# kubernetes-sigs/karpenter

Measured on NVIDIA H100. Metric: pods scheduled/sec, higher is better.
Workload: dtype int64

## Files before the change

### karpenter_b200/csrc/kp_api.cu

```cuda
#include <cuda_runtime.h>
#include <cub/cub.cuh>

#include <dlfcn.h>

#include <chrono>
#include <cstdio>
#include <cstdlib>
#include <memory>
#include <string>
#include <vector>

#include "kp_consolidate.cuh"
#include "kp_gosort_host.hpp"
#include "kp_prep.hpp"

#define CK(call)                                                                                     \
  do {                                                                                               \
    cudaError_t e_ = (call);                                                                         \
    if (e_ != cudaSuccess) {                                                                         \
      h->err = std::string(#call) + ": " + cudaGetErrorString(e_);                                   \
      return KP_ERR_CUDA;                                                                            \
    }                                                                                                \
  } while (0)

// ... 199 lines not shown
  if (i >= n) return;
  const KeyInfo ki{val_int, isint, univ};
  const kp_slot_case c = cs[i];
  const Slot a{c.flags_a, c.mask_a, c.gte_a, c.lte_a}, b{c.flags_b, c.mask_b, c.gte_b, c.lte_b};
  kp_slot_out o;
  memset(&o, 0, sizeof(o));
  if (slot_present(a) && slot_present(b)) {
    const Slot r = slot_intersection(ki, a, b);
    o.mask = r.m;
    o.gte = r.gte;
    o.lte = r.lte;
    o.flags = r.f;
    o.op = slot_op(r);
    o.has_intersection = slot_has_intersection(ki, a, b);
  }
  o.has_value = c.value >= 0 ? slot_has(ki, a, c.value) : 0;
  o.compatible = slot_compatible(ki, a, b, c.well_known != 0, c.allow_undefined != 0);
  out[i] = o;
}

static int kp_consolidate_impl(kp_handle* h, const kp_problem* p, const kp_consol_input* in, int64_t deadline_ms,
                               kp_consol_result* out);
extern "C" {

int kp_debug_slot_algebra(kp_handle* h, const int64_t* value_int, uint64_t value_is_int, uint64_t universe,
                          const kp_slot_case* cases, int32_t n, kp_slot_out* out) {
  if (n < 0 || !value_int || (n > 0 && (!cases || !out))) return h->err = "kp_debug_slot_algebra: bad arguments", KP_ERR_INVALID;
  cudaSetDevice(h->device);
  int64_t* dv = nullptr;
  kp_slot_case* dc = nullptr;
  kp_slot_out* dout = nullptr;
  CK(cudaMalloc(&dv, 64 * 8));
  CK(cudaMalloc(&dc, sizeof(kp_slot_case) * std::max(n, 1)));
  CK(cudaMalloc(&dout, sizeof(kp_slot_out) * std::max(n, 1)));
  CK(cudaMemcpy(dv, value_int, 64 * 8, cudaMemcpyHostToDevice));
  CK(cudaMemcpy(dc, cases, sizeof(kp_slot_case) * n, cudaMemcpyHostToDevice));
  if (n > 0) k_slot_kats<<<(n + 127) / 128, 128, 0, h->stream>>>(dv, value_is_int, universe, dc, n, dout);
  CK(cudaStreamSynchronize(h->stream));
  CK(cudaGetLastError());
  CK(cudaMemcpy(out, dout, sizeof(kp_slot_out) * n, cudaMemcpyDeviceToHost));
  cudaFree(dv);
  cudaFree(dc);
  cudaFree(dout);
  return KP_OK;
}
}

extern "C" {

#define KP_TRUNC_BLOCKS 132
int kp_version(void) { return KP_ABI_VERSION; }

int kp_go_sort_f64(const double* keys, int32_t n, int32_t* perm_out) {
  if (n < 0 || (n > 0 && (!keys || !perm_out))) return KP_ERR_INVALID;
  host_go_sort(keys, n, perm_out);
  return KP_OK;
}
int kp_go_sort_i64(const int64_t* keys, int32_t n, int32_t* perm_out) {
  if (n < 0 || (n > 0 && (!keys || !perm_out))) return KP_ERR_INVALID;
  host_go_sort(keys, n, perm_out);
  return KP_OK;
}

int kp_create(int device, kp_handle** out) {
  *out = nullptr;
  int count = 0;
  if (cudaGetDeviceCount(&count) != cudaSuccess || count == 0) return KP_ERR_CUDA;
  kp_handle* h = new kp_handle();
  if (device < 0) cudaGetDevice(&device);
  h->device = device;
  if (cudaSetDevice(device) != cudaSuccess || cudaStreamCreate(&h->stream) != cudaSuccess) {
    delete h;
    return KP_ERR_CUDA;
  }
  cudaEventCreate(&h->ev0);
  cudaEventCreate(&h->ev1);
  cudaEventCreate(&h->ev3);
  cudaDeviceGetAttribute(&h->n_sm, cudaDevAttrMultiProcessorCount, device);
  cudaDeviceSetLimit(cudaLimitStackSize, 16384);
  *out = h;
  return KP_OK;
}

void kp_destroy(kp_handle* h) {
  if (!h) return;
  cudaSetDevice(h->device);
  h->arena.destroy();
  cudaFree(h->d_devs);
  cudaFree(h->d_plan);
  if (h->comm && g_nccl.CommDestroy) g_nccl.CommDestroy(h->comm);
  if (h->ev3) cudaEventDestroy(h->ev3);
  if (h->ev0) cudaEventDestroy(h->ev0);
  if (h->ev1) cudaEventDestroy(h->ev1);
  if (h->stream) cudaStreamDestroy(h->stream);
  delete h;
}

const char* kp_last_error(kp_handle* h) { return h ? h->err.c_str() : "no handle"; }

int kp_get_stats(kp_handle* h, kp_stats* out) {
  *out = h->stats;
  return KP_OK;
}

static int upload_tables(kp_handle* h, Instance& in, const kp_problem* p, int cmax_hint) {
  HostTables& t = in.host;
  KpDev& d = in.dev;
  memset(&d, 0, sizeof(d));
  d.K = t.K;
  d.R = t.R;
  d.T = t.T;
  d.ITW = t.ITW;
  d.N = t.N;
  d.X = t.X;
  d.G = t.G;
  d.GH = t.GH;
  d.E = t.E;
  d.D = t.D;
  d.n_reqsets = t.n_reqsets;
  d.n_taintsets = t.n_taintsets;
  d.n_tolsets = t.n_tolsets;
  d.has_bounds = t.has_bounds;
  d.hostname_key = t.hostname_key;
  d.nodes_res = t.nodes_res;
  d.n_rv = t.n_rv;
  d.stable_order = p->claim_order_mode == 1;
  CK(up(h, &d.key_wellknown, t.key_wellknown));
  CK(up(h, &d.key_univ, t.key_univ));
  CK(up(h, &d.val_int, t.val_int));
  CK(up(h, &d.val_isint, t.val_isint));
  CK(up(h, &d.rs_flags, t.rs_flags));
  CK(up(h, &d.rs_mask, t.rs_mask));
  CK(up(h, &d.rs_gte, t.rs_gte));
  CK(up(h, &d.rs_lte, t.rs_lte));
  CK(up(h, &d.tol_ok, t.tol_ok));
  CK(up(h, &d.itv_off, t.itv_off));
  CK(up(h, &d.itv, t.itv));
  CK(up(h, &d.it_nokey, t.it_nokey));
  CK(up(h, &d.it_dne, t.it_dne));
  CK(up(h, &d.it_nonempty, t.it_nonempty));
  CK(up(h, &d.it_valid, t.it_valid));
  CK(up(h, &d.ge_off, t.ge_off));
  CK(up(h, &d.ge_vals, t.ge_vals));
  CK(up(h, &d.ge_bits, t.ge_bits));
  d.n_ge = (int)t.ge_vals.size();
  d.n_itv = std::max(t.itv_off[d.K], 1);
  CK(up(h, &d.off_slots, t.off_slots));
  CK(up(h, &d.off_keys, t.off_keys));
  CK(up(h, &d.offset_bits, t.offset_bits));
  CK(up(h, &d.it_capacity, t.it_capacity));
  CK(up(h, &d.tmpl_rs, t.tmpl_rs));
  CK(up(h, &d.tmpl_taintset, t.tmpl_taintset));
  CK(up(h, &d.tmpl_its_raw, t.tmpl_its_raw));
  CK(zeros(h, &d.tmpl_its, t.tmpl_its_raw.size()));
  CK(up(h, &d.tmpl_daemon, t.tmpl_daemon));
  CK(up_mut(h, in, &d.tmpl_remaining, t.tmpl_remaining));
  CK(up(h, &d.tmpl_limit_present, t.tmpl_limit_present));
  CK(up(h, &d.cls_req, t.cls_req));
  CK(up(h, &d.cls_rs, t.cls_rs));
  CK(up(h, &d.cls_tolset, t.cls_tolset));
  CK(up(h, &d.cls_relax, t.cls_relax));
  d.mv_strict = t.min_values_strict ? 1 : 0;
  CK(up(h, &d.tmpl_mv_off, t.tmpl_mv_off));
  CK(up(h, &d.tmpl_mv_key, t.tmpl_mv_key));
  CK(up(h, &d.tmpl_mv_need, t.tmpl_mv_need));
  CK(up(h, &d.mv_val_off, t.mv_val_off));
  CK(up(h, &d.mv_masks, t.mv_masks));
  CK(up(h, &d.cls_match, t.cls_match));
  CK(up(h, &d.cls_rec, t.cls_rec));
  {
    if (t.N > 64) return h->err = "more than 64 NodePools", KP_ERR_CAPACITY;
    const ClassPlan& plan = t.plan;
    const bool domain_fp = !getenv("KP_NO_DOMAIN_FP");
    const size_t XK = (size_t)std::max(t.X, 1) * t.K;
    std::vector<int64_t> pg(XK, 0), pl(XK, 0), sg(XK, 0), sl(XK, 0);
    std::vector<ClsLane> rows((size_t)std::max(t.X, 1) * 32);
    memset(rows.data(), 0, rows.size() * sizeof(ClsLane));
    for (int x = 0; x < t.X; x++) {
      const int nm = t.cls_match_off[x + 1] - t.cls_match_off[x], nr = t.cls_rec_off[x + 1] - t.cls_rec_off[x];
      const int asig = plan.asig[x];
      int tki = 0xff;
      if (!plan.chain[x]) {
        tki = asig < 64 ? asig | TKI_ABIT : 0xff;
        if (plan.fast[x] && asig < 64) tki |= TKI_FAST;
        if (plan.fp[x] && nm <= KP_PG && nr <= KP_PG && domain_fp) tki |= TKI_FP | (plan.has_tk[x] ? TKI_TK : 0);
        if (nm + nr > 0) tki |= TKI_TOPO;
      }
      const int32_t hdr[KP_HDR] = {t.cls_tolset[x], t.cls_rv[x], t.cls_match_off[x], t.cls_match_off[x + 1], t.cls_rec_off[x],
                                   t.cls_rec_off[x + 1], plan.fsig[x], plan.nsig[x], plan.hchk_off[x], plan.hchk_off[x + 1]};
      const size_t a = (size_t)t.cls_rs[x] * t.K, b = (size_t)t.cls_strict_rs[x] * t.K;
      for (int l = 0; l < 32; l++) {
        ClsLane& c = rows[(size_t)x * 32 + l];
        if (l < t.K) {
          c.pod_m = t.rs_mask[a + l];
          c.strict_m = t.rs_mask[b + l];
          c.pod_f = t.rs_flags[a + l];
          c.strict_f = t.rs_flags[b + l];
          pg[(size_t)x * t.K + l] = t.rs_gte[a + l];
          pl[(size_t)x * t.K + l] = t.rs_lte[a + l];
          sg[(size_t)x * t.K + l] = t.rs_gte[b + l];
          sl[(size_t)x * t.K + l] = t.rs_lte[b + l];
        }
        if (l < t.R) c.req = t.cls_req[(size_t)x * t.R + l];
        if (l < KP_HDR) c.hdr = hdr[l];
        if (l == KP_HDR + 2) c.hdr = (int32_t)(plan.tok[x] & 0xffffffffull);
        if (l == KP_HDR + 3) c.hdr = (int32_t)(plan.tok[x] >> 32);
        if (l == KP_HDR + 4) c.hdr = t.cls_relax[x];
        if (l == KP_HDR + 5) c.hdr = tki;
        if (l == KP_HDR + 10) c.hdr = t.cls_vol_next[x];
        if (l >= KP_HDR + 6 && l <= KP_HDR + 9 && p->n_hostports > 0 && p->class_hostports) {
          const uint64_t ports = p->class_hostports[x];
          uint64_t conf = 0;
          for (uint64_t m = ports; m;) {
            const int i = __builtin_ctzll(m);
            m &= m - 1;
            conf |= p->hostport_conflicts[i];
          }
          const uint64_t v = l < KP_HDR + 8 ? ports : conf;
          c.hdr = (int32_t)(((l - KP_HDR) & 1) ? (v >> 32) : (v & 0xffffffffull));
        }
      }
    }
    std::vector<int4> hchk;
    for (const HostCheck& c : plan.hchk) hchk.push_back(int4{c.row, c.type | (c.self << 8), c.max_skew, c.g});
    if (hchk.empty()) hchk.push_back(int4{0, 0, 0, 0});
    std::vector<int32_t> nsig_rs = plan.nsig_rs, nsig_tolset = plan.nsig_tolset;
    if (nsig_rs.empty()) {
      nsig_rs.push_back(0);
      nsig_tolset.push_back(-1);
    }
    d.tk_key = plan.tk_key;
    d.n_fsig = plan.n_fsig;
    d.n_nsig = (int)plan.nsig_rs.size();
    d.EW = (t.E + 31) / 32;
    in.strict_undefined = plan.strict_undefined ? 1 : 0;
    std::vector<int64_t> rv_req((size_t)std::max(t.n_rv, 1) * t.R, 0);
    for (int x = 0; x < t.X; x++)
      for (int r = 0; r < t.R; r++) rv_req[(size_t)t.cls_rv[x] * t.R + r] = t.cls_req[(size_t)x * t.R + r];
    {
      const int32_t *a_, *b_;
      const int64_t* c_;
      CK(up(h, &a_, nsig_rs));
      CK(up(h, &b_, nsig_tolset));
      CK(up(h, &c_, rv_req));
      in.d_nsig_rs = const_cast<int32_t*>(a_);
      in.d_nsig_tolset = const_cast<int32_t*>(b_);
      in.d_rv_req = const_cast<int64_t*>(c_);
    }
    CK(up(h, &d.cls_hchk, hchk));
    std::vector<uint32_t> nact(std::max(d.EW, 1), 0);
    for (int n = 0; n < t.E; n++)
      if (t.node_flags[n] & KP_NODE_SCHEDULABLE) nact[n >> 5] |= 1u << (n & 31);
    CK(up_mut(h, in, &d.nactive, nact));
    d.ESW = (d.EW + 31) / 32;
    CK(zeros(h, &d.nfit_sum, (size_t)std::max(t.n_rv, 1) * std::max(d.ESW, 1)));
    CK(zeros(h, &d.nstat_sum, (size_t)std::max(d.n_nsig, 1) * std::max(d.ESW, 1)));
    CK(zeros(h, &d.nfit, (size_t)std::max(t.n_rv, 1) * std::max(d.EW, 1)));
    CK(zeros(h, &d.nstat, (size_t)std::max(d.n_nsig, 1) * std::max(d.EW, 1)));
    CK(up(h, &d.cls_lane, rows));
    CK(up(h, &d.cp_g, pg));
    CK(up(h, &d.cp_l, pl));
    CK(up(h, &d.cs_g, sg));
    CK(up(h, &d.cs_l, sl));
  }
  CK(up(h, &d.groups, t.groups));
  CK(up(h, &d.filter_rs, t.filter_rs));
  CK(up_mut(h, in, &d.dom_cnt, t.dom_cnt));
  CK(up_mut(h, in, &d.dom_reg, t.dom_reg));
  CK(up_mut(h, in, &d.dom_pop, t.dom_pop));
  d.tk_slot = nullptr;
  d.tk_reg = d.tk_pop = nullptr;
  d.tk_cnt = nullptr;
  d.tk_nv = t.plan.tk_key >= 0 ? 64 - __builtin_clzll(t.key_univ[t.plan.tk_key] | 1ull) : 0;
  d.n_lazy = 0;
  for (int32_t b : t.g_born) d.n_lazy += b == 0;
  CK(up_mut(h, in, &d.g_born, t.g_born));
  CK(up_mut(h, in, &d.g_birth, t.g_birth));
  CK(up(h, &d.cls_lazy_off, t.cls_lazy_off));
  CK(up(h, &d.cls_lazy, t.cls_lazy));
  CK(up_mut(h, in, &d.g_ndomains, t.g_ndomains));
  CK(up_mut(h, in, &d.g_nempty, t.g_nempty));
  CK(up(h, &d.node_taintset, t.node_taintset));
  CK(up(h, &d.node_flags, t.node_flags));
  CK(up_mut(h, in, &d.node_rem, t.node_rem));
  CK(up_mut(h, in, &d.node_rem_present, t.node_rem_present));
  CK(up_mut(h, in, &d.node_sflags, t.node_sflags));
  CK(up_mut(h, in, &d.node_smask, t.node_smask));
  CK(up_mut(h, in, &d.node_sgte, t.node_sgte));
  CK(up_mut(h, in, &d.node_slte, t.node_slte));
  CK(zeros(h, &d.node_npods, (size_t)std::max(t.E, 1)));
  d.Cmax = cmax_hint;
  size_t C = (size_t)d.Cmax;
  CK(zeros(h, &d.c_tmpl, C));
  CK(zeros(h, &d.c_npods, C));
  CK(zeros(h, &d.c_req, C * t.R));
  CK(zeros(h, &d.c_sflags, C * t.K));
  CK(zeros(h, &d.c_smask, C * t.K));
  CK(zeros(h, &d.c_sgte, C * t.K));
  CK(zeros(h, &d.c_slte, C * t.K));
  CK(zeros(h, &d.c_its, C * t.ITW));
  CK(zeros(h, &d.c_j, C * t.R));
  CK(zeros(h, &d.order, C));
  CK(zeros(h, &d.cnt_at, C));
  CK(zeros(h, &d.cmask, C));
  CK(zeros(h, &d.amask, C));
  CK(zeros(h, &d.c_dom, C));
  d.n_hostports = p->n_hostports > 0 ? p->n_hostports : 0;
  if (d.n_hostports > 64) return h->err = "more than 64 distinct host ports", KP_ERR_CAPACITY;
  if (d.n_hostports > 0 && !p->hostport_conflicts) return h->err = "hostport_conflicts is null", KP_ERR_INVALID;
  {
    std::vector<unsigned long long> np(std::max(t.E, 1), 0ull), tp(std::max(t.N, 1), 0ull);
    for (int n = 0; n < t.E; n++)
      if (d.n_hostports && p->node_hostports) np[n] = p->node_hostports[n];
    for (int n = 0; n < t.N; n++)
      if (d.n_hostports && p->tmpl_hostports) tp[n] = p->tmpl_hostports[n];
    CK(up_mut(h, in, &d.node_ports, np));
    CK(up(h, &d.tmpl_ports, tp));
    CK(zeros(h, &d.c_ports, C));
  }
  d.n_rsv = t.n_rsv;
  d.rsv_strict = t.rsv_strict ? 1 : 0;
  d.rsv_sets = 0;
  {
    std::vector<int32_t> sr(std::max(t.D, 1), -1);
    for (int dd = 0; dd < t.D && dd < (int)t.set_rsv.size(); dd++) {
      sr[dd] = t.set_rsv[dd];
      if (sr[dd] >= 0) d.rsv_sets |= 1u << dd;
    }
    CK(up(h, &d.set_rsv, sr));
    std::vector<int32_t> cap0 = t.rsv_cap0;
    if (cap0.empty()) cap0.push_back(0);
    CK(up_mut(h, in, &d.rsv_cap, cap0));
    CK(zeros(h, &d.c_rsv, C));
    d.rsv_ct_key = p->reservation_capacity_type_key;
    d.rsv_reserved_val = p->reservation_reserved_value;
    d.rsv_id_key = p->reservation_id_key;
    memset(d.rsv_val_of, 0, sizeof(d.rsv_val_of));
    if (t.n_rsv > 0) {
      if (d.rsv_ct_key < 0 || d.rsv_ct_key >= t.K || d.rsv_id_key < 0 || d.rsv_id_key >= t.K || !p->reservation_value ||
          d.rsv_reserved_val < 0 || d.rsv_reserved_val >= 64)
        return h->err = "reserved offerings need reservation_capacity_type_key / reservation_id_key / reservation_value", KP_ERR_INVALID;
      for (int i = 0; i < t.n_rsv; i++) {
        if (p->reservation_value[i] < 0 || p->reservation_value[i] >= 64) return h->err = "reservation_value out of range", KP_ERR_INVALID;
        d.rsv_val_of[i] = 1ull << p->reservation_value[i];
      }
    }
  }
  d.tmpl_all = t.N >= 64 ? ~0ull : ((1ull << t.N) - 1);
  d.H = t.E + d.Cmax;
  d.GHS = std::max(t.GH, 1);
  CK(zeros(h, &d.host_cnt, (size_t)d.GHS * d.H));
  {
    std::vector<int32_t> tr((size_t)std::max(t.E, 1) * d.GHS, 0);
    for (int r = 0; r < t.GH; r++)
      for (int n = 0; n < t.E; n++) tr[(size_t)n * d.GHS + r] = t.host_cnt_nodes[(size_t)r * t.E + n];
    CK(up(h, &in.d_host_cnt_nodes, tr));
  }
  d.HW = (d.H + 31) / 32;
  CK(zeros(h, &d.host_pop, (size_t)std::max(t.GH, 1) * d.HW));
  {
    const int ew = (t.E + 31) / 32;
    std::vector<uint32_t> bits((size_t)std::max(t.GH, 1) * std::max(ew, 1), 0);
    for (int r = 0; r < t.GH; r++)
      for (int n = 0; n < t.E; n++)
        if (t.host_cnt_nodes[(size_t)r * t.E + n] > 0) bits[(size_t)r * ew + (n >> 5)] |= 1u << (n & 31);
    CK(up(h, &in.d_host_pop_nodes, bits));
  }
  CK(zeros(h, &d.n_claims, 1));
  CK(zeros(h, &d.counters, KP_NCOUNTERS));
  CK(zeros(h, &d.status, 1));
  return KP_OK;
}

static int reset_dynamic(kp_handle* h, Instance& in) {
  HostTables& t = in.host;
  KpDev& d = in.dev;
  for (auto& r : in.resets) CK(cudaMemcpyAsync(r.dst, r.src, r.bytes, cudaMemcpyDeviceToDevice, h->stream));
  CK(cudaMemsetAsync(d.node_npods, 0, (size_t)std::max(t.E, 1) * 4, h->stream));
  size_t C = (size_t)d.Cmax;
  CK(cudaMemsetAsync(d.c_npods, 0, C * 4, h->stream));
  CK(cudaMemsetAsync(d.cmask, 0, C * sizeof(ulonglong2), h->stream));
  CK(cudaMemsetAsync(d.amask, 0, C * 8, h->stream));
  CK(cudaMemsetAsync(d.c_rsv, 0, C * 8, h->stream));
  if (in.d_dropped) CK(cudaMemsetAsync(in.d_dropped, 0, C, h->stream));
  CK(cudaMemsetAsync(d.host_cnt, 0, (size_t)d.GHS * d.H * 4, h->stream));
  if (t.E && t.GH)
    CK(cudaMemcpyAsync(d.host_cnt, in.d_host_cnt_nodes, (size_t)t.E * d.GHS * 4, cudaMemcpyDeviceToDevice, h->stream));
  CK(cudaMemsetAsync(d.host_pop, 0, (size_t)std::max(t.GH, 1) * d.HW * 4, h->stream));
  if (t.E && t.GH) {
    const size_t ew = (size_t)(t.E + 31) / 32;
    CK(cudaMemcpy2DAsync(d.host_pop, (size_t)d.HW * 4, in.d_host_pop_nodes, ew * 4, ew * 4, t.GH,
                         cudaMemcpyDeviceToDevice, h->stream));
  }
  CK(cudaMemsetAsync(d.n_claims, 0, 4, h->stream));
  CK(cudaMemsetAsync(d.counters, 0, 128, h->stream));
  CK(cudaMemsetAsync(d.status, 0, 4, h->stream));
  CK(cudaMemsetAsync(d.last_len, 0, (size_t)std::max<int64_t>(in.P, 1) * 4, h->stream));
  return KP_OK;
}

static int plan_tables(const KpDev& d, size_t fixed, size_t budget) {
  const size_t tb = kp_tab_bytes(d);
  return (fixed + tb <= budget && tb <= 110 * 1024) ? (int)tb : 0;
}

static void plan_solve(Instance& in) {
  KpDev& d = in.dev;
  const size_t budget = 224 * 1024;
  d.tab_bytes = plan_tables(d, SolveSmem(d, 0, 0, 0, 0, 0).tab, budget);
  auto layout = [&](int CS, int CQ, int CR) { return SolveSmem(d, d.tab_bytes, CS, CQ, CR, in.tk_groups); };
  const bool dom_fp = std::any_of(in.host.plan.fp.begin(), in.host.plan.fp.end(), [](uint8_t f) { return f != 0; });
  in.tk_groups = 0;
  if (dom_fp && !in.cohort && d.tk_key >= 0 && d.tk_nv > 0 && d.tk_nv <= 64) {
    int ntk = 0;
    for (const KpGroup& G : in.host.groups) ntk += G.key == d.tk_key;
    const SolveSmem L(d, d.tab_bytes, 0, 0, 0, ntk);
    if (ntk > 0 && L.s_req - L.tk_slot <= 64 * 1024) in.tk_groups = ntk;
  }
  int CR = std::min(d.Cmax, 512);
  while (CR > 0 && layout(0, CR, CR).cmask > budget / 2) CR -= 32;
  CR = std::max(CR, 0);
  const SolveSmem whole = layout(0, CR, CR);
  const size_t rows = whole.cmask - whole.s_req;
  int CQ = CR;
  if (dom_fp) {
    CQ = std::min((d.Cmax + 31) / 32 * 32, (int)(rows / ((size_t)d.R * 12 + 1)) / 32 * 32);
    while (CQ > 0 && layout(0, CQ, 0).cmask - whole.s_req > rows) CQ -= 32;
    CR = 0;
    while (CR + 32 <= CQ && layout(0, CQ, CR + 32).cmask - whole.s_req <= rows) CR += 32;
  }
  int CS = 0;
  if (layout(64, CQ, CR).total <= budget) {
    int lo = 64, hi = ((d.Cmax + 31) / 32) * 32;
    while (lo < hi) {
      int mid = ((lo + hi + 32) / 64) * 32;
      if (mid <= lo) mid = lo + 32;
      if (layout(mid, CQ, CR).total <= budget)
        lo = mid;
      else
        hi = mid - 32;
    }
    CS = lo;
  }
  if (const char* cap = getenv("KP_SMEM_CAP")) {
    long v[4];
    bool set[4] = {false, false, false, false};
    for (int f = 0; f < 4 && cap; f++) {
      char* end;
      v[f] = std::max(0l, strtol(cap, &end, 10));
      set[f] = end != cap;
      cap = strchr(cap, ',');
      if (cap) cap++;
    }
    if (set[0]) CS = (int)std::min<long>(CS, v[0] / 32 * 32);
    if (set[1]) CQ = (int)std::min<long>(CQ, v[1]);
    if (set[2]) CR = (int)std::min<long>(CR, v[2]);
    if (set[3] && v[3] < in.tk_groups) in.tk_groups = 0;
  }
  CR = std::min(CR, CQ);
  in.lean = in.host.G == 0 && !in.host.has_bounds && !in.host.min_values_strict && in.host.n_rsv == 0 && d.n_hostports == 0 &&
            !in.host.has_vol_alts && !getenv("KP_NO_LEAN");
  if (in.host.has_vol_alts) in.cohort = false;
  in.CS = CS;
  in.CQ = CQ;
  in.CR = CR;
  in.smem = layout(CS, CQ, CR).total;
  if (getenv("KP_DEBUG"))
    fprintf(stderr, "[kp] solver plan: tables %zu B, topology-key groups on chip %d, hot rows %d, cold rows %d, small arrays %d, %zu B shared\n",
            (size_t)d.tab_bytes, in.tk_groups, CQ, CR, CS, in.smem);
}

static void begin_upload(kp_handle* h, kp_handle::Uploader by) {
  cudaSetDevice(h->device);
  cudaStreamSynchronize(h->stream);
  h->insts.clear();
  h->uploaded = by;
  h->d_gcnt = nullptr;
  h->gcnt_slots = 0;
  h->arena.reset();
  h->stats = kp_stats{};
}

static int add_instance(kp_handle* h, const kp_problem* p, int64_t cmax) {
  h->insts.push_back(std::make_unique<Instance>());
  Instance& in = *h->insts.back();
  auto t0 = std::chrono::steady_clock::now();
  std::vector<uint8_t> active(p->n_nodes, 0);
  for (int i = 0; i < p->n_nodes; i++) active[i] = (p->node_flags[i] & KP_NODE_SCHEDULABLE) != 0;
  std::vector<int32_t> pending(p->pod_class, p->pod_class + p->n_pods);
  int rc = kp_prepare(p, active, {}, pending, in.host, h->err);
  if (rc != KP_OK) return rc;
  auto t1 = std::chrono::steady_clock::now();
  h->stats.prep_ms += std::chrono::duration<double, std::milli>(t1 - t0).count();
  in.P = p->n_pods;
  in.n_keys = p->n_keys;
  in.n_resources = p->n_resources;
  in.n_its = p->n_its;
  in.n_nodes = p->n_nodes;
  in.hostname_key = in.host.hostname_key;
  in.key_nvalues.resize(p->n_keys);
  for (int k = 0; k < p->n_keys; k++) in.key_nvalues[k] = p->key_value_off[k + 1] - p->key_value_off[k];
  if (p->n_pods >= (1ll << 31) - 2) return h->err = "more than 2^31 pods", KP_ERR_CAPACITY;
  rc = upload_tables(h, in, p, (int)cmax);
  if (rc != KP_OK) return rc;
  KpDev& d = in.dev;
  d.P = p->n_pods;
  size_t P = (size_t)p->n_pods;
  CK(up_raw(h, &in.d_pod_class, p->pod_class, P));
  d.pod_class = in.d_pod_class;
  if (p->pod_creation) {
    CK(up_raw(h, &in.d_pod_creation, p->pod_creation, P));
  } else {
    CK(zeros(h, &in.d_pod_creation, P));
  }
  CK(up_raw(h, &in.d_uid_hi, p->pod_uid_hi, P));
  CK(up_raw(h, &in.d_uid_lo, p->pod_uid_lo, P));
  const std::vector<int64_t>& rank = in.host.plan.rank;
  CK(up_raw(h, &in.d_class_rank, rank.data(), rank.size()));
  {
    const int X = in.host.X;
    std::vector<int64_t> pods_of(std::max(X, 1), 0), classes_at(std::max(X, 1), 0);
    for (size_t i = 0; i < P; i++) pods_of[p->pod_class[i]]++;
    for (int x = 0; x < X; x++)
      if (pods_of[x] > 0) classes_at[rank[x]]++;
    int64_t in_runs = 0;
    for (int x = 0; x < X; x++)
      if (pods_of[x] > 1 && classes_at[rank[x]] == 1) in_runs += pods_of[x];
    in.cohort = (in_runs * 4 >= (int64_t)P && P > 0 && !getenv("KP_NO_COHORT")) || getenv("KP_COHORT");
    d.cohort = in.cohort ? 1 : 0;
  }
  in.max_its = p->max_instance_types > 0 ? p->max_instance_types : 0;
  if (in.max_its > 0) {
    const int T = p->n_its;
    const PriceLists ml = order_by_price(p, in.host);
    CK(up(h, &in.price_tabs.ml_off, ml.off));
    CK(up(h, &in.price_tabs.ml_set, ml.set));
    CK(up(h, &in.price_tabs.ml_price, ml.price));
    const size_t NW = (size_t)KP_TRUNC_BLOCKS * 4;
    CK(h->arena.alloc(&in.trunc_key, NW * std::max(T, 1)));
    CK(h->arena.alloc(&in.trunc_val, NW * std::max(T, 1)));
    CK(h->arena.alloc(&in.trunc_bits, NW * std::max((T + 63) / 64, 1)));
    CK(zeros(h, &in.d_dropped, (size_t)std::max<int64_t>(d.Cmax, 1)));
  }
  {
    int64_t* ka;
    int64_t* kb;
    CK(h->arena.alloc(&ka, P));
    CK(h->arena.alloc(&kb, P));
    CK(h->arena.alloc(&in.sort_perm_b, P));
    in.sort_keys_a = ka;
    in.sort_keys_b = kb;
    size_t n1 = 0, n2 = 0;
    cub::DeviceRadixSort::SortPairs(nullptr, n1, (const uint64_t*)nullptr, (uint64_t*)nullptr, (const int32_t*)nullptr,
                                    (int32_t*)nullptr, (int)std::max<size_t>(P, 1));
    cub::DeviceRadixSort::SortPairs(nullptr, n2, (const int64_t*)nullptr, (int64_t*)nullptr, (const int32_t*)nullptr,
                                    (int32_t*)nullptr, (int)std::max<size_t>(P, 1));
    in.sort_tmp_bytes = std::max(n1, n2);
    char* tmp;
    CK(h->arena.alloc(&tmp, in.sort_tmp_bytes));
    in.sort_tmp = tmp;
  }
  CK(zeros(h, &d.queue, P + 1));
  CK(zeros(h, &d.qcls, P + 1));
  CK(zeros(h, &d.last_len, P));
  CK(zeros(h, &d.pod_target, P));
  CK(zeros(h, &d.pod_error, P));
  CK(cudaStreamSynchronize(h->stream));
  auto t2 = std::chrono::steady_clock::now();
  h->stats.upload_ms += std::chrono::duration<double, std::milli>(t2 - t1).count();
  plan_solve(in);
  in.resident = true;
  return KP_OK;
}

static int upload(kp_handle* h, const kp_problem* const* problems, int n, const int64_t* cmax, kp_handle::Uploader by) {
  begin_upload(h, by);
  for (int b = 0; b < n; b++) {
    int rc = add_instance(h, problems[b], cmax[b]);
    if (rc != KP_OK) return rc;
  }
  return KP_OK;
}

static int64_t cmax_guess(const kp_problem* p) {
  return std::max<int64_t>(1, std::min<int64_t>(p->n_pods, std::max<int64_t>(4096, p->n_pods / 8)));
}

int kp_upload(kp_handle* h, const kp_problem* p) {
  const int64_t cmax = cmax_guess(p);
  return upload(h, &p, 1, &cmax, kp_handle::SINGLE);
}

__global__ void k_iota(int32_t* p, int64_t n) {
  int64_t i = blockIdx.x * (int64_t)blockDim.x + threadIdx.x;
  if (i < n) p[i] = (int32_t)i;
}

static int sort_queue(kp_handle* h, Instance& in) {
  KpDev& d = in.dev;
  const int64_t P = in.P;
  if (P <= 0) return KP_OK;
  const int nb = (int)((P + 255) / 256), n = (int)P;
  int32_t* perm_a = d.queue;
  int32_t* perm_b = in.sort_perm_b;
  uint64_t *ua = (uint64_t*)in.sort_keys_a, *ub = (uint64_t*)in.sort_keys_b;
  int64_t *sa = (int64_t*)in.sort_keys_a, *sb = (int64_t*)in.sort_keys_b;
  size_t tb = in.sort_tmp_bytes;
  k_iota<<<nb, 256, 0, h->stream>>>(perm_a, P);
  k_gather<<<nb, 256, 0, h->stream>>>(in.d_uid_lo, perm_a, P, ua);
  CK(cub::DeviceRadixSort::SortPairs(in.sort_tmp, tb, ua, ub, perm_a, perm_b, n, 0, 64, h->stream));
  k_gather<<<nb, 256, 0, h->stream>>>(in.d_uid_hi, perm_b, P, ua);
  CK(cub::DeviceRadixSort::SortPairs(in.sort_tmp, tb, ua, ub, perm_b, perm_a, n, 0, 64, h->stream));
  k_gather<<<nb, 256, 0, h->stream>>>(in.d_pod_creation, perm_a, P, sa);
  CK(cub::DeviceRadixSort::SortPairs(in.sort_tmp, tb, sa, sb, perm_a, perm_b, n, 0, 64, h->stream));
  k_sort_keys<<<nb, 256, 0, h->stream>>>(d.pod_class, in.d_class_rank, perm_b, P, sa);
  CK(cub::DeviceRadixSort::SortPairs(in.sort_tmp, tb, sa, sb, perm_b, perm_a, n, 0, 64, h->stream));
  k_gather<<<nb, 256, 0, h->stream>>>(d.pod_class, d.queue, P, d.qcls);
  h->stats.kernel_launches += 6;
  return KP_OK;
}

static int launch_node_cand(kp_handle* h, Instance& in) {
  KpDev& d = in.dev;
  if (d.E <= 0) return KP_OK;
  dim3 grid((d.E + 255) / 256, d.n_nsig + d.n_rv);
  k_node_cand<<<grid, 256, 0, h->stream>>>(d, in.d_nsig_rs, in.d_nsig_tolset, in.d_rv_req, in.strict_undefined);
  const int nsum = (d.n_rv + d.n_nsig) * d.ESW;
  k_node_sum<<<(nsum + 255) / 256, 256, 0, h->stream>>>(d);
  h->stats.kernel_launches += 2;
  return KP_OK;
}

static int prep_solve(kp_handle* h, Instance& in) {
  KpDev& d = in.dev;
  if (d.N > 0) {
    k_feasibility<<<(d.N * 32 + 255) / 256, 256, 0, h->stream>>>(d, nullptr, 1);
    h->stats.kernel_launches++;
  }
  int rc = sort_queue(h, in);
  if (rc != KP_OK) return rc;
  if (in.P > 0) {
    k_fill_i32<<<(int)((in.P + 255) / 256), 256, 0, h->stream>>>(d.pod_target, in.P, KP_TARGET_UNSCHEDULED);
    h->stats.kernel_launches++;
  }
  return launch_node_cand(h, in);
}

static int reduce_counters(kp_handle* h) {
  if (!h->d_gcnt) return KP_OK;
  CK(cudaEventRecord(h->ev3, h->stream));
  CK(cudaMemsetAsync(h->d_gcnt, 0, (size_t)h->gcnt_slots * 4, h->stream));
  for (auto& in : h->insts)
    if (in->n_slots > 0) {
      k_scatter_counts<<<(int)((in->n_slots + 255) / 256), 256, 0, h->stream>>>(in->dev.dom_cnt, in->d_slot_src, in->n_slots,
                                                                                 h->d_gcnt + in->slot_off);
      h->stats.kernel_launches++;
    }
  if (h->comm) {
    int rc = g_nccl.AllReduce(h->d_gcnt, h->d_gcnt, (size_t)h->gcnt_slots,  2,  0, h->comm, h->stream);
    if (rc != 0) return h->err = std::string("ncclAllReduce: ") + (g_nccl.GetErrorString ? g_nccl.GetErrorString(rc) : "?"), KP_ERR_CUDA;
  }
  return KP_OK;
}

static const void* solver_kernel(const std::vector<std::unique_ptr<Instance>>& insts) {
  bool lean = true, cohort = false, vol = false;
  for (auto& in : insts) {
    lean = lean && in->lean;
    cohort = cohort || in->cohort;
    vol = vol || in->host.has_vol_alts;
  }
  if (vol) return (const void*)k_wsolve_batch<false, false, true>;
  return lean ? (cohort ? (const void*)k_wsolve_batch<true, true> : (const void*)k_wsolve_batch<true, false>)
              : (cohort ? (const void*)k_wsolve_batch<false, true> : (const void*)k_wsolve_batch<false, false>);
}

static int run_solve(kp_handle* h, int64_t deadline_ms, std::vector<int32_t>& statuses) {
  const int n = (int)h->insts.size();
  statuses.assign(n, KP_OK);
  if (n == 0) return KP_OK;
  cudaSetDevice(h->device);
  if (n > h->devs_cap) {
    cudaFree(h->d_devs);
    cudaFree(h->d_plan);
    h->d_devs = nullptr;
    h->d_plan = nullptr;
    h->devs_cap = 0;
    CK(cudaMalloc(&h->d_devs, sizeof(KpDev) * n));
    CK(cudaMalloc(&h->d_plan, sizeof(int4) * n));
    h->devs_cap = n;
  }
  std::vector<KpDev> devs(n);
  std::vector<int4> plan(n);
  size_t smem = 0;
  for (int b = 0; b < n; b++) {
    Instance& in = *h->insts[b];
    if (!in.resident) return h->err = "the last upload did not complete", KP_ERR_INVALID;
    in.dev.deadline_ns = deadline_ms > 0 ? deadline_ms * 1000000ll : 0;
    int rc = reset_dynamic(h, in);
    if (rc != KP_OK) return rc;
    devs[b] = in.dev;
    plan[b] = make_int4(in.CS, in.CQ, in.CR, in.tk_groups);
    smem = std::max(smem, in.smem);
  }
  CK(cudaMemcpyAsync(h->d_devs, devs.data(), sizeof(KpDev) * n, cudaMemcpyHostToDevice, h->stream));
  CK(cudaMemcpyAsync(h->d_plan, plan.data(), sizeof(int4) * n, cudaMemcpyHostToDevice, h->stream));
  CK(cudaEventRecord(h->ev0, h->stream));
  h->stats.kernel_launches = 0;
  h->stats.cohort_pods = 0;
  for (auto& in : h->insts) {
    int rc = prep_solve(h, *in);
    if (rc != KP_OK) return rc;
  }
  const void* fn = solver_kernel(h->insts);
  CK(cudaFuncSetAttribute(fn, cudaFuncAttributeMaxDynamicSharedMemorySize, (int)smem));
  {
    void* args[] = {(void*)&h->d_devs, (void*)&h->d_plan};
    CK(cudaLaunchKernel(fn, dim3(n), dim3(64), args, smem, h->stream));
  }
  h->stats.kernel_launches++;
  for (auto& in : h->insts)
    if (in->max_its > 0) {
      k_truncate_claims<<<KP_TRUNC_BLOCKS, 128, 0, h->stream>>>(in->dev, in->price_tabs, in->max_its, in->trunc_key, in->trunc_val,
                                                                 in->trunc_bits, in->d_dropped);
      if (in->P > 0)
        k_mark_dropped<<<(int)((in->P + 255) / 256), 256, 0, h->stream>>>(in->dev.pod_target, in->dev.pod_error, in->d_dropped, in->P);
      h->stats.kernel_launches += 2;
    }
  int rc = reduce_counters(h);
  if (rc != KP_OK) return rc;
  CK(cudaEventRecord(h->ev1, h->stream));
  CK(cudaStreamSynchronize(h->stream));
  CK(cudaGetLastError());
  float ms = 0;
  cudaEventElapsedTime(&ms, h->ev0, h->ev1);
  h->stats.solve_ms = ms;
  if (h->d_gcnt) cudaEventElapsedTime(&h->allreduce_ms, h->ev3, h->ev1);
  if (getenv("KP_DEBUG")) fprintf(stderr, "[kp] %d instance(s): step %.3f ms\n", n, ms);
  for (int b = 0; b < n; b++) CK(cudaMemcpy(&statuses[b], h->insts[b]->dev.status, 4, cudaMemcpyDeviceToHost));
  return KP_OK;
}

struct ReqLayout {
  int K, hostname_key;
  std::vector<int> woff;
  explicit ReqLayout(const Instance& in) : K(in.n_keys), hostname_key(in.hostname_key), woff(in.n_keys + 1, 0) {
    for (int k = 0; k < K; k++) woff[k + 1] = woff[k] + (k == hostname_key ? 0 : (in.key_nvalues[k] + 63) / 64);
  }
  int words() const { return woff[K]; }
  void store(size_t r, const uint8_t* sf, const uint64_t* sm, const int64_t* sg, const int64_t* sl, uint8_t* flags,
             int64_t* gte, int64_t* lte, uint64_t* mask) const {
    for (int k = 0; k < K; k++) {
      const uint8_t f = sf[k];
      if (!(f & SF_PRESENT) || k == hostname_key) continue;
      flags[r * K + k] = KP_SLOT_PRESENT | ((f & SF_COMPLEMENT) ? KP_REQ_COMPLEMENT : 0) | ((f & SF_HAS_GTE) ? KP_REQ_HAS_GTE : 0) |
                         ((f & SF_HAS_LTE) ? KP_REQ_HAS_LTE : 0);
      if ((f & SF_HAS_GTE) && sg) gte[r * K + k] = sg[k];
      if ((f & SF_HAS_LTE) && sl) lte[r * K + k] = sl[k];
      if (woff[k + 1] > woff[k]) mask[r * words() + woff[k]] = sm[k];
    }
  }
};

static int download(kp_handle* h, Instance& in, kp_result* out) {
  KpDev& d = in.dev;
  auto t0 = std::chrono::steady_clock::now();
  memset(out, 0, sizeof(*out));
  int32_t nclaims = 0;
  int64_t counters[16];
  CK(cudaMemcpy(&nclaims, d.n_claims, 4, cudaMemcpyDeviceToHost));
  CK(cudaMemcpy(counters, d.counters, 128, cudaMemcpyDeviceToHost));
  h->stats.cohort_pods += counters[5];
  if (getenv("KP_DEBUG"))
    fprintf(stderr, "[kp] slow_sorts=%lld evals=%lld commits=%lld fast_commits=%lld cohort_pods=%lld\n", (long long)counters[4],
            (long long)counters[6], (long long)counters[3], (long long)counters[9], (long long)counters[5]);
  int64_t P = in.P;
  int K = in.n_keys, R = in.n_resources, ITW = (in.n_its + 63) / 64;
  size_t C = (size_t)nclaims, c1 = C ? C : 1;
  out->n_pods = P;
  out->pod_target = (int32_t*)malloc(sizeof(int32_t) * (P ? P : 1));
  out->pod_error = (uint8_t*)malloc(P ? P : 1);
  CK(cudaMemcpy(out->pod_target, d.pod_target, P * 4, cudaMemcpyDeviceToHost));
  CK(cudaMemcpy(out->pod_error, d.pod_error, P, cudaMemcpyDeviceToHost));
  out->n_claims = nclaims;
  out->claim_template = (int32_t*)calloc(c1, 4);
  out->claim_npods = (int32_t*)calloc(c1, 4);
  out->claim_rank = (int32_t*)calloc(c1, 4);
  out->claim_reservations = (uint64_t*)calloc(c1, 8);
  CK(cudaMemcpy(out->claim_reservations, d.c_rsv, C * 8, cudaMemcpyDeviceToHost));
  out->claim_dropped = (uint8_t*)calloc(c1, 1);
  if (in.d_dropped) CK(cudaMemcpy(out->claim_dropped, in.d_dropped, C, cudaMemcpyDeviceToHost));
  out->claim_requests = (int64_t*)calloc(c1 * R, 8);
  out->it_words = ITW;
  out->claim_its = (uint64_t*)calloc(c1 * (ITW ? ITW : 1), 8);
  CK(cudaMemcpy(out->claim_template, d.c_tmpl, C * 4, cudaMemcpyDeviceToHost));
  CK(cudaMemcpy(out->claim_npods, d.c_npods, C * 4, cudaMemcpyDeviceToHost));
  CK(cudaMemcpy(out->claim_requests, d.c_req, C * R * 8, cudaMemcpyDeviceToHost));
  CK(cudaMemcpy(out->claim_its, d.c_its, C * ITW * 8, cudaMemcpyDeviceToHost));
  std::vector<int32_t> order(c1);
  CK(cudaMemcpy(order.data(), d.order, C * 4, cudaMemcpyDeviceToHost));
  for (size_t pos = 0; pos < C; pos++) out->claim_rank[order[pos]] = (int32_t)pos;
  std::vector<uint8_t> sf(c1 * K);
  std::vector<uint64_t> sm(c1 * K);
  std::vector<int64_t> sg(c1 * K), sl(c1 * K);
  CK(cudaMemcpy(sf.data(), d.c_sflags, C * K, cudaMemcpyDeviceToHost));
  CK(cudaMemcpy(sm.data(), d.c_smask, C * K * 8, cudaMemcpyDeviceToHost));
  CK(cudaMemcpy(sg.data(), d.c_sgte, C * K * 8, cudaMemcpyDeviceToHost));
  CK(cudaMemcpy(sl.data(), d.c_slte, C * K * 8, cudaMemcpyDeviceToHost));
  const ReqLayout L(in);
  const int MW = L.words();
  out->n_keys = K;
  out->mask_words = MW;
  out->claim_req_flags = (uint8_t*)calloc(c1 * (K ? K : 1), 1);
  out->claim_req_gte = (int64_t*)calloc(c1 * (K ? K : 1), 8);
  out->claim_req_lte = (int64_t*)calloc(c1 * (K ? K : 1), 8);
  out->claim_req_mask = (uint64_t*)calloc(c1 * (MW ? MW : 1), 8);
  for (size_t c = 0; c < C; c++)
    L.store(c, sf.data() + c * K, sm.data() + c * K, sg.data() + c * K, sl.data() + c * K, out->claim_req_flags,
            out->claim_req_gte, out->claim_req_lte, out->claim_req_mask);
  HostTables& t = in.host;
  std::vector<int32_t> cnt((size_t)std::max(t.G, 1) * 64);
  CK(cudaMemcpy(cnt.data(), d.dom_cnt, cnt.size() * 4, cudaMemcpyDeviceToHost));
  std::vector<int32_t> birth(std::max(t.G, 1));
  CK(cudaMemcpy(birth.data(), d.g_birth, birth.size() * 4, cudaMemcpyDeviceToHost));
  std::vector<int> gorder;
  for (int g = 0; g < t.n_regular; g++)
    if (t.g_born[g]) gorder.push_back(g);
  {
    std::vector<std::pair<int, int>> born;
    for (int g = 0; g < t.n_regular; g++)
      if (!t.g_born[g] && birth[g] >= 0) born.push_back({birth[g], g});
    std::sort(born.begin(), born.end());
    for (auto& b : born) gorder.push_back(b.second);
  }
  for (int g = t.n_regular; g < t.G; g++) gorder.push_back(g);
  std::vector<int32_t> off{0}, flat;
  for (int g : gorder) {
    int key = t.groups[g].key;
    if (key != t.hostname_key) {
      int nv = in.key_nvalues[key];
      for (int v = 0; v < nv; v++) flat.push_back(cnt[(size_t)g * 64 + v]);
    }
    off.push_back((int32_t)flat.size());
  }
  out->n_groups = (int32_t)gorder.size();
  out->n_domain_slots = (int32_t)flat.size();
  out->group_domain_off = (int32_t*)malloc(off.size() * 4);
  memcpy(out->group_domain_off, off.data(), off.size() * 4);
  out->domain_counts = (int32_t*)malloc((flat.size() ? flat.size() : 1) * 4);
  if (!flat.empty()) memcpy(out->domain_counts, flat.data(), flat.size() * 4);
  out->n_existing_evals = counters[0];
  out->n_inflight_evals = counters[1];
  out->n_template_evals = counters[2];
  out->n_commits = counters[3];
  out->solve_ms = h->stats.solve_ms;
  h->stats.bytes_d2h += P * 5 + C * (8 + (size_t)R * 8 + (size_t)ITW * 8 + (size_t)K * 25) + cnt.size() * 4;
  auto t1 = std::chrono::steady_clock::now();
  h->stats.download_ms += std::chrono::duration<double, std::milli>(t1 - t0).count();
  return KP_OK;
}

static int download_all(kp_handle* h, const std::vector<int32_t>& statuses, kp_result* outs) {
  h->stats.download_ms = 0;
  h->stats.bytes_d2h = 0;
  int worst = KP_OK;
  for (size_t b = 0; b < h->insts.size(); b++) {
    int rc = download(h, *h->insts[b], &outs[b]);
    if (rc != KP_OK) {
      for (size_t i = 0; i < b; i++) kp_result_free(&outs[i]);
      return rc;
    }
    if (statuses[b] == KP_DEADLINE) worst = KP_DEADLINE;
  }
  return worst;
}

static int solve_uploaded(kp_handle* h, int64_t deadline_ms, kp_result* outs) {
  std::vector<int32_t> st;
  int rc = run_solve(h, deadline_ms, st);
  if (rc != KP_OK) return rc;
  for (int32_t s : st)
    if (s != KP_OK && s != KP_DEADLINE) return h->err = "claim capacity exceeded", s;
  return download_all(h, st, outs);
}

static int solve_growing(kp_handle* h, const kp_problem* const* problems, int n, kp_handle::Uploader by, int64_t deadline_ms,
                         kp_result* outs) {
  std::vector<int64_t> cmax(n);
  for (int b = 0; b < n; b++) cmax[b] = cmax_guess(problems[b]);
  for (;;) {
    int rc = upload(h, problems, n, cmax.data(), by);
    if (rc != KP_OK) return rc;
    std::vector<int32_t> st;
    rc = run_solve(h, deadline_ms, st);
    if (rc != KP_OK) return rc;
    bool grow = false;
    for (int b = 0; b < n; b++) {
      if (st[b] == KP_ERR_CAPACITY && cmax[b] < problems[b]->n_pods) {
        cmax[b] = std::min<int64_t>(problems[b]->n_pods, cmax[b] * 4);
        grow = true;
      } else if (st[b] != KP_OK && st[b] != KP_DEADLINE) {
        return h->err = "claim capacity exceeded", st[b];
      }
    }
    if (!grow) return download_all(h, st, outs);
  }
}

int kp_solve_resident(kp_handle* h, int64_t deadline_ms, kp_result* out) {
  if (h->uploaded != kp_handle::SINGLE) return h->err = "kp_upload has not been called", KP_ERR_INVALID;
  return solve_uploaded(h, deadline_ms, out);
}

int kp_solve(kp_handle* h, const kp_problem* p, int64_t deadline_ms, kp_result* out) {
  return solve_growing(h, &p, 1, kp_handle::SINGLE, deadline_ms, out);
}

int kp_comm_unique_id(uint8_t* id128) {
  std::string err;
  if (!nccl_load(err)) return KP_ERR_CUDA;
  KpNcclId id;
  if (g_nccl.GetUniqueId(&id) != 0) return KP_ERR_CUDA;
  memcpy(id128, &id, sizeof(id));
  return KP_OK;
}

int kp_comm_init(kp_handle* h, const uint8_t* id128, int32_t rank, int32_t world) {
  if (!nccl_load(h->err)) return KP_ERR_CUDA;
  if (h->comm) {
    g_nccl.CommDestroy(h->comm);
    h->comm = nullptr;
  }
  cudaSetDevice(h->device);
  KpNcclId id;
  memcpy(&id, id128, sizeof(id));
  int rc = g_nccl.CommInitRank(&h->comm, world, id, rank);
  if (rc != 0) return h->err = std::string("ncclCommInitRank: ") + (g_nccl.GetErrorString ? g_nccl.GetErrorString(rc) : "?"), KP_ERR_CUDA;
  h->comm_rank = rank;
  h->comm_world = world;
  return KP_OK;
}

static Instance* pick_instance(kp_handle* h, int32_t instance) {
  const size_t i = instance < 0 ? 0 : (size_t)instance;
  if (h->uploaded != (instance < 0 ? kp_handle::SINGLE : kp_handle::BATCH) || i >= h->insts.size()) return nullptr;
  return h->insts[i]->resident ? h->insts[i].get() : nullptr;
}
int64_t kp_comm_counter_slots(kp_handle* h, int32_t instance) {
  Instance* in = pick_instance(h, instance);
  if (!in) return -1;
  int64_t n = 0;
  for (int g = 0; g < in->host.G; g++)
    if (in->host.groups[g].key != in->host.hostname_key) n += in->key_nvalues[in->host.groups[g].key];
  return n;
}

int kp_comm_set_counter_layout(kp_handle* h, int64_t total_slots, const int64_t* slot_offset, int32_t n_instances) {
  cudaSetDevice(h->device);
  if (n_instances <= 0 ? !pick_instance(h, -1) : h->uploaded != kp_handle::BATCH || n_instances != (int)h->insts.size())
    return h->err = "kp_comm_set_counter_layout: the instances do not match the upload", KP_ERR_INVALID;
  if (total_slots < 0) return h->err = "kp_comm_set_counter_layout: negative size", KP_ERR_INVALID;
  CK(h->arena.alloc(&h->d_gcnt, (size_t)std::max<int64_t>(total_slots, 1)));
  h->gcnt_slots = total_slots;
  for (size_t i = 0; i < h->insts.size(); i++) {
    Instance* in = h->insts[i].get();
    std::vector<int32_t> src;
    for (int g = 0; g < in->host.G; g++) {
      const int key = in->host.groups[g].key;
      if (key == in->host.hostname_key) continue;
      for (int v = 0; v < in->key_nvalues[key]; v++) src.push_back(g * 64 + v);
    }
    in->n_slots = (int64_t)src.size();
    in->slot_off = slot_offset[i];
    if (in->slot_off < 0 || in->slot_off + in->n_slots > total_slots)
      return h->err = "kp_comm_set_counter_layout: slice outside the table", KP_ERR_INVALID;
    CK(h->arena.alloc(&in->d_slot_src, std::max<size_t>(src.size(), 1)));
    if (!src.empty()) CK(cudaMemcpyAsync(in->d_slot_src, src.data(), src.size() * 4, cudaMemcpyHostToDevice, h->stream));
    CK(cudaStreamSynchronize(h->stream));
  }
  return KP_OK;
}

int kp_comm_global_counts(kp_handle* h, int32_t* out, int64_t n) {
  if (!h->d_gcnt || n != h->gcnt_slots) return h->err = "kp_comm_global_counts: no table of that size", KP_ERR_INVALID;
  cudaSetDevice(h->device);
  CK(cudaMemcpy(out, h->d_gcnt, (size_t)n * 4, cudaMemcpyDeviceToHost));
  return KP_OK;
}

double kp_comm_last_allreduce_ms(kp_handle* h) { return h->allreduce_ms; }

#ifdef KP_PHASE_PROF
int kp_phase_profile(kp_handle* h, int32_t instance, int64_t* out, int32_t n) {
  Instance* in = pick_instance(h, instance);
  if (!in || n < KP_NPHASE + 1) return h->err = "kp_phase_profile: no such instance or buffer too small", -1;
  cudaSetDevice(h->device);
  CK(cudaMemcpy(out, in->dev.counters + KP_PROF_AT, (KP_NPHASE + 1) * 8, cudaMemcpyDeviceToHost));
  return KP_NPHASE + 1;
}
#endif

void kp_comm_destroy(kp_handle* h) {
  if (h->comm && g_nccl.CommDestroy) g_nccl.CommDestroy(h->comm);
  h->comm = nullptr;
}

int kp_upload_batch(kp_handle* h, const kp_problem* const* problems, int32_t n) {
  if (n < 0 || (n > 0 && !problems)) return h->err = "kp_upload_batch: bad arguments", KP_ERR_INVALID;
  std::vector<int64_t> cmax(n);
  for (int b = 0; b < n; b++) cmax[b] = cmax_guess(problems[b]);
  return upload(h, problems, n, cmax.data(), kp_handle::BATCH);
}

int kp_solve_batch_resident(kp_handle* h, int64_t deadline_ms, kp_result* outs) {
  if (h->uploaded != kp_handle::BATCH) return KP_OK;
  return solve_uploaded(h, deadline_ms, outs);
}

int kp_solve_batch(kp_handle* h, const kp_problem* const* problems, int32_t n, int64_t deadline_ms, kp_result* outs) {
  if (n < 0 || (n > 0 && (!problems || !outs))) return h->err = "kp_solve_batch: bad arguments", KP_ERR_INVALID;
  return solve_growing(h, problems, n, kp_handle::BATCH, deadline_ms, outs);
}

void kp_result_free(kp_result* r) {
  free(r->pod_target);
  free(r->pod_error);
  free(r->claim_template);
  free(r->claim_npods);
  free(r->claim_rank);
  free(r->claim_requests);
  free(r->claim_its);
  free(r->claim_req_flags);
  free(r->claim_req_gte);
  free(r->claim_req_lte);
  free(r->claim_req_mask);
  free(r->group_domain_off);
  free(r->domain_counts);
  free(r->claim_reservations);
  free(r->claim_dropped);
  memset(r, 0, sizeof(*r));
}

int kp_feasibility(kp_handle* h, const kp_problem* p, uint64_t* out_bits, int32_t* out_it_words) {
  const int64_t one = 1;
  int rc = upload(h, &p, 1, &one, kp_handle::SINGLE);
  if (rc != KP_OK) return rc;
  KpDev& d = h->insts[0]->dev;
  *out_it_words = d.ITW;
  size_t n = (size_t)d.X * d.N * d.ITW;
  uint64_t* dout;
  CK(cudaMalloc(&dout, std::max<size_t>(n, 1) * 8));
  if (d.N > 0) k_feasibility<<<(d.N * 32 + 255) / 256, 256, 0, h->stream>>>(d, nullptr, 1);
  CK(cudaEventRecord(h->ev0, h->stream));
  if (d.N > 0 && d.X > 0) {
    int blocks = h->n_sm * 8;
    k_feasibility<<<blocks, 256, 0, h->stream>>>(d, dout, 0);
  }
  CK(cudaEventRecord(h->ev1, h->stream));
  CK(cudaStreamSynchronize(h->stream));
  CK(cudaGetLastError());
  float ms = 0;
  cudaEventElapsedTime(&ms, h->ev0, h->ev1);
  h->stats.solve_ms = ms;
  CK(cudaMemcpy(out_bits, dout, n * 8, cudaMemcpyDeviceToHost));
  cudaFree(dout);
  return KP_OK;
}

int kp_consolidate(kp_handle* h, const kp_problem* cluster, const kp_consol_input* in, int64_t deadline_ms,
                   kp_consol_result* out) {
  memset(out, 0, sizeof(*out));
  int rc = kp_consolidate_impl(h, cluster, in, deadline_ms, out);
  if (rc != KP_OK && rc != KP_DEADLINE) kp_consol_result_free(out);
  return rc;
}

void kp_consol_result_free(kp_consol_result* r) {
  free(r->decision);
  free(r->replacement_its);
  free(r->n_new_claims);
  free(r->n_unscheduled);
  free(r->repl_template);
  free(r->repl_requests);
  free(r->repl_req_flags);
  free(r->repl_req_gte);
  free(r->repl_req_lte);
  free(r->repl_req_mask);
  free(r->repl_order_off);
  free(r->repl_order);
  memset(r, 0, sizeof(*r));
}
}

__global__ void k_scatter_rank(const int32_t* perm, int64_t n, int32_t* rank) {
  int64_t i = blockIdx.x * (int64_t)blockDim.x + threadIdx.x;
  if (i < n) rank[perm[i]] = (int32_t)i;
}

static int read_consol(kp_handle* h, const KpConsol& q, int n, const int32_t* at, const ReqLayout& L, int R, int ITW,
                       std::vector<std::vector<int32_t>>& order_rows, kp_consol_result* out) {
  const size_t K = (size_t)L.K, n1 = (size_t)std::max(n, 1), cap = (size_t)q.order_cap;
  auto sub = [&](size_t b) { return at ? (size_t)at[b] : b; };
  auto rows = [&](auto* dst, const auto* src, size_t width) {
    const size_t row = width * sizeof(*dst);
    if (!at) return cudaMemcpy(dst, src, n * row, cudaMemcpyDeviceToHost);
    std::vector<std::remove_pointer_t<decltype(dst)>> tmp(n1 * width);
    const cudaError_t e = cudaMemcpy(tmp.data(), src, n * row, cudaMemcpyDeviceToHost);
    for (size_t b = 0; b < (size_t)n; b++) memcpy(dst + sub(b) * width, tmp.data() + b * width, row);
    return e;
  };
  CK(rows(out->decision, q.decision, 1));
  CK(rows(out->replacement_its, q.replacement_its, ITW));
  CK(rows(out->n_new_claims, q.n_new_claims, 1));
  CK(rows(out->n_unscheduled, q.n_unscheduled, 1));
  CK(rows(out->repl_template, q.repl_tmpl, 1));
  CK(rows(out->repl_requests, q.repl_req, R));
  std::vector<uint8_t> sfl(n1 * K);
  std::vector<uint64_t> smk(n1 * K);
  std::vector<int32_t> on(n1), ord(q.repl_order ? n1 * cap : 0);
  std::vector<int64_t> sg(q.repl_sgte ? n1 * K : 0), sl(sg.size());
  CK(cudaMemcpy(sfl.data(), q.repl_sflags, (size_t)n * K, cudaMemcpyDeviceToHost));
  CK(cudaMemcpy(smk.data(), q.repl_smask, (size_t)n * K * 8, cudaMemcpyDeviceToHost));
  if (q.repl_sgte) {
    CK(cudaMemcpy(sg.data(), q.repl_sgte, (size_t)n * K * 8, cudaMemcpyDeviceToHost));
    CK(cudaMemcpy(sl.data(), q.repl_slte, (size_t)n * K * 8, cudaMemcpyDeviceToHost));
  }
  if (q.repl_order) {
    CK(cudaMemcpy(ord.data(), q.repl_order, (size_t)n * cap * 4, cudaMemcpyDeviceToHost));
    CK(cudaMemcpy(on.data(), q.repl_order_n, (size_t)n * 4, cudaMemcpyDeviceToHost));
  }
  for (size_t b = 0; b < (size_t)n; b++) {
    const size_t s = sub(b);
    if (out->decision[s] != KP_DECISION_REPLACE)
      out->repl_template[s] = -1;
    else
      L.store(s, sfl.data() + b * K, smk.data() + b * K, q.repl_sgte ? sg.data() + b * K : nullptr,
              q.repl_sgte ? sl.data() + b * K : nullptr, out->repl_req_flags, out->repl_req_gte, out->repl_req_lte,
              out->repl_req_mask);
    if (q.repl_order) order_rows[s].assign(ord.begin() + b * cap, ord.begin() + b * cap + on[b]);
  }
  return KP_OK;
}

static int kp_consolidate_impl(kp_handle* h, const kp_problem* p, const kp_consol_input* in, int64_t deadline_ms,
                               kp_consol_result* out) {
  const auto t_call = std::chrono::steady_clock::now();
  const int S = in->n_subsets;
  const int n_extra = in->n_extra_pods > 0 ? in->n_extra_pods : 0;
  if (p->n_nodes > 0 && !in->node_pod_off) return h->err = "kp_consolidate: node_pod_off is null", KP_ERR_INVALID;
  const int64_t extra_row0 = p->n_nodes > 0 ? in->node_pod_off[p->n_nodes] : 0;
  if (n_extra > 0 && (!in->extra_pod_kind || extra_row0 + n_extra != p->n_pods))
    return h->err = "kp_consolidate: the extra pods must be the last n_extra_pods rows of the pod table, with kinds", KP_ERR_INVALID;
  for (int i = 0; i < n_extra; i++)
    if (in->extra_pod_kind[i] != KP_EXTRA_PENDING && in->extra_pod_kind[i] != KP_EXTRA_DELETING_NODE)
      return h->err = "kp_consolidate: unknown extra pod kind", KP_ERR_INVALID;
  const int64_t one = 1;
  int rc = upload(h, &p, 1, &one, kp_handle::SINGLE);
  if (rc != KP_OK) return rc;
  Instance& cl = *h->insts[0];
  HostTables& t = cl.host;
  KpDev& d = cl.dev;
  if (t.has_vol_alts) {
    h->err = "consolidation with pods that have several volume-topology alternatives is not supported yet";
    return KP_ERR_UNSUPPORTED;
  }
  if (t.has_min_values && !t.min_values_strict) {
    h->err = "consolidation with minValues under the BestEffort policy is not supported yet";
    return KP_ERR_UNSUPPORTED;
  }
  const int K = t.K, R = t.R, ITW = t.ITW, E = t.E, T = t.T;
  const bool general = t.G > 0;
  const ReqLayout L(cl);
  const int MW = L.words();
  {
    const size_t s1 = S ? S : 1;
    out->n_subsets = S;
    out->it_words = ITW;
    out->n_keys = K;
    out->mask_words = MW;
    out->n_resources = R;
    out->decision = (uint8_t*)malloc(s1);
    memset(out->decision, KP_DECISION_UNKNOWN, s1);
    out->replacement_its = (uint64_t*)calloc(s1 * (ITW ? ITW : 1), sizeof(uint64_t));
    out->n_new_claims = (int32_t*)calloc(s1, sizeof(int32_t));
    out->n_unscheduled = (int32_t*)calloc(s1, sizeof(int32_t));
    out->repl_template = (int32_t*)malloc(s1 * 4);
    for (size_t i = 0; i < s1; i++) out->repl_template[i] = -1;
    out->repl_requests = (int64_t*)calloc(s1 * (R ? R : 1), 8);
    out->repl_req_flags = (uint8_t*)calloc(s1 * (K ? K : 1), 1);
    out->repl_req_gte = (int64_t*)calloc(s1 * (K ? K : 1), 8);
    out->repl_req_lte = (int64_t*)calloc(s1 * (K ? K : 1), 8);
    out->repl_req_mask = (uint64_t*)calloc(s1 * (MW ? MW : 1), 8);
  }
  const int order_cap = std::min(std::max(T, 1), 600);
  std::vector<std::vector<int32_t>> order_rows(in->export_price_order ? S : 0);
  auto finish_order = [&]() {
    if (!in->export_price_order) return;
    out->repl_order_off = (int32_t*)calloc((size_t)S + 1, 4);
    size_t tot = 0;
    for (int s_ = 0; s_ < S; s_++) {
      tot += order_rows[s_].size();
      out->repl_order_off[s_ + 1] = (int32_t)tot;
    }
    out->repl_order = (int32_t*)calloc(tot ? tot : 1, 4);
    for (int s_ = 0; s_ < S; s_++)
      if (!order_rows[s_].empty()) memcpy(out->repl_order + out->repl_order_off[s_], order_rows[s_].data(), order_rows[s_].size() * 4);
  };
  auto ms_left = [&]() -> int64_t {
    if (deadline_ms <= 0) return -1;
    const double used = std::chrono::duration<double, std::milli>(std::chrono::steady_clock::now() - t_call).count();
    return std::max<int64_t>(0, deadline_ms - (int64_t)used);
  };
  auto t_begin = std::chrono::steady_clock::now();
  const ConsolPrices cp = consol_prices(p, t, in);
  const PriceLists ml = order_by_price(p, t);
  auto upload_prices = [&](KpConsol& q) -> int {
    q.ct_key = in->capacity_type_key;
    q.ct_spot = in->ct_spot;
    q.ct_od = in->ct_on_demand;
    q.export_order = in->export_price_order ? 1 : 0;
    q.order_cap = order_cap;
    q.ct_order_valid = cp.ct_valid;
    q.spot_to_spot_enabled = in->spot_to_spot_enabled;
    q.T = T;
    CK(up(h, &q.node_price, cp.node_price));
    uint8_t* u8;
    CK(up_raw(h, &u8, in->node_is_spot, (size_t)E));
    q.node_is_spot = u8;
    int32_t* nit = nullptr;
    CK(up_raw(h, &nit, in->node_it, (size_t)E));
    q.node_it = nit;
    q.filter_same_type = in->filter_same_instance_type;
    CK(up(h, &q.ml_off, ml.off));
    CK(up(h, &q.ml_set, ml.set));
    CK(up(h, &q.ml_price, ml.price));
    CK(up(h, &q.wl_off, cp.worst.off));
    CK(up(h, &q.wl_set, cp.worst.set));
    CK(up(h, &q.wl_price, cp.worst.price));
    return KP_OK;
  };
  auto alloc_rows = [&](KpConsol& q, size_t n) -> int {
    CK(zeros(h, &q.decision, n));
    CK(zeros(h, &q.replacement_its, n * std::max(ITW, 1)));
    CK(zeros(h, &q.n_new_claims, n));
    CK(zeros(h, &q.n_unscheduled, n));
    CK(zeros(h, &q.repl_tmpl, n));
    CK(zeros(h, &q.repl_req, n * std::max(R, 1)));
    CK(zeros(h, &q.repl_sflags, n * std::max(K, 1)));
    CK(zeros(h, &q.repl_smask, n * std::max(K, 1)));
    if (t.has_bounds) {
      CK(zeros(h, &q.repl_sgte, n * std::max(K, 1)));
      CK(zeros(h, &q.repl_slte, n * std::max(K, 1)));
    }
    if (in->export_price_order) {
      CK(zeros(h, &q.repl_order, n * order_cap));
      CK(zeros(h, &q.repl_order_n, n));
    }
    return KP_OK;
  };
#define KP_ALLOC_SCRATCH(f, type, count, present) \
  if (present) CK(zeros(h, &q.ws.f, slots * (size_t)(count)));
  for (int s = 0; s < S; s++)
    for (int i = in->subset_off[s]; i < in->subset_off[s + 1]; i++)
      if (in->subset_nodes[i] < 0 || in->subset_nodes[i] >= E) return h->err = "subset node out of range", KP_ERR_INVALID;
  if (general) {
    const std::unique_ptr<Instance> cluster = std::move(h->insts[0]);
    h->insts.clear();
    h->uploaded = kp_handle::NONE;
    double total_ms = 0;
    bool timed_out = false;
    const int CHUNK = 2 * h->n_sm;
    std::vector<uint8_t> is_cand(std::max(E, 1), 0), flags(std::max(E, 1), 0);
    for (int c0 = 0; c0 < S && !timed_out; c0 += CHUNK) {
      const int c1 = std::min(S, c0 + CHUNK);
      if (deadline_ms > 0 && ms_left() == 0) {
        timed_out = true;
        break;
      }
      begin_upload(h, kp_handle::NONE);
      std::vector<int> set_of;
      std::vector<int32_t> soff{0}, snodes_all;
      for (int s = c0; s < c1; s++) {
        const int so = in->subset_off[s], sn = in->subset_off[s + 1] - so;
        std::fill(is_cand.begin(), is_cand.end(), 0);
        for (int i = 0; i < sn; i++) is_cand[in->subset_nodes[so + i]] = 1;
        for (int n = 0; n < E; n++)
          flags[n] = is_cand[n] ? (uint8_t)(p->node_flags[n] & ~KP_NODE_SCHEDULABLE) : p->node_flags[n];
        std::vector<int32_t> pod_class, run_class(p->run_class, p->run_class + p->n_running),
            run_node(p->run_node, p->run_node + p->n_running);
        std::vector<int64_t> creation;
        std::vector<uint64_t> uid_hi, uid_lo;
        std::vector<uint8_t> kinds;
        auto take = [&](int64_t j, uint8_t kind) {
          pod_class.push_back(p->pod_class[j]);
          creation.push_back(p->pod_creation ? p->pod_creation[j] : 0);
          uid_hi.push_back(p->pod_uid_hi[j]);
          uid_lo.push_back(p->pod_uid_lo[j]);
          kinds.push_back(kind);
        };
        for (int n = 0; n < E; n++)
          for (int j = in->node_pod_off[n]; j < in->node_pod_off[n + 1]; j++) {
// ... 197 lines not shown
```

### karpenter_b200/csrc/kp_consolidate.cuh

```cuda
#pragma once
#include "kp_wsolve.cuh"

#define KP_ALIGN16(x) (((x) + 15) & ~(size_t)15)

#define KP_STAGED_TABLES(X, d)                                    \
  X(key_wellknown, uint8_t, d.K)                                  \
  X(key_univ, uint64_t, d.K)                                      \
  X(val_isint, uint64_t, d.K)                                     \
  X(ge_off, int32_t, (size_t)d.R + 1)                             \
  X(ge_vals, int64_t, d.n_ge)                                     \
  X(ge_bits, uint64_t, (size_t)d.n_ge * d.ITW)                    \
  X(itv_off, int32_t, (size_t)d.K + 1)                            \
  X(itv, uint64_t, (size_t)d.n_itv * d.ITW)                       \
  X(it_nokey, uint64_t, (size_t)d.K * d.ITW)                      \
  X(it_dne, uint64_t, (size_t)d.K * d.ITW)                        \
  X(it_nonempty, uint64_t, (size_t)d.K * d.ITW)                   \
  X(it_valid, uint64_t, d.ITW)                                    \
  X(off_slots, Slot, (size_t)(d.D > 0 ? d.D : 1) * d.K)           \
  X(off_keys, uint32_t, d.D > 0 ? d.D : 1)                        \
  X(offset_bits, uint64_t, (size_t)(d.D > 0 ? d.D : 1) * d.ITW)   \
  X(tmpl_taintset, int32_t, d.N > 0 ? d.N : 1)                    \
  X(nfit_sum, uint32_t, (size_t)d.n_rv * d.ESW)                   \
  X(nstat_sum, uint32_t, (size_t)d.n_nsig * d.ESW)

__host__ __device__ inline size_t kp_tab_bytes(const KpDev& d) {
  size_t b = 0;
#define KP_TAB_BYTES(field, type, count) b += KP_ALIGN16(sizeof(type) * (size_t)(count));
  KP_STAGED_TABLES(KP_TAB_BYTES, d)
#undef KP_TAB_BYTES
  return b;
}

__device__ __forceinline__ void stage_tables(const KpDev& d_in, KpDev* ds, unsigned char* tab) {
  const int tid = threadIdx.x, nt = blockDim.x;
  {
    const int* src = reinterpret_cast<const int*>(&d_in);
    int* dst = reinterpret_cast<int*>(ds);
    for (int i = tid; i < (int)(sizeof(KpDev) / 4); i += nt) dst[i] = src[i];
  }
  __syncthreads();
  if (d_in.tab_bytes > 0) {
    size_t off = 0;
#define KP_STAGE(field, type, count)                                     \
  {                                                                      \
    size_t n_ = (size_t)(count);                                         \
    type* dst_ = reinterpret_cast<type*>(tab + off);                     \
    const type* src_ = d_in.field;                                       \
    for (size_t i_ = tid; i_ < n_; i_ += nt) dst_[i_] = src_[i_];        \
    if (tid == 0) ds->field = dst_;                                      \
    off += KP_ALIGN16(sizeof(type) * n_);                                \
  }
    KP_STAGED_TABLES(KP_STAGE, d_in)
#undef KP_STAGE
  }
  __syncthreads();
}

__global__ void __launch_bounds__(256) k_node_cand(KpDev d, const int32_t* nsig_rs, const int32_t* nsig_tolset,
                                                    const int64_t* rv_req, int strict_undefined) {
  const int n = blockIdx.x * blockDim.x + threadIdx.x, row = blockIdx.y, lane = threadIdx.x & 31;
  bool bit = false;
  if (n < d.E) {
    if (row < d.n_nsig) {
      bit = tolerated(d, nsig_tolset[row], d.node_taintset[n]);
      const int rs = nsig_rs[row];
      for (int k = 0; rs >= 0 && k < d.K && bit; k++) {
        Slot pod = rs_slot(d, rs, k);
        if (!slot_present(pod)) continue;
        Slot nd = load_slot(d.node_sflags, d.node_smask, d.node_sgte, d.node_slte, (size_t)n * d.K + k, d.has_bounds);
        if (!slot_present(nd)) {
          if (strict_undefined && !op_is_negative(slot_op(pod))) bit = false;
        } else if (!slot_has_intersection(key_info(d, k), nd, pod) &&
                   !(op_is_negative(slot_op(pod)) && op_is_negative(slot_op(nd)))) {
          bit = false;
        }
      }
    } else {
      const int rv = row - d.n_nsig;
      const uint32_t pr = d.node_rem_present[n];
      bit = true;
      for (int r = 0; r < d.R; r++) {
        const int64_t rem = d.node_rem[(size_t)n * d.R + r];
        const bool present = (pr >> r) & 1;
        if (present && rem < 0) bit = false;
        if (rv_req[(size_t)rv * d.R + r] > (present ? rem : 0)) bit = false;
      }
    }
  }
  const unsigned m = __ballot_sync(FULL, bit);
  const int w = n >> 5;
  if (lane == 0 && w < d.EW) {
    if (row < d.n_nsig)
      d.nstat[(size_t)row * d.EW + w] = m;
    else
      d.nfit[(size_t)(row - d.n_nsig) * d.EW + w] = m;
  }
}

__global__ void __launch_bounds__(256) k_node_sum(KpDev d) {
  const int i = blockIdx.x * blockDim.x + threadIdx.x, rows = d.n_rv + d.n_nsig;
  if (i >= rows * d.ESW) return;
  const int row = i / d.ESW, s = i % d.ESW;
  const uint32_t* src = row < d.n_rv ? d.nfit + (size_t)row * d.EW : d.nstat + (size_t)(row - d.n_rv) * d.EW;
  uint32_t out = 0;
  for (int w = 0; w < 32; w++) {
    const int idx = s * 32 + w;
    if (idx < d.EW && (src[idx] & d.nactive[idx])) out |= 1u << w;
  }
  if (row < d.n_rv)
    d.nfit_sum[(size_t)row * d.ESW + s] = out;
  else
    d.nstat_sum[(size_t)(row - d.n_rv) * d.ESW + s] = out;
}

struct WSolveShared {
  KpDev ds;
  WInst inst;
  StageRing ring;
  Slot scratch[KP_MAXK];
};

struct SolveSmem {
  size_t tab, tk_slot, tk_reg, tk_pop, tk_cnt, s_req, s_j, s_smask, s_its, s_sflags, cmask, amask, order, cnt_at, c_tmpl,
      c_dom, total;
  __host__ __device__ SolveSmem(const KpDev& d, size_t tab_bytes, int CS, int CQ, int CR, int ntk) {
    size_t o = KP_ALIGN16(sizeof(WSolveShared));
    auto at = [&o](size_t& r, size_t bytes) {
      r = o;
      o += bytes;
    };
    at(tab, tab_bytes);
    const size_t tk = ntk > 0 ? ntk : 0, q = CQ > 0 ? CQ : 0, c = CR > 0 ? CR : 0, s = CS > 0 ? CS : 0;
    at(tk_slot, tk ? KP_ALIGN16((size_t)d.G * 4) : 0);
    at(tk_reg, KP_ALIGN16(tk * 8));
    at(tk_pop, KP_ALIGN16(tk * 8));
    at(tk_cnt, KP_ALIGN16(tk * d.tk_nv * 4));
    at(s_req, KP_ALIGN16(q * d.R * 8));
    at(s_j, KP_ALIGN16(q * d.R * 4));
    at(s_smask, KP_ALIGN16(c * d.K * 8));
    at(s_its, KP_ALIGN16(c * d.ITW * 8));
    at(s_sflags, KP_ALIGN16(c * d.K));
    at(cmask, s * 16);
    at(amask, s * 8);
    at(order, s * 4);
    at(cnt_at, s * 4);
    at(c_tmpl, s * 4);
    at(c_dom, s);
    total = o + 64;
  }
};

template <bool LEAN, bool COHORT, bool VOL>
__device__ __forceinline__ void wsolve_cta(const KpDev& d_in, int CS, int CQ, int CR, int ntk) {
  extern __shared__ __align__(16) unsigned char smem_raw[];
  WSolveShared& sh = *reinterpret_cast<WSolveShared*>(smem_raw);
  const int lane = threadIdx.x & 31, warp = threadIdx.x >> 5;
  stage_tables(d_in, &sh.ds, smem_raw + SolveSmem(d_in, 0, 0, 0, 0, 0).tab);
  const KpDev& d = sh.ds;
  WInst& I = sh.inst;
  const SolveSmem L(d, d.tab_bytes, CS, CQ, CR, ntk);
  int32_t* s_slot = nullptr;
  uint64_t *s_reg = nullptr, *s_pop = nullptr;
  int32_t* s_cnt = nullptr;
  if (ntk > 0) {
    const int nv = d_in.tk_nv;
    s_slot = reinterpret_cast<int32_t*>(smem_raw + L.tk_slot);
    s_reg = reinterpret_cast<uint64_t*>(smem_raw + L.tk_reg);
    s_pop = reinterpret_cast<uint64_t*>(smem_raw + L.tk_pop);
    s_cnt = reinterpret_cast<int32_t*>(smem_raw + L.tk_cnt);
    if (warp == 0) {
      for (int base = 0, n = 0; base < d_in.G; base += 32) {
        const int g = base + lane;
        const KpGroup* G_ = g < d_in.G ? d_in.groups + g : nullptr;
        const bool on = G_ && G_->key == d_in.tk_key;
        const unsigned m = __ballot_sync(FULL, on);
        const int s = n + __popc(m & ((1u << lane) - 1));
        if (g < d_in.G) s_slot[g] = on ? s : -1;
        if (on) {
          s_reg[s] = d_in.dom_reg[g];
          s_pop[s] = d_in.dom_pop[g];
          for (int v = 0; v < nv; v++) s_cnt[s * nv + v] = d_in.dom_cnt[G_->dom_off + v];
        }
        n += __popc(m);
      }
    }
  }
  const int Cmax = d.Cmax;
  if (threadIdx.x == 0) {
    sh.ring.produced = 0;
    sh.ring.consumed = 0;
    sh.ring.tail_pub = (int)d.P;
    sh.ring.done = 0;
    sh.ring.skip_to = 0;
    I.P = (int)d.P;
    I.queue = d.queue;
    I.qcls = d.qcls;
    I.last_len = d.last_len;
    I.pod_target = d.pod_target;
    I.pod_error = d.pod_error;
    I.pod_kind = d.pod_kind;
    I.Cmax = Cmax;
    I.c_tmpl = d.c_tmpl;
    I.c_npods = d.c_npods;
    I.c_req = d.c_req;
    I.c_sflags = d.c_sflags;
    I.c_smask = d.c_smask;
    I.c_sgte = d.c_sgte;
    I.c_slte = d.c_slte;
    I.c_its = d.c_its;
    I.c_j = d.c_j;
    I.order = d.order;
    I.cnt_at = d.cnt_at;
    I.cmask = d.cmask;
    I.amask = d.amask;
    I.tmpl_remaining = d.tmpl_remaining;
    I.node_rem = d.node_rem;
    I.node_rem_present = d.node_rem_present;
    I.node_sflags = d.node_sflags;
    I.node_smask = d.node_smask;
    I.node_sgte = d.node_sgte;
    I.node_slte = d.node_slte;
    I.node_npods = d.node_npods;
    I.nfit = d.nfit;
    I.nstat = d.nstat;
    I.nactive = d.nactive;
    I.nfit_sum = d.nfit_sum;
    I.nstat_sum = d.nstat_sum;
    I.n_removed = 0;
    I.removed = nullptr;
    I.ov_cap = 0;
    I.n_ov = 0;
    I.CS = 0;
    I.g_order = d.order;
    I.g_cnt_at = d.cnt_at;
    I.g_c_tmpl = d.c_tmpl;
    I.g_cmask = d.cmask;
    I.g_amask = d.amask;
    I.c_dom = d.c_dom;
    I.g_c_dom = d.c_dom;
    I.rsv_cap = d.rsv_cap;
    I.c_rsv = d.c_rsv;
    I.c_ports = d.c_ports;
    I.node_ports = d.node_ports;
    I.ov_ports = nullptr;
    I.CQ = 0;
    I.CR = 0;
    if (ntk > 0) {
      sh.ds.tk_slot = s_slot;
      sh.ds.tk_reg = s_reg;
      sh.ds.tk_pop = s_pop;
      sh.ds.tk_cnt = s_cnt;
    }
    if (CQ > 0) {
      I.s_req = reinterpret_cast<int64_t*>(smem_raw + L.s_req);
      I.s_j = reinterpret_cast<int32_t*>(smem_raw + L.s_j);
      I.CQ = CQ;
    }
    if (CR > 0) {
      I.s_smask = reinterpret_cast<uint64_t*>(smem_raw + L.s_smask);
      I.s_its = reinterpret_cast<uint64_t*>(smem_raw + L.s_its);
      I.s_sflags = reinterpret_cast<uint8_t*>(smem_raw + L.s_sflags);
      I.CR = CR;
    }
    if (CS > 0) {
      I.cmask = reinterpret_cast<ulonglong2*>(smem_raw + L.cmask);
      I.amask = reinterpret_cast<unsigned long long*>(smem_raw + L.amask);
      I.order = reinterpret_cast<int32_t*>(smem_raw + L.order);
      I.cnt_at = reinterpret_cast<int32_t*>(smem_raw + L.cnt_at);
      I.c_tmpl = reinterpret_cast<int32_t*>(smem_raw + L.c_tmpl);
      I.c_dom = reinterpret_cast<uint8_t*>(smem_raw + L.c_dom);
      I.CS = CS;
    }
  }
  __syncthreads();
  if (warp == 1) {
    stager_run<COHORT>(d, I, &sh.ring, lane);
    return;
  }
  wsolve_run<false, true, LEAN, COHORT, VOL>(d, I, sh.ring.slot[0], sh.scratch, lane, &sh.ring);
  const int nC = I.n_claims;
  claim_rows_flush(d, I, nC, lane);
  if (ntk > 0) {
    for (int g = lane; g < d.G; g += 32) {
      const int s = s_slot[g];
      if (s < 0) continue;
      d_in.dom_reg[g] = s_reg[s];
      d_in.dom_pop[g] = s_pop[s];
      for (int v = 0; v < d.tk_nv; v++) d_in.dom_cnt[d_in.groups[g].dom_off + v] = s_cnt[s * d.tk_nv + v];
    }
    __syncwarp();
  }
  if (!LEAN) claims_finalize(d, I.c_sflags, I.c_smask, I.c_rsv, nC, lane);
  if (I.CS > 0) {
    for (int i = lane; i < nC; i += 32) {
      d_in.order[i] = I.order[i];
      d_in.cnt_at[i] = I.cnt_at[i];
      d_in.c_tmpl[i] = I.c_tmpl[i];
    }
  }
  if (lane == 0) {
    *d.n_claims = nC;
    *d.status = I.status;
    d.counters[0] = I.ev_existing;
    d.counters[1] = I.ev_inflight;
    d.counters[2] = I.ev_tmpl;
    d.counters[3] = I.commits;
    d.counters[4] = I.slow_sorts;
    d.counters[5] = I.scan_chunks;
    d.counters[6] = I.evals;
    d.counters[7] = I.n_unsched;
    d.counters[8] = I.n_uninit;
    d.counters[9] = I.fast_commits;
#ifdef KP_PHASE_PROF
    for (int p = 0; p < KP_NPHASE; p++) d.counters[KP_PROF_AT + p] = I.prof[p];
    d.counters[KP_PROF_AT + KP_NPHASE] = I.prof_total;
#endif
  }
}
template <bool LEAN, bool COHORT, bool VOL = false>
__global__ void __launch_bounds__(64, 1) k_wsolve_batch(const KpDev* __restrict__ devs, const int4* __restrict__ plan) {
  const int4 pl = plan[blockIdx.x];
  wsolve_cta<LEAN, COHORT, VOL>(devs[blockIdx.x], pl.x, pl.y, pl.z, LEAN || COHORT ? 0 : pl.w);
}


#define KP_SORT_SCRATCH(X, d, q)                                     \
  X(sort_key, double, q.T, true)                                     \
  X(sort_val, int32_t, q.T, true)                                    \
  X(sort_bits, unsigned long long, d.ITW, true)
#define KP_CONSOL_SCRATCH(X, d, q)                                   \
  X(queue, int32_t, (size_t)q.capq + 1, true)                        \
  X(qcls, int32_t, (size_t)q.capq + 1, true)                         \
  X(last_len, int32_t, q.capq, true)                                 \
  X(clsl, int32_t, q.capq, true)                                     \
  X(rk, int32_t, q.capq, true)                                       \
  X(kindl, uint8_t, q.capq, q.n_extra > 0)  \
  X(rsv_cap, int32_t, d.n_rsv, d.n_rsv > 0)  \
  X(c_rsv, unsigned long long, q.capq, d.n_rsv > 0)                  \
  X(c_ports, unsigned long long, q.capq, d.n_hostports > 0)  \
  X(ov_ports, unsigned long long, q.capq, d.n_hostports > 0)         \
  X(c_tmpl, int32_t, q.capq, true)                                   \
  X(c_npods, int32_t, q.capq, true)                                  \
  X(order, int32_t, q.capq, true)                                    \
  X(cnt_at, int32_t, q.capq, true)                                   \
  X(c_req, int64_t, (size_t)q.capq * d.R, true)                      \
  X(c_sflags, uint8_t, (size_t)q.capq * d.K, true)                   \
  X(c_smask, uint64_t, (size_t)q.capq * d.K, true)                   \
  X(c_its, uint64_t, (size_t)q.capq * d.ITW, true)                   \
  X(c_j, int32_t, (size_t)q.capq * d.R, true)                        \
  KP_SORT_SCRATCH(X, d, q)                                           \
  X(cmask, ulonglong2, q.capq, true)                                 \
  X(amask, unsigned long long, q.capq, true)                         \
  X(tmpl_remaining, int64_t, (size_t)(d.N > 0 ? d.N : 1) * d.R, true) \
  X(ov_node, int32_t, q.capq, true)                                  \
  X(ov_rem, int64_t, (size_t)q.capq * d.R, true)                     \
  X(ov_present, uint32_t, q.capq, true)                              \
  X(ov_sflags, uint8_t, (size_t)q.capq * d.K, true)                  \
  X(ov_smask, uint64_t, (size_t)q.capq * d.K, true)                  \
  X(c_sgte, int64_t, (size_t)q.capq * d.K, d.has_bounds)             \
  X(c_slte, int64_t, (size_t)q.capq * d.K, d.has_bounds)             \
  X(ov_sgte, int64_t, (size_t)q.capq * d.K, d.has_bounds)            \
  X(ov_slte, int64_t, (size_t)q.capq * d.K, d.has_bounds)
struct ConsolScratch {
#define KP_SCRATCH_FIELD(f, type, count, present) type* f;
  KP_CONSOL_SCRATCH(KP_SCRATCH_FIELD, , )
#undef KP_SCRATCH_FIELD
};

struct KpConsol {
  int n_subsets;
  const int32_t* subset_off;
  const int32_t* subset_nodes;
  const int32_t* node_pod_off;
  const int32_t* pod_class;
  const int32_t* pod_rank;
  const double* node_price;
  const uint8_t* node_is_spot;
  const int32_t* node_it;
  int filter_same_type;
  const int32_t* node_tmpl;
  const int64_t* node_capacity;
  const int64_t* tmpl_remaining0;
  const int32_t* wl_off;
  const int32_t* wl_set;
  const double* wl_price;
  const int32_t* ml_off;
  const int32_t* ml_set;
  const double* ml_price;
  int T;
  int ct_key, ct_spot, ct_od, ct_order_valid;
  int spot_to_spot_enabled;
  int n_extra, extra_row0;
  const uint8_t* extra_kind;
  long long deadline_ns;
  unsigned long long* t_start;
  int capq;
  ConsolScratch ws;
  uint8_t* decision;
  uint64_t* replacement_its;
  int32_t* n_new_claims;
  int32_t* n_unscheduled;
  int32_t* repl_tmpl;
  int64_t* repl_req;
  uint8_t* repl_sflags;
  uint64_t* repl_smask;
  int64_t *repl_sgte, *repl_slte;
  int export_order;
  int32_t* repl_order;
  int32_t* repl_order_n;
  int order_cap;
  int32_t* next;
  int32_t* status;
};

__device__ __forceinline__ ConsolScratch consol_slot(const KpDev& d, const KpConsol& q, size_t slot) {
  ConsolScratch w;
#define KP_SCRATCH_SLOT(f, type, count, present) w.f = (present) ? q.ws.f + slot * (size_t)(count) : nullptr;
  KP_CONSOL_SCRATCH(KP_SCRATCH_SLOT, d, q)
#undef KP_SCRATCH_SLOT
  return w;
}

struct PriceTabs {
  const int32_t* ml_off;
  const int32_t* ml_set;
  const double* ml_price;
};
__device__ __forceinline__ void order_by_price(const PriceTabs& pt, uint64_t cur, int n_its, unsigned okmask, double* sk,
                                               int32_t* sv, int ITW, int lane) {
  const int cw = lane < ITW ? __popcll(cur) : 0;
  int pre = cw;
  for (int o = 1; o < 32; o <<= 1) {
    const int t = __shfl_up_sync(FULL, pre, o);
    if (lane >= o) pre += t;
  }
  int at = pre - cw;
  for (uint64_t bits = lane < ITW ? cur : 0ull; bits;) {
    const int b = __ffsll((long long)bits) - 1;
    bits &= bits - 1;
    const int t = lane * 64 + b;
    double mp = 1.7976931348623157e308;
    for (int e = pt.ml_off[t]; e < pt.ml_off[t + 1]; e++)
      if ((okmask >> pt.ml_set[e]) & 1u) {
        mp = pt.ml_price[e];
        break;
      }
    sk[at] = mp;
    sv[at] = t;
    at++;
  }
  __syncwarp();
  WarpSorterT<double> srt{sk, sv, lane};
  srt.pdqsort(0, n_its, WarpSorterT<double>::bits_len((unsigned long long)n_its));
}
__device__ __forceinline__ uint64_t first_types_bitmap(const int32_t* sv, int n, unsigned long long* sb, int ITW, int lane) {
  if (lane < ITW) sb[lane] = 0ull;
  __syncwarp();
  for (int i = lane; i < n; i += 32) atomicOr(&sb[sv[i] >> 6], 1ull << (sv[i] & 63));
  __syncwarp();
  return lane < ITW ? sb[lane] : 0ull;
}

__device__ __forceinline__ void consol_decide(const KpDev& d, const KpConsol& q, size_t slot, Slot* scratch,
                                              const uint8_t* c_sflags, const uint64_t* c_smask, const int64_t* c_sgte,
                                              const int64_t* c_slte, const uint64_t* c_its, int c_tmpl0, const int64_t* c_req0,
                                              int c_npods0, int sn, const int32_t* snodes, int unscheduled, int n_new, int s,
                                              int lane) {
  const int K = d.K, ITW = d.ITW;
  int decision = KP_DECISION_NOOP;
  uint64_t rep = 0;
  bool have_slots = false;
  bool spot_pinned = false, mv_dropped = false;
  int n_ord_out = 0;
  if (!unscheduled) {
    if (n_new == 0) {
      decision = KP_DECISION_DELETE;
    } else if (n_new == 1) {
      Slot S = lane < K ? load_slot(c_sflags, c_smask, c_sgte, c_slte, (size_t)lane, d.has_bounds) : slot_absent();
      const uint64_t its = lane < ITW ? c_its[lane] : 0ull;
      int n_its = lane < ITW ? __popcll(its) : 0;
      for (int o = 16; o; o >>= 1) n_its += __shfl_xor_sync(FULL, n_its, o);
      double price = 0;
      bool zero = false, all_spot = true;
      for (int i = 0; i < sn; i++) {
        const double np = q.node_price[snodes[i]];
        if (np < 0) zero = true;
        price += np;
        if (!q.node_is_spot[snodes[i]]) all_spot = false;
      }
      if (zero) price = 0.0;
      bool spot_ok = false;
      if (q.ct_key >= 0 && q.ct_spot >= 0) {
        const uint32_t f = __shfl_sync(FULL, S.f, q.ct_key);
        const uint64_t m = __shfl_sync(FULL, S.m, q.ct_key);
        const int64_t g = __shfl_sync(FULL, S.gte, q.ct_key), l = __shfl_sync(FULL, S.lte, q.ct_key);
        spot_ok = slot_has(key_info(d, q.ct_key), Slot{f, m, g, l}, q.ct_spot);
      }
      if (lane < K) scratch[lane] = S;
      __syncwarp();
      have_slots = true;
      unsigned okmask = offering_ok_mask(d, scratch, lane);
      const bool spot_path = all_spot && spot_ok;
      uint64_t cur = its;
      const ConsolScratch w = consol_slot(d, q, slot);
      double* sk = w.sort_key;
      int32_t* sv = w.sort_val;
      unsigned long long* sb = w.sort_bits;
      int n_ord = 0;
      const bool need_order = n_its > 600 || (spot_path && q.spot_to_spot_enabled) || q.export_order;
      if (need_order) {
        order_by_price(PriceTabs{q.ml_off, q.ml_set, q.ml_price}, cur, n_its, okmask, sk, sv, ITW, lane);
        n_ord = n_its;
        if (n_ord > 600) {
          n_ord = 600;
          cur = first_types_bitmap(sv, n_ord, sb, ITW, lane);
          if (d.mv_strict && !min_values_ok(d, c_tmpl0, cur, lane)) {
            mv_dropped = true;
            unscheduled = c_npods0;
          }
        }
      }
      if (mv_dropped) {
        decision = KP_DECISION_NOOP;
      } else if (spot_path && !q.spot_to_spot_enabled) {
        decision = KP_DECISION_NOOP;
      } else {
        if (spot_path) {
          if (lane == q.ct_key)
            scratch[lane] = slot_add(key_info(d, lane), scratch[lane], Slot{SF_PRESENT, 1ull << q.ct_spot, 0, 0});
          spot_pinned = true;
          __syncwarp();
          okmask = offering_ok_mask(d, scratch, lane);
          uint64_t keep = 0;
          for (uint64_t bits = lane < ITW ? cur : 0ull; bits;) {
            const int b = __ffsll((long long)bits) - 1;
            bits &= bits - 1;
            const int t = lane * 64 + b;
            for (int e = q.ml_off[t]; e < q.ml_off[t + 1]; e++)
              if ((okmask >> q.ml_set[e]) & 1u) {
                keep |= 1ull << b;
                break;
              }
          }
          cur = keep;
        }
        if (lane < ITW) {
          for (uint64_t bits = cur; bits;) {
            const int b = __ffsll((long long)bits) - 1;
            bits &= bits - 1;
            const int t = lane * 64 + b;
            double worst = 1.7976931348623157e308;
            for (int ci = 0; ci < 3 && worst > 1e308; ci++) {
              if (q.ct_key < 0 || !((q.ct_order_valid >> ci) & 1)) continue;
              for (int e = q.wl_off[t * 3 + ci]; e < q.wl_off[t * 3 + ci + 1]; e++)
                if ((okmask >> q.wl_set[e]) & 1u) {
                  worst = q.wl_price[e];
                  break;
                }
            }
            if (worst < price) rep |= 1ull << b;
          }
        }
        bool any = __any_sync(FULL, rep != 0);
        if (any && d.mv_strict && !min_values_ok(d, c_tmpl0, rep, lane)) any = false;
        if (any && spot_path && sn == 1) {
          int total = lane < ITW ? __popcll(rep) : 0;
          for (int o = 16; o; o >>= 1) total += __shfl_xor_sync(FULL, total, o);
          if (total < 15) {
            any = false;
          } else {
            if (lane < ITW) sb[lane] = rep;
            __syncwarp();
            auto prefix_bits = [&](int n) {
              uint64_t acc = 0;
              int taken = 0;
              for (int b0 = 0; b0 < n_ord && taken < n; b0 += 32) {
                const int i = b0 + lane;
                const int t = i < n_ord ? sv[i] : 0;
                const bool in = i < n_ord && ((sb[t >> 6] >> (t & 63)) & 1ull);
                const unsigned m = __ballot_sync(FULL, in);
                const int rank = taken + __popc(m & ((1u << lane) - 1));
                const bool take = in && rank < n;
                for (int l = 0; l < 32; l++) {
                  const int tt = __shfl_sync(FULL, take ? t : -1, l);
                  if (tt >= 0 && (tt >> 6) == lane) acc |= 1ull << (tt & 63);
                }
                taken += __popc(m);
              }
              return acc;
            };
            uint64_t first = prefix_bits(15);
            if (d.mv_strict && !min_values_ok(d, c_tmpl0, first, lane)) {
              int bad = 15, good = total;
              while (good - bad > 1) {
                const int mid = (good + bad) >> 1;
                if (min_values_ok(d, c_tmpl0, prefix_bits(mid), lane))
                  good = mid;
                else
                  bad = mid;
              }
              first = prefix_bits(good);
            }
            rep = first;
          }
        }
        if (any && q.filter_same_type && sn >= 2) {
          double max_price = 1.7976931348623157e308;
          for (int i = 0; i < sn; i++) {
            const int t = q.node_it[snodes[i]];
            if (t < 0) continue;
            const bool in_rep = (__shfl_sync(FULL, rep, t >> 6) >> (t & 63)) & 1ull;
            if (!in_rep) continue;
            double mine = 1.7976931348623157e308;
            for (int j = 0; j < sn; j++)
              if (q.node_it[snodes[j]] == t && q.node_price[snodes[j]] >= 0 && q.node_price[snodes[j]] < mine)
                mine = q.node_price[snodes[j]];
            if (mine > 1e308) mine = 0.0;
            if (mine < max_price) max_price = mine;
          }
          if (max_price < 1e308) {
            uint64_t keep = 0;
            if (lane < ITW)
              for (uint64_t bits = rep; bits;) {
                const int b = __ffsll((long long)bits) - 1;
                bits &= bits - 1;
                const int t = lane * 64 + b;
                double worst = 1.7976931348623157e308;
                for (int ci = 0; ci < 3 && worst > 1e308; ci++) {
                  if (q.ct_key < 0 || !((q.ct_order_valid >> ci) & 1)) continue;
                  for (int e = q.wl_off[t * 3 + ci]; e < q.wl_off[t * 3 + ci + 1]; e++)
                    if ((okmask >> q.wl_set[e]) & 1u) {
                      worst = q.wl_price[e];
                      break;
                    }
                }
                if (worst < max_price) keep |= 1ull << b;
              }
            rep = keep;
            any = __any_sync(FULL, rep != 0);
            if (any && d.mv_strict && !min_values_ok(d, c_tmpl0, rep, lane)) any = false;
          }
        }
        if (any) decision = KP_DECISION_REPLACE;
        if (any && q.export_order && q.repl_order) {
          if (lane < ITW) sb[lane] = rep;
          __syncwarp();
          int32_t* dst = q.repl_order + (size_t)s * q.order_cap;
          for (int b0 = 0; b0 < n_ord; b0 += 32) {
            const int i = b0 + lane;
            const int t = i < n_ord ? sv[i] : 0;
            const bool in = i < n_ord && ((sb[t >> 6] >> (t & 63)) & 1ull);
            const unsigned m = __ballot_sync(FULL, in);
            const int at = n_ord_out + __popc(m & ((1u << lane) - 1));
            if (in && at < q.order_cap) dst[at] = t;
            n_ord_out += __popc(m);
          }
          if (n_ord_out > q.order_cap) n_ord_out = q.order_cap;
        }
      }
    }
  }
  if (decision != KP_DECISION_REPLACE) rep = 0;
  if (lane < ITW) q.replacement_its[(size_t)s * ITW + lane] = rep;
  if (q.repl_tmpl) {
    const bool repl = decision == KP_DECISION_REPLACE && have_slots;
    Slot F = slot_absent();
    if (repl && lane < K) {
      F = scratch[lane];
      if (!spot_pinned && lane == q.ct_key && q.ct_spot >= 0 && q.ct_od >= 0) {
        const KeyInfo ki = key_info(d, lane);
        if (slot_has(ki, F, q.ct_spot) && slot_has(ki, F, q.ct_od)) F = slot_add(ki, F, Slot{SF_PRESENT, 1ull << q.ct_spot, 0, 0});
      }
    }
    if (lane < K) {
      const size_t i = (size_t)s * K + lane;
      q.repl_sflags[i] = (uint8_t)F.f;
      q.repl_smask[i] = F.m;
      if (q.repl_sgte) {
        q.repl_sgte[i] = F.gte;
        q.repl_slte[i] = F.lte;
      }
    }
    if (lane < d.R) q.repl_req[(size_t)s * d.R + lane] = repl ? c_req0[lane] : 0;
    if (lane == 0) {
      q.repl_tmpl[s] = repl ? c_tmpl0 : -1;
      if (q.repl_order_n) q.repl_order_n[s] = repl ? n_ord_out : 0;
    }
  }
  if (lane == 0) {
    q.decision[s] = (uint8_t)decision;
    q.n_new_claims[s] = n_new;
    q.n_unscheduled[s] = unscheduled;
  }
  __syncwarp();
}

#define CONSOL_WARPS 8
struct ConsolWarp {
  WInst inst;
  PodCtx ctx;
  Slot scratch[KP_MAXK];
};
struct ConsolShared {
  KpDev ds;
  ConsolWarp w[CONSOL_WARPS];
};

#ifndef CONSOL_MIN_CTAS
#define CONSOL_MIN_CTAS 2
#endif
template <bool LEAN>
__global__ void __launch_bounds__(CONSOL_WARPS * 32, CONSOL_MIN_CTAS) k_consolidate(const __grid_constant__ KpDev d_in,
                                                                    const __grid_constant__ KpConsol q) {
  extern __shared__ __align__(16) unsigned char smem_raw[];
  ConsolShared& sh = *reinterpret_cast<ConsolShared*>(smem_raw);
  const int lane = threadIdx.x & 31, warp = threadIdx.x >> 5;
  stage_tables(d_in, &sh.ds, smem_raw + KP_ALIGN16(sizeof(ConsolShared)));
  const KpDev& d = sh.ds;
  ConsolWarp& W = sh.w[warp];
  WInst& I = W.inst;
  const int R = d.R, N = d.N;
  const size_t slot = (size_t)blockIdx.x * CONSOL_WARPS + warp;
  const int capq = q.capq;
  const ConsolScratch w = consol_slot(d, q, slot);
  if (lane == 0) {
    I.queue = w.queue;
    I.qcls = w.qcls;
    I.last_len = w.last_len;
    I.pod_target = nullptr;
    I.pod_error = nullptr;
    I.Cmax = capq;
    I.c_tmpl = w.c_tmpl;
    I.c_npods = w.c_npods;
    I.c_req = w.c_req;
    I.c_sflags = w.c_sflags;
    I.c_smask = w.c_smask;
    I.c_sgte = w.c_sgte;
    I.c_slte = w.c_slte;
    I.c_its = w.c_its;
    I.c_j = w.c_j;
    I.order = w.order;
    I.cnt_at = w.cnt_at;
    I.cmask = w.cmask;
    I.amask = w.amask;
    I.tmpl_remaining = w.tmpl_remaining;
    I.node_rem = d.node_rem;
    I.node_rem_present = d.node_rem_present;
    I.node_sflags = d.node_sflags;
    I.node_smask = d.node_smask;
    I.node_sgte = d.node_sgte;
    I.node_slte = d.node_slte;
    I.node_npods = nullptr;
    I.nfit = d.nfit;
    I.nstat = d.nstat;
    I.nactive = d.nactive;
    I.nfit_sum = d.nfit_sum;
    I.nstat_sum = d.nstat_sum;
    I.CS = 0;
    I.CQ = 0;
    I.CR = 0;
    I.c_dom = nullptr;
    I.g_c_dom = nullptr;
    I.rsv_cap = w.rsv_cap;
    I.c_rsv = w.c_rsv;
    I.c_ports = w.c_ports;
    I.ov_ports = w.ov_ports;
    I.node_ports = d.node_ports;
    I.ov_cap = capq;
    I.ov_node = w.ov_node;
    I.ov_rem = w.ov_rem;
    I.ov_present = w.ov_present;
    I.ov_sflags = w.ov_sflags;
    I.ov_smask = w.ov_smask;
    I.ov_sgte = w.ov_sgte;
    I.ov_slte = w.ov_slte;
  }
  __syncwarp();
  int32_t* clsl = w.clsl;
  int32_t* rk = w.rk;
  uint8_t* kindl = w.kindl;
  if (lane == 0) I.pod_kind = kindl;
  unsigned long long t0 = 0;
  if (q.deadline_ns > 0) {
    if (lane == 0) {
      unsigned long long now;
      asm volatile("mov.u64 %0, %%globaltimer;" : "=l"(now));
      t0 = atomicCAS(q.t_start, 0ull, now);
      if (t0 == 0) t0 = now;
    }
    t0 = __shfl_sync(FULL, t0, 0);
  }

  for (;;) {
    if (q.deadline_ns > 0) {
      unsigned long long now;
      asm volatile("mov.u64 %0, %%globaltimer;" : "=l"(now));
      now = __shfl_sync(FULL, now, 0);
      if ((long long)(now - t0) > q.deadline_ns) break;
    }
    int s = 0;
    if (lane == 0) s = atomicAdd(q.next, 1);
    s = __shfl_sync(FULL, s, 0);
    if (s >= q.n_subsets) break;
    const int so = q.subset_off[s], sn = q.subset_off[s + 1] - so;
    const int32_t* snodes = q.subset_nodes + so;
    int n = 0;
    for (int i = 0; i < sn; i++) {
      const int node = snodes[i];
      const int a = q.node_pod_off[node], b = q.node_pod_off[node + 1];
      for (int j = a + lane; j < b; j += 32) {
        const int o = n + (j - a);
        if (o < capq) {
          clsl[o] = q.pod_class[j];
          rk[o] = q.pod_rank[j];
        }
      }
      n += b - a;
    }
    const int n_cand_pods = n;
    for (int j = lane; j < q.n_extra; j += 32) {
      const int o = n + j;
      if (o < capq) {
        clsl[o] = q.pod_class[q.extra_row0 + j];
        rk[o] = q.pod_rank[q.extra_row0 + j];
      }
    }
    n += q.n_extra;
    if (kindl)
      for (int i = lane; i < n && i < capq; i += 32) kindl[i] = i < n_cand_pods ? 0 : q.extra_kind[i - n_cand_pods];
    if (n > capq) {
      if (lane == 0) *q.status = KP_ERR_CAPACITY;
      break;
    }
    __syncwarp();
    for (int i = lane; i < n; i += 32) {
      const int my = rk[i];
      int pos = 0;
      for (int j = 0; j < n; j++) pos += rk[j] < my ? 1 : 0;
      I.queue[pos] = i;
      I.qcls[pos] = clsl[i];
    }
    if (lane == 0) {
      I.P = n;
      I.n_ov = 0;
      I.n_removed = sn;
      I.removed = snodes;
    }
    for (int i = lane; i < d.n_rsv; i += 32) I.rsv_cap[i] = d.rsv_cap[i];
    for (int i = lane; i < N * R; i += 32) {
      const int t = i / R, r = i % R;
      int64_t rem = q.tmpl_remaining0[i];
      if ((d.tmpl_limit_present[t] >> r) & 1)
        for (int c = 0; c < sn; c++)
          if (q.node_tmpl[snodes[c]] == t) rem += q.node_capacity[(size_t)snodes[c] * R + r];
      I.tmpl_remaining[i] = rem;
    }
    __syncwarp();
    wsolve_run<true, false, LEAN>(d, I, W.ctx, W.scratch, lane);
    if (I.status != KP_OK) {
      if (lane == 0) *q.status = I.status;
      break;
    }
    if (!LEAN) claims_finalize(d, I.c_sflags, I.c_smask, I.c_rsv, I.n_claims, lane);
    consol_decide(d, q, slot, W.scratch, I.c_sflags, I.c_smask, I.c_sgte, I.c_slte, I.c_its, I.n_claims > 0 ? I.c_tmpl[0] : -1,
                  I.c_req, I.n_claims > 0 ? I.c_npods[0] : 0, sn, snodes, I.n_unsched + I.n_uninit, I.n_claims, s, lane);
  }
}

__global__ void __launch_bounds__(32) k_decide_batch(const KpDev* __restrict__ devs, KpConsol q, const int32_t* __restrict__ soff,
                                                     const int32_t* __restrict__ snodes) {
  __shared__ Slot scratch[KP_MAXK];
  const int lane = threadIdx.x, b = blockIdx.x;
  const KpDev& d = devs[b];
  const int unscheduled = (int)(d.counters[7] + d.counters[8]);
  const int n_new = *d.n_claims;
  consol_decide(d, q, (size_t)b, scratch, d.c_sflags, d.c_smask, d.c_sgte, d.c_slte, d.c_its, n_new > 0 ? d.c_tmpl[0] : -1,
                d.c_req, n_new > 0 ? d.c_npods[0] : 0, soff[b + 1] - soff[b], snodes + soff[b], unscheduled, n_new, b, lane);
}

__global__ void __launch_bounds__(128) k_truncate_claims(KpDev d, PriceTabs pt, int max_n, double* sort_key, int32_t* sort_val,
                                                         unsigned long long* sort_bits, uint8_t* dropped) {
  __shared__ Slot scratch[4][KP_MAXK];
  const int lane = threadIdx.x & 31, wi = threadIdx.x >> 5, warp = blockIdx.x * 4 + wi, nw = gridDim.x * 4;
  const int K = d.K, ITW = d.ITW, nC = *d.n_claims;
  double* sk = sort_key + (size_t)warp * d.T;
  int32_t* sv = sort_val + (size_t)warp * d.T;
  unsigned long long* sb = sort_bits + (size_t)warp * ITW;
  for (int c = warp; c < nC; c += nw) {
    const uint64_t its = lane < ITW ? d.c_its[(size_t)c * ITW + lane] : 0ull;
    int n_its = lane < ITW ? __popcll(its) : 0;
    for (int o = 16; o; o >>= 1) n_its += __shfl_xor_sync(FULL, n_its, o);
    if (n_its <= max_n) continue;
    if (lane < K) scratch[wi][lane] = load_slot(d.c_sflags, d.c_smask, d.c_sgte, d.c_slte, (size_t)c * K + lane, d.has_bounds);
    __syncwarp();
    const unsigned okmask = offering_ok_mask(d, scratch[wi], lane);
    order_by_price(pt, its, n_its, okmask, sk, sv, ITW, lane);
    const uint64_t cur = first_types_bitmap(sv, max_n, sb, ITW, lane);
    if (lane < ITW) d.c_its[(size_t)c * ITW + lane] = cur;
    const bool ok = !d.mv_strict || min_values_ok(d, d.c_tmpl[c], cur, lane);
    if (lane == 0 && !ok) dropped[c] = 1;
    __syncwarp();
  }
}
__global__ void __launch_bounds__(256) k_mark_dropped(const int32_t* pod_target, uint8_t* pod_error, const uint8_t* dropped, int64_t P) {
  const int64_t i = blockIdx.x * (int64_t)blockDim.x + threadIdx.x;
  if (i >= P) return;
  const int t = pod_target[i];
  if (t <= -2 && dropped[-2 - t]) pod_error[i] = KP_PODERR_MINVALUES_TRUNCATED;
}
```

### karpenter_b200/csrc/kp_gosort.cuh

```cuda
#pragma once
#include <cuda_runtime.h>

#ifndef FULL
#define FULL 0xffffffffu
#endif

template <class K>
struct WarpSorterT {
  K* key;
  int* val;
  int lane;

  __device__ bool less(int i, int j) const { return key[i] < key[j]; }
  __device__ void swap(int i, int j) {
    if (lane == 0) {
      K tk = key[i];
      key[i] = key[j];
      key[j] = tk;
      int t = val[i];
      val[i] = val[j];
      val[j] = t;
    }
    __syncwarp();
  }
  __device__ int first_not_less(int i, int j, K pv) const {
    for (int b = i; b <= j; b += 32) {
      int idx = b + lane;
      unsigned m = __ballot_sync(FULL, idx <= j && !(key[idx] < pv));
      if (m) return b + __ffs(m) - 1;
    }
    return j + 1;
  }
  __device__ int last_less(int i, int j, K pv) const {
    for (int b = j; b >= i; b -= 32) {
      int idx = b - lane;
      unsigned m = __ballot_sync(FULL, idx >= i && key[idx] < pv);
      if (m) return b - (__ffs(m) - 1);
    }
    return i - 1;
  }
  __device__ int first_greater(int i, int j, K pv) const {
    for (int b = i; b <= j; b += 32) {
      int idx = b + lane;
      unsigned m = __ballot_sync(FULL, idx <= j && pv < key[idx]);
      if (m) return b + __ffs(m) - 1;
    }
    return j + 1;
  }
  __device__ int last_not_greater(int i, int j, K pv) const {
    for (int b = j; b >= i; b -= 32) {
      int idx = b - lane;
      unsigned m = __ballot_sync(FULL, idx >= i && !(pv < key[idx]));
      if (m) return b - (__ffs(m) - 1);
    }
    return i - 1;
  }
  __device__ void rotate_right(int to, int from) {
    const K ek = key[from];
    const int ev = val[from];
    for (int b0 = from; b0 > to; b0 -= 32) {
      const int i = b0 - lane;
      K vk = 0;
      int vv = 0;
      if (i > to) {
        vk = key[i - 1];
        vv = val[i - 1];
      }
      __syncwarp();
      if (i > to) {
        key[i] = vk;
        val[i] = vv;
      }
      __syncwarp();
    }
    if (lane == 0) {
      key[to] = ek;
      val[to] = ev;
    }
    __syncwarp();
  }
  __device__ void rotate_left(int from, int to) {
    const K ek = key[from];
    const int ev = val[from];
    for (int b0 = from; b0 < to; b0 += 32) {
      const int i = b0 + lane;
      K vk = 0;
      int vv = 0;
      if (i < to) {
        vk = key[i + 1];
        vv = val[i + 1];
      }
      __syncwarp();
      if (i < to) {
        key[i] = vk;
        val[i] = vv;
      }
      __syncwarp();
    }
    if (lane == 0) {
      key[to] = ek;
      val[to] = ev;
    }
    __syncwarp();
  }
  __device__ void insertion_sort(int a, int b) {
    const int n = b - a;
    K k = 0;
    int v = 0;
    if (lane < n) {
      k = key[a + lane];
      v = val[a + lane];
    }
    int rank = 0;
    for (int j = 0; j < n; j++) {
      const K kj = __shfl_sync(FULL, k, j);
      rank += (kj < k || (kj == k && j < lane)) ? 1 : 0;
    }
    __syncwarp();
    if (lane < n) {
      key[a + rank] = k;
      val[a + rank] = v;
    }
    __syncwarp();
  }
  __device__ void sift_down(int lo, int hi, int first) {
    int root = lo;
    for (;;) {
      int child = 2 * root + 1;
      if (child >= hi) return;
      if (child + 1 < hi && less(first + child, first + child + 1)) child++;
      if (!less(first + root, first + child)) return;
      swap(first + root, first + child);
      root = child;
    }
  }
  __device__ void heap_sort(int a, int b) {
    int first = a, lo = 0, hi = b - a;
    for (int i = (hi - 1) / 2; i >= 0; i--) sift_down(i, hi, first);
    for (int i = hi - 1; i >= 0; i--) {
      swap(first, first + i);
      sift_down(lo, i, first);
    }
  }
  __device__ int partition(int a, int b, int pivot, bool* already) {
    swap(a, pivot);
    const K pv = key[a];
    int i = a + 1, j = b - 1;
    i = first_not_less(i, j, pv);
    j = last_less(i, j, pv);
    if (i > j) {
      swap(j, a);
      *already = true;
      return j;
    }
    swap(i, j);
    i++;
    j--;
    for (;;) {
      i = first_not_less(i, j, pv);
      j = last_less(i, j, pv);
      if (i > j) break;
      swap(i, j);
      i++;
      j--;
    }
    swap(j, a);
    *already = false;
    return j;
  }
  __device__ int partition_equal(int a, int b, int pivot) {
    swap(a, pivot);
    const K pv = key[a];
    int i = a + 1, j = b - 1;
    for (;;) {
      i = first_greater(i, j, pv);
      j = last_not_greater(i, j, pv);
      if (i > j) break;
      swap(i, j);
      i++;
      j--;
    }
    return i;
  }
  __device__ bool partial_insertion_sort(int a, int b) {
    int i = a + 1;
    for (int j = 0; j < 5; j++) {
      {
        int found = b;
        for (int b0 = i; b0 < b; b0 += 32) {
          int idx = b0 + lane;
          unsigned m = __ballot_sync(FULL, idx < b && key[idx] < key[idx - 1]);
          if (m) {
            found = b0 + __ffs(m) - 1;
            break;
          }
        }
        i = found;
      }
      if (i == b) return true;
      if (b - a < 50) return false;
      swap(i, i - 1);
      if (i - a >= 2) {
        const K x = key[i - 1];
        int stop = last_not_greater_from(i - 2, x);
        if (stop + 1 < i - 1) rotate_right(stop + 1, i - 1);
      }
      if (b - i >= 2) {
        const K x = key[i];
        int stop = b;
        for (int b0 = i + 1; b0 < b; b0 += 32) {
          int idx = b0 + lane;
          unsigned m = __ballot_sync(FULL, idx < b && !(key[idx] < x));
          if (m) {
            stop = b0 + __ffs(m) - 1;
            break;
          }
        }
        if (stop - 1 > i) rotate_left(i, stop - 1);
      }
    }
    return false;
  }
  __device__ int last_not_greater_from(int hi, K x) const {
    for (int b = hi; b >= 0; b -= 32) {
      int idx = b - lane;
      unsigned m = __ballot_sync(FULL, idx >= 0 && !(x < key[idx]));
      if (m) return b - (__ffs(m) - 1);
    }
    return -1;
  }
  __device__ static int bits_len(unsigned long long x) { return x ? 64 - __clzll((long long)x) : 0; }
  __device__ void break_patterns(int a, int b) {
    int length = b - a;
    if (length >= 8) {
      unsigned long long random = (unsigned long long)length;
      unsigned long long modulus = 1ull << bits_len((unsigned long long)length);
      int idx = a + (length / 4) * 2 - 1;
      for (int i = 0; i < 3; i++) {
        random ^= random << 13;
        random ^= random >> 7;
        random ^= random << 17;
        int other = (int)(random & (modulus - 1));
        if (other >= length) other -= length;
        swap(idx - 1 + i, a + other);
      }
    }
  }
  __device__ void order2(int* a, int* b, int* swaps) const {
    if (less(*b, *a)) {
      (*swaps)++;
      int t = *a;
      *a = *b;
      *b = t;
    }
  }
  __device__ int median(int a, int b, int c, int* swaps) const {
    order2(&a, &b, swaps);
    order2(&b, &c, swaps);
    order2(&a, &b, swaps);
    return b;
  }
  __device__ int choose_pivot(int a, int b, int* hint) const {
    int l = b - a, swaps = 0;
    int i = a + l / 4 * 1, j = a + l / 4 * 2, k = a + l / 4 * 3;
    if (l >= 8) {
      if (l >= 50) {
        i = median(i - 1, i, i + 1, &swaps);
        j = median(j - 1, j, j + 1, &swaps);
        k = median(k - 1, k, k + 1, &swaps);
      }
      j = median(i, j, k, &swaps);
    }
    *hint = swaps == 0 ? 1 : (swaps == 12 ? 2 : 0);
    return j;
  }
  __device__ void reverse_range(int a, int b) {
    const int n = b - a;
    for (int b0 = 0; b0 < n / 2; b0 += 32) {
      const int t = b0 + lane;
      if (t < n / 2) {
        const int i = a + t, j = b - 1 - t;
        K tk = key[i];
        int tv = val[i];
        key[i] = key[j];
        val[i] = val[j];
        key[j] = tk;
        val[j] = tv;
      }
    }
    __syncwarp();
  }
  __device__ void pdqsort(int a, int b, int limit) {
    bool wasBalanced = true, wasPartitioned = true;
    for (;;) {
      int length = b - a;
      if (length <= 12) {
        insertion_sort(a, b);
        return;
      }
      if (limit == 0) {
        heap_sort(a, b);
        return;
      }
      if (!wasBalanced) {
        break_patterns(a, b);
        limit--;
      }
      int hint;
      int pivot = choose_pivot(a, b, &hint);
      if (hint == 2) {
        reverse_range(a, b);
        pivot = (b - 1) - (pivot - a);
        hint = 1;
      }
      if (wasBalanced && wasPartitioned && hint == 1) {
        if (partial_insertion_sort(a, b)) return;
      }
      if (a > 0 && !less(a - 1, pivot)) {
        a = partition_equal(a, b, pivot);
        continue;
      }
      bool already;
      int mid = partition(a, b, pivot, &already);
      wasPartitioned = already;
      int leftLen = mid - a, rightLen = b - mid;
      int balanceThreshold = length / 8;
      if (leftLen < rightLen) {
        wasBalanced = leftLen >= balanceThreshold;
        pdqsort(a, mid, limit);
        a = mid + 1;
      } else {
        wasBalanced = rightLen >= balanceThreshold;
        pdqsort(mid + 1, b, limit);
        b = mid;
      }
    }
  }
};
using WarpSorter = WarpSorterT<int>;
```

### karpenter_b200/csrc/kp_tables.hpp

```cpp
#pragma once
#include <cstdint>
#ifndef __CUDACC__
struct int4 { int x, y, z, w; };
struct ulonglong2 { unsigned long long x, y; };
#endif

#define KP_MAXK 32
#define KP_MAXR 8
#define KP_MAX_ITW 32
#define KP_MAX_OFFSETS 32
#define KP_HDR 10

#define SF_COMPLEMENT 0x01u
#define SF_HAS_GTE 0x02u
#define SF_HAS_LTE 0x04u
#define SF_PRESENT 0x10u

#define OP_IN 0
#define OP_NOT_IN 1
#define OP_EXISTS 2
#define OP_DNE 3

struct Slot {
  uint32_t f;
  uint64_t m;
  int64_t gte, lte;
};

struct ClsLane {
  uint64_t pod_m, strict_m;
  int64_t req;
  int32_t hdr;
  uint8_t pod_f, strict_f, pad[2];
};
static_assert(sizeof(ClsLane) == 32, "ClsLane is loaded as two 16-byte vectors");

struct KpGroup {
  int32_t key;
  int32_t type;
  int32_t max_skew;
  int32_t min_domains;
  int32_t inverse;
  int32_t dom_off;
  int32_t filter_off, filter_n;
  int32_t taint_policy, affinity_policy;
  int32_t tolset;
  int32_t host_row;
};
static_assert(sizeof(KpGroup) == 48, "KpGroup is read by value on the solver's critical path: three 16-byte loads");


struct KpDev {
  int K, R, T, ITW, N, X, G, GH, E, D;
  int n_reqsets, n_taintsets, n_tolsets;
  int has_bounds;
  int hostname_key;
  const uint8_t* key_wellknown;
  const uint64_t* key_univ;
  const int64_t* val_int;
  const uint64_t* val_isint;
  const uint8_t* rs_flags;
  const uint64_t* rs_mask;
  const int64_t* rs_gte;
  const int64_t* rs_lte;
  const uint8_t* tol_ok;
  const int32_t* itv_off;
  const uint64_t* itv;
  const uint64_t* it_nokey;
  const uint64_t* it_dne;
  const uint64_t* it_nonempty;
  const uint64_t* it_valid;
  const int32_t* ge_off;
  const int64_t* ge_vals;
  const uint64_t* ge_bits;
  const Slot* off_slots;
  const uint32_t* off_keys;
  const uint64_t* offset_bits;
  int tab_bytes;
  int n_ge, n_itv;
  const int64_t* it_capacity;
  const int32_t* tmpl_rs;
  const int32_t* tmpl_taintset;
  const uint64_t* tmpl_its_raw;
  uint64_t* tmpl_its;
  const int64_t* tmpl_daemon;
  int64_t* tmpl_remaining;
  const uint32_t* tmpl_limit_present;
  int nodes_res;
  const int64_t* cls_req;
  const int32_t* cls_rs;
  const int32_t* cls_tolset;
  const int32_t* cls_relax;
  int n_lazy;
  int32_t* g_born;
  int32_t* g_birth;
  const int32_t* cls_lazy_off;
  const int32_t* cls_lazy;
  int mv_strict;
  const int32_t* tmpl_mv_off;
  const int32_t* tmpl_mv_key;
  const int32_t* tmpl_mv_need;
  const int32_t* mv_val_off;
  const uint64_t* mv_masks;
  int n_rv;
  const int32_t* cls_match;
  const int32_t* cls_rec;
  const ClsLane* cls_lane;
  const int4* cls_hchk;
  const int64_t* cp_g;
  const int64_t* cp_l;
  const int64_t* cs_g;
  const int64_t* cs_l;
  const KpGroup* groups;
  const int32_t* filter_rs;
  int32_t* dom_cnt;
  uint64_t* dom_reg;
  uint64_t* dom_pop;
  int32_t* tk_slot;
  uint64_t *tk_reg, *tk_pop;
  int32_t* tk_cnt;
  int tk_nv;
  int32_t* g_ndomains;
  int32_t* g_nempty;
  int32_t* host_cnt;
  int GHS;
  uint32_t* host_pop;
  int HW;
  int H;
  const int32_t* node_taintset;
  const uint8_t* node_flags;
  int64_t* node_rem;
  uint32_t* node_rem_present;
  uint8_t* node_sflags;
  uint64_t* node_smask;
  int64_t* node_sgte;
  int64_t* node_slte;
  int32_t* node_npods;
  int Cmax;
  int32_t* c_tmpl;
  int32_t* c_npods;
  int64_t* c_req;
  uint8_t* c_sflags;
  uint64_t* c_smask;
  int64_t* c_sgte;
  int64_t* c_slte;
  uint64_t* c_its;
  int32_t* c_j;
  int32_t* order;
  int32_t* cnt_at;
  int n_fsig;
  ulonglong2* cmask;
  unsigned long long* amask;
  unsigned long long tmpl_all;
  int n_nsig, EW;
  uint32_t* nfit;
  uint32_t* nstat;
  uint32_t* nactive;
  int ESW;
  uint32_t* nfit_sum;
  uint32_t* nstat_sum;
  int64_t P;
  const int32_t* pod_class;
  int32_t* queue;
  int32_t* qcls;
  int32_t* last_len;
  int32_t* pod_target;
  uint8_t* pod_error;
  const uint8_t* pod_kind;
  int32_t* n_claims;
  int64_t* counters;
  int32_t* status;
  int stable_order;
  int n_hostports;
  int cohort;
  unsigned long long* c_ports;
  unsigned long long* node_ports;
  const unsigned long long* tmpl_ports;
  int n_rsv, rsv_strict;
  unsigned rsv_sets;
  const int32_t* set_rsv;
  int32_t* rsv_cap;
  unsigned long long* c_rsv;
  int rsv_ct_key, rsv_reserved_val, rsv_id_key;
  unsigned long long rsv_val_of[64];
  int tk_key;
  uint8_t* c_dom;
  long long deadline_ns;
};
```

### karpenter_b200/csrc/kp_wsolve.cuh

```cuda
#pragma once
#include "kp_gosort.cuh"
#include "kp_kernels.cuh"

enum { PERT_NONE = 0, PERT_INC = 1, PERT_APPEND = 2 };

enum { PH_POP = 0, PH_SORT, PH_DMASK, PH_SCAN, PH_FAST, PH_RECORD, PH_EVAL, PH_NEW, PH_OTHER, KP_NPHASE };
#ifdef KP_PHASE_PROF
#define KP_PROF_LAP(p)                        \
  do {                                        \
    const long long t_ = clock64();           \
    if (lane == 0) I.prof[p] += t_ - prof_t;  \
    prof_t = t_;                              \
  } while (0)
#define KP_PROF_AT 16
#define KP_NCOUNTERS (KP_PROF_AT + KP_NPHASE + 1)
#else
#define KP_PROF_LAP(p) \
  do {                 \
  } while (0)
#define KP_NCOUNTERS 16
#endif

struct WInst {
  int P;
  int32_t* queue;
  int32_t* qcls;
  int32_t* last_len;
  int32_t* pod_target;
  uint8_t* pod_error;
  const uint8_t* pod_kind;
  int Cmax;
  int32_t *c_tmpl, *c_npods;
  int64_t* c_req;
  uint8_t* c_sflags;
  uint64_t* c_smask;
  int64_t *c_sgte, *c_slte;
  uint64_t* c_its;
  int32_t* c_j;
  int CQ, CR;
  uint8_t* s_sflags;
  uint64_t* s_smask;
  int64_t* s_req;
  int32_t* s_j;
  uint64_t* s_its;
  int32_t *order, *cnt_at;
  ulonglong2* cmask;
  unsigned long long* amask;
  unsigned long long* g_amask;
  uint8_t *c_dom, *g_c_dom;
  int32_t* rsv_cap;
  unsigned long long* c_rsv;
  unsigned long long *c_ports, *node_ports, *ov_ports;
  int CS;
  int32_t *g_order, *g_cnt_at, *g_c_tmpl;
  ulonglong2* g_cmask;
  int64_t* tmpl_remaining;
  int64_t* node_rem;
  uint32_t* node_rem_present;
  uint8_t* node_sflags;
  uint64_t* node_smask;
  int64_t *node_sgte, *node_slte;
  int32_t* node_npods;
  uint32_t *nfit, *nstat;
  const uint32_t* nactive;
  const uint32_t *nfit_sum, *nstat_sum;
  int n_removed;
  const int32_t* removed;
  int ov_cap, n_ov;
  int32_t* ov_node;
  int64_t* ov_rem;
  uint32_t* ov_present;
  uint8_t* ov_sflags;
  uint64_t* ov_smask;
  int64_t *ov_sgte, *ov_slte;
  int n_claims, n_unsched, n_uninit, status;
  long long ev_existing, ev_inflight, ev_tmpl, commits, slow_sorts, scan_chunks, evals, fast_commits;
#ifdef KP_PHASE_PROF
  long long prof[KP_NPHASE], prof_total;
#endif
};

__device__ __forceinline__ int ov_find(const WInst& I, int node, int lane) {
  for (int b = 0; b < I.n_ov; b += 32) {
    int i = b + lane;
    unsigned m = __ballot_sync(FULL, i < I.n_ov && I.ov_node[i] == node);
    if (m) return b + __ffs(m) - 1;
  }
  return -1;
}

template <bool LEAN = false>
__device__ __forceinline__ void claim_load(const KpDev& d, const WInst& I, int c, int lane, Slot* b, int64_t* q,
                                           uint64_t* its, int* j) {
  const int K = d.K, R = d.R, ITW = d.ITW;
  *b = slot_absent();
  *q = 0;
  *its = 0;
  *j = 0;
  if (c < I.CR) {
    if (lane < K) {
      b->f = I.s_sflags[c * K + lane];
      b->m = I.s_smask[c * K + lane];
    }
    if (lane < ITW) *its = I.s_its[c * ITW + lane];
  } else {
    if (lane < K) {
      b->f = I.c_sflags[(size_t)c * K + lane];
      b->m = I.c_smask[(size_t)c * K + lane];
    }
    if (lane < ITW) *its = I.c_its[(size_t)c * ITW + lane];
  }
  if (lane < R) {
    if (c < I.CQ) {
      *q = I.s_req[c * R + lane];
      *j = I.s_j[c * R + lane];
    } else {
      *q = I.c_req[(size_t)c * R + lane];
      *j = I.c_j[(size_t)c * R + lane];
    }
  }
  if (!LEAN && d.has_bounds && lane < K) {
    b->gte = I.c_sgte[(size_t)c * K + lane];
    b->lte = I.c_slte[(size_t)c * K + lane];
  }
}
template <bool LEAN = false>
__device__ __forceinline__ void claim_store(const KpDev& d, WInst& I, int c, int lane, const Eval& ev, bool slots) {
  const int K = d.K, R = d.R, ITW = d.ITW;
  if (!LEAN && slots && I.c_dom && lane == d.tk_key)
    I.c_dom[c] = (ev.F.f == SF_PRESENT && __popcll(ev.F.m) == 1) ? (uint8_t)(__ffsll((long long)ev.F.m) - 1) : (uint8_t)0xff;
  if (c < I.CR) {
    if (slots && lane < K) {
      I.s_sflags[c * K + lane] = (uint8_t)ev.F.f;
      I.s_smask[c * K + lane] = ev.F.m;
    }
    if (lane < ITW) I.s_its[c * ITW + lane] = ev.its;
  } else {
    if (slots && lane < K) {
      I.c_sflags[(size_t)c * K + lane] = (uint8_t)ev.F.f;
      I.c_smask[(size_t)c * K + lane] = ev.F.m;
    }
    if (lane < ITW) I.c_its[(size_t)c * ITW + lane] = ev.its;
  }
  if (lane < R) {
    if (c < I.CQ) {
      I.s_req[c * R + lane] = ev.q;
      I.s_j[c * R + lane] = ev.j;
    } else {
      I.c_req[(size_t)c * R + lane] = ev.q;
      I.c_j[(size_t)c * R + lane] = ev.j;
    }
  }
  if (!LEAN && slots && d.has_bounds && lane < K) {
    I.c_sgte[(size_t)c * K + lane] = ev.F.gte;
    I.c_slte[(size_t)c * K + lane] = ev.F.lte;
  }
}
__device__ __forceinline__ void claim_load_rq(const KpDev& d, const WInst& I, int c, int lane, int64_t* q, int* j) {
  *q = 0;
  *j = 0;
  if (lane < d.R) {
    if (c < I.CQ) {
      *q = I.s_req[c * d.R + lane];
      *j = I.s_j[c * d.R + lane];
    } else {
      *q = I.c_req[(size_t)c * d.R + lane];
      *j = I.c_j[(size_t)c * d.R + lane];
    }
  }
}
__device__ __forceinline__ uint64_t claim_load_its(const KpDev& d, const WInst& I, int c, int lane) {
  if (lane >= d.ITW) return 0ull;
  return c < I.CR ? I.s_its[c * d.ITW + lane] : I.c_its[(size_t)c * d.ITW + lane];
}
__device__ __forceinline__ void claim_store_rq(const KpDev& d, WInst& I, int c, int lane, int64_t q, int j, bool with_its,
                                               uint64_t its) {
  if (lane < d.R) {
    if (c < I.CQ) {
      I.s_req[c * d.R + lane] = q;
      I.s_j[c * d.R + lane] = j;
    } else {
      I.c_req[(size_t)c * d.R + lane] = q;
      I.c_j[(size_t)c * d.R + lane] = j;
    }
  }
  if (with_its && lane < d.ITW) {
    if (c < I.CR)
      I.s_its[c * d.ITW + lane] = its;
    else
      I.c_its[(size_t)c * d.ITW + lane] = its;
  }
}
__device__ __forceinline__ void claim_rows_flush(const KpDev& d, WInst& I, int nC, int lane) {
  const int n = nC < I.CR ? nC : I.CR, nq = nC < I.CQ ? nC : I.CQ;
  for (int i = lane; i < n * d.K; i += 32) {
    I.c_sflags[i] = I.s_sflags[i];
    I.c_smask[i] = I.s_smask[i];
  }
  for (int i = lane; i < nq * d.R; i += 32) {
    I.c_req[i] = I.s_req[i];
    I.c_j[i] = I.s_j[i];
  }
  for (int i = lane; i < n * d.ITW; i += 32) I.c_its[i] = I.s_its[i];
  __syncwarp();
}

struct ScanCtx {
  unsigned long long fbit, rbit, tok;
  bool all_tmpl;
  int hoff, hend;
  int first_clear, first_rclear;
  bool use_ez;
  uint64_t ez;
  const int4* hc;
};
template <int U, bool LEAN = false>
__device__ __forceinline__ int next_candidate(const KpDev& d, const WInst& I, const int32_t* ord, int nC, int from,
                                              ScanCtx& sc, int lane, int E, int* cc_out, int limit = 0x7fffffff) {
  const ulonglong2* cm = I.cmask;
  if (limit > nC) limit = nC;
  for (int base = from; base < limit; base += 32 * U) {
    bool pass[U], fclear[U], rclear[U];
    int c[U];
#pragma unroll
    for (int u = 0; u < U; u++) {
      const int pos = base + u * 32 + lane;
      c[u] = -1;
      pass[u] = fclear[u] = rclear[u] = false;
      if (pos < limit && pos >= from) {
        c[u] = ord[pos];
        const ulonglong2 mk = cm[c[u]];
        fclear[u] = !(mk.x & sc.fbit);
        rclear[u] = !(mk.y & sc.rbit);
        pass[u] = fclear[u] && rclear[u];
        if (pass[u] && !sc.all_tmpl) pass[u] = (sc.tok >> I.c_tmpl[c[u]]) & 1ull;
      }
    }
    if (!LEAN && sc.use_ez) {
#pragma unroll
      for (int u = 0; u < U; u++)
        if (pass[u]) {
          const int z = I.c_dom[c[u]];
          if (z != 0xff) pass[u] = (sc.ez >> z) & 1ull;
        }
    }
    for (int i = sc.hoff; !LEAN && i < sc.hend; i += 2) {
      const bool two = i + 1 < sc.hend;
      const int4 ha = sc.hc[i], hb = two ? sc.hc[i + 1] : ha;
      const bool cnt_a = (ha.y & 0xff) == KP_TOPO_SPREAD, cnt_b = (hb.y & 0xff) == KP_TOPO_SPREAD;
      int ca[U], cb[U];
#pragma unroll
      for (int u = 0; u < U; u++) {
        const int hi = E + c[u];
        ca[u] = cb[u] = 0;
        if (pass[u]) {
          ca[u] = cnt_a ? __ldcg(d.host_cnt + (size_t)hi * d.GHS + ha.x)
                        : (int)((d.host_pop[(size_t)ha.x * d.HW + (hi >> 5)] >> (hi & 31)) & 1u);
          if (two)
            cb[u] = cnt_b ? __ldcg(d.host_cnt + (size_t)hi * d.GHS + hb.x)
                          : (int)((d.host_pop[(size_t)hb.x * d.HW + (hi >> 5)] >> (hi & 31)) & 1u);
        }
      }
#pragma unroll
      for (int r = 0; r < 2; r++) {
        if (r == 1 && !two) break;
        const int4 hc = r == 0 ? ha : hb;
        const int type = hc.y & 0xff, self = hc.y >> 8;
#pragma unroll
        for (int u = 0; u < U; u++) {
          if (!pass[u]) continue;
          const int hcnt = r == 0 ? ca[u] : cb[u];
          if (type == KP_TOPO_SPREAD)
            pass[u] = hcnt + self <= hc.z;
          else if (type == KP_TOPO_AFFINITY)
            pass[u] = hcnt > 0 || (self && (d.g_ndomains[hc.w] - d.g_nempty[hc.w]) == 0);
          else
            pass[u] = hcnt == 0;
        }
      }
    }
#pragma unroll
    for (int u = 0; u < U; u++) {
      if (sc.fbit && sc.first_clear < 0) {
        const unsigned fm = __ballot_sync(FULL, fclear[u]);
        if (fm) sc.first_clear = base + u * 32 + __ffs(fm) - 1;
      }
      if (sc.rbit && sc.first_rclear < 0) {
        const unsigned rm = __ballot_sync(FULL, rclear[u]);
        if (rm) sc.first_rclear = base + u * 32 + __ffs(rm) - 1;
      }
      const unsigned m = __ballot_sync(FULL, pass[u]);
      if (m) {
        const int l = __ffs(m) - 1;
        *cc_out = __shfl_sync(FULL, c[u], l);
        return base + u * 32 + l;
      }
    }
  }
  return -1;
}

template <bool LEAN>
__device__ __forceinline__ bool cheap_pass(const KpDev& d, const WInst& I, const ScanCtx& sc, int c, int E) {
  const ulonglong2 mk = I.cmask[c];
  bool pass = !(mk.x & sc.fbit) && !(mk.y & sc.rbit);
  if (pass && !sc.all_tmpl) pass = (sc.tok >> I.c_tmpl[c]) & 1ull;
  for (int i = sc.hoff; !LEAN && pass && i < sc.hend; i++) {
    const int4 hc = sc.hc[i];
    const int type = hc.y & 0xff, self = hc.y >> 8, hi = E + c;
    const int hcnt = type == KP_TOPO_SPREAD ? __ldcg(d.host_cnt + (size_t)hi * d.GHS + hc.x)
                                            : (int)((d.host_pop[(size_t)hc.x * d.HW + (hi >> 5)] >> (hi & 31)) & 1u);
    if (type == KP_TOPO_SPREAD)
      pass = hcnt + self <= hc.z;
    else if (type == KP_TOPO_AFFINITY)
      pass = hcnt > 0 || (self && (d.g_ndomains[hc.w] - d.g_nempty[hc.w]) == 0);
    else
      pass = hcnt == 0;
  }
  return pass;
}

__device__ __forceinline__ bool fp_fit(const KpDev& d, const WInst& I, const PodCtx& px, int cc, int k, int lane, int64_t* q_out,
                                       int* lo_out, bool* any_adv_out, uint64_t* its_out) {
  int64_t q;
  int j;
  claim_load_rq(d, I, cc, lane, &q, &j);
  int lo = j;
  bool adv = false;
  if (lane < d.R) {
    q += px.req[lane] * (int64_t)k;
    const int end = d.ge_off[lane + 1];
    while (lo < end && d.ge_vals[lo] < q) lo++;
    adv = lo != j;
  }
  unsigned advm = __ballot_sync(FULL, adv);
  const bool any_adv = advm != 0;
  uint64_t its = 0;
  bool ok = true;
  if (any_adv) {
    its = claim_load_its(d, I, cc, lane);
    const int jj = (lane < d.R && lo == d.ge_off[lane + 1]) ? -1 : lo;
    while (advm) {
      const int r = __ffs(advm) - 1;
      advm &= advm - 1;
      const int jr = __shfl_sync(FULL, jj, r);
      if (lane < d.ITW) its &= jr >= 0 ? d.ge_bits[(size_t)jr * d.ITW + lane] : 0ull;
    }
    ok = __any_sync(FULL, its != 0);
  }
  *q_out = q;
  *lo_out = lo;
  *any_adv_out = any_adv;
  *its_out = its;
  return ok;
}

__device__ __forceinline__ void migrate_small(const KpDev& d, WInst& I, int nC, int lane) {
  for (int i = lane; i < nC; i += 32) {
    I.g_order[i] = I.order[i];
    I.g_cnt_at[i] = I.cnt_at[i];
    I.g_c_tmpl[i] = I.c_tmpl[i];
    I.g_cmask[i] = I.cmask[i];
    I.g_amask[i] = I.amask[i];
    if (I.c_dom) I.g_c_dom[i] = I.c_dom[i];
  }
  __syncwarp();
  if (lane == 0) {
    I.order = I.g_order;
    I.cnt_at = I.g_cnt_at;
    I.c_tmpl = I.g_c_tmpl;
    I.cmask = I.g_cmask;
    I.amask = I.g_amask;
    if (I.c_dom) I.c_dom = I.g_c_dom;
    I.CS = 0;
  }
  __syncwarp();
}

#define KP_RING 8
struct StageRing {
  volatile int produced;
  volatile int consumed;
  volatile int tail_pub;
  volatile int done;
  volatile int skip_to;
  PodCtx slot[KP_RING];
};

template <bool COHORT>
__device__ void stager_run(const KpDev& d, const WInst& I, StageRing* ring, const int lane) {
  const int cap = I.P + 1;
  for (int base = 0;;) {
    int avail;
    for (;;) {
      if (ring->done) return;
      const int sk = __shfl_sync(FULL, (int)ring->skip_to, 0);
      if (sk > base) base = sk;
      avail = __shfl_sync(FULL, (int)ring->tail_pub, 0) - base;
      if (avail > 0) break;
      __nanosleep(64);
    }
    __threadfence_block();
    if (avail > 32) avail = 32;
    int li = 0, X = -1;
    if (lane < avail) {
      const int qi = (base + lane) % cap;
      li = __ldcg(I.queue + qi);
      X = __ldcg(I.qcls + qi);
    }
    ClassRegs nxt = load_class_regs(d, __shfl_sync(FULL, X, 0), __shfl_sync(FULL, li, 0), lane);
    bool rebased = false;
    for (int i = 0; i < avail; i++) {
      const int idx = base + i;
      const ClassRegs c = nxt;
      if (i + 1 < avail) nxt = load_class_regs(d, __shfl_sync(FULL, X, i + 1), __shfl_sync(FULL, li, i + 1), lane);
      int sk = 0;
      for (;;) {
        if (ring->done) return;
        sk = ring->skip_to;
        if (sk > idx || idx - ring->consumed < KP_RING) break;
        __nanosleep(32);
      }
      sk = __shfl_sync(FULL, sk, 0);
      if (sk > idx) {
        base = sk;
        rebased = true;
        break;
      }
      PodCtx& slot = ring->slot[idx & (KP_RING - 1)];
      store_class_regs(d, slot, c, lane);
      if (COHORT) {
        const int Xi = __shfl_sync(FULL, X, i);
        const unsigned same = __ballot_sync(FULL, lane >= i && lane < avail && X == Xi && base + lane < I.P);
        const unsigned tail_m = same >> i;
        const int run = tail_m == FULL ? 32 : __ffs(~tail_m) - 1;
        const int rp = __shfl_sync(FULL, li, (i + lane) & 31);
        slot.run_pod[lane] = rp;
        if (lane == 0) slot.run_n = run;
      }
      __syncwarp();
      if (slot.n_hc > 0) {
        const int g8 = lane >> 3, l8 = lane & 7;
        for (int k = g8; k < slot.n_hc; k += 4) {
          const int w = (d.E >> 5) + l8 * 32;
          if (w < d.HW) prefetch_l1(d.host_pop + (size_t)slot.hc[k].x * d.HW + w);
        }
      }
      if (!d.tk_slot && slot.n_mg > 0 && lane < 2 * slot.n_mg) {
        const KpGroup& G = slot.mg[lane >> 1];
        if (G.key == d.tk_key) prefetch_l1(d.dom_cnt + G.dom_off + (lane & 1) * 32);
      }
      __threadfence_block();
      __syncwarp();
      if (lane == 0) ring->produced = idx + 1;
    }
    if (!rebased) base += avail;
  }
}

struct CohortOut {
  int state;
  int npods;
  int nevals;
  long long ev_sum;
  int pert, pert_pos;
  unsigned moved;
  int w0, gE;
};
template <bool LEAN>
__device__ __noinline__ CohortOut cohort_try(const KpDev& d, WInst& I, const PodCtx& px, const ScanCtx sc, int32_t* ord, int32_t* cnt,
                                             const int nC, const int lb, const int cpos, const int cc, const int E, const int lane,
                                             const unsigned long long abit, const unsigned long long rbit, const bool fast_ok,
                                             const bool has_tk) {
  CohortOut out;
  out.state = 0;
  out.npods = 0;
  out.nevals = 0;
  out.ev_sum = 0;
  out.pert = PERT_NONE;
  out.pert_pos = 0;
  out.moved = 0;
  out.w0 = 0;
  out.gE = 0;
  bool fp0 = (I.amask[cc] & abit) != 0;
  if (fp0 && !fast_ok && has_tk) fp0 = I.c_dom[cc] != 0xff;
  if (!fp0) return out;
  int w0 = cpos;
  if (!LEAN && sc.use_ez) {
    ScanCtx st = sc;
    st.use_ez = false;
    st.first_clear = 0;
    st.first_rclear = 0;
    int c2;
    w0 = st.hend > st.hoff ? next_candidate<4, LEAN>(d, I, ord, nC, lb, st, lane, E, &c2)
                           : next_candidate<1, LEAN>(d, I, ord, nC, lb, st, lane, E, &c2);
    if (w0 < 0 || w0 > cpos) w0 = cpos;
  }
  const int pw = w0 + lane;
  int wc = -1, wn = -1;
  if (pw < nC) {
    wc = ord[pw];
    wn = cnt[pw];
  }
  const int c0 = __shfl_sync(FULL, wn, 0);
  const unsigned gmask = __ballot_sync(FULL, pw < nC && wn == c0);
  const int gsz = gmask == FULL ? 32 : __ffs(~gmask) - 1;
  const int L = px.run_n;
  if (fast_ok && gsz == 1) {
    const int nxt = __shfl_sync(FULL, wn, 1);
    int kcap = L;
    if (w0 + 1 < nC && (long long)nxt - c0 + 1 < kcap) kcap = nxt - c0 + 1;
    int64_t q, qb;
    int lo, lob;
    bool adv, advb;
    uint64_t its, itsb;
    int k = kcap;
    out.nevals = 1;
    if (!fp_fit(d, I, px, cc, k, lane, &q, &lo, &adv, &its)) {
      int good = 0, bad = kcap;
      while (bad - good > 1) {
        const int mid = (good + bad) >> 1;
        if (fp_fit(d, I, px, cc, mid, lane, &qb, &lob, &advb, &itsb)) {
          good = mid;
          q = qb;
          lo = lob;
          adv = advb;
          its = itsb;
        } else {
          bad = mid;
        }
      }
      k = good;
    }
    if (k == 0) {
      if (lane == 0) I.cmask[cc].y |= rbit;
      __syncwarp();
      out.state = 1;
      return out;
    }
    claim_store_rq(d, I, cc, lane, q, lo, adv, its);
    if (lane == 0) cnt[cpos] += k;
    if (I.pod_target && lane < k) {
      I.pod_target[px.run_pod[lane]] = KP_TARGET_CLAIM(cc);
      I.pod_error[px.run_pod[lane]] = KP_PODERR_NONE;
    }
    __syncwarp();
    out.state = 2;
    out.npods = k;
    out.ev_sum = (long long)k * (cpos + 1);
    out.pert = PERT_INC;
    out.pert_pos = cpos;
    return out;
  }
  if (!(gsz >= 2 && cpos < w0 + gsz && (d.stable_order || nC <= 12 || nC >= 50))) return out;
  bool wpass = false, wfp = false;
  int wz = -1;
  if (lane < gsz) {
    wpass = cheap_pass<LEAN>(d, I, sc, wc, E);
    if (wpass) {
      wfp = (I.amask[wc] & abit) != 0;
      if (wfp && !fast_ok && has_tk) {
        wz = I.c_dom[wc];
        wfp = wz != 0xff;
      }
    }
  }
  unsigned avail = __ballot_sync(FULL, wpass && wfp);
  const unsigned bar = __ballot_sync(FULL, wpass && !wfp);
  if (bar) avail &= (1u << (__ffs(bar) - 1)) - 1;
  if (!((avail >> (cpos - w0)) & 1u)) return out;
  const bool gend_known = gsz < 32 || w0 + 32 >= nC;
  unsigned picked = 0;
  int npick = 0, nmoved = 0, my_t = -1, j = 0;
  int prev_l = -1, prev_pj = 0;
  bool prev_inv = false;
  while (j < L) {
    if (prev_l >= 0) {
      bool stable = true;
      if (prev_inv && !d.stable_order && nC > 12) {
        const int q4 = nC / 4, pj = prev_pj;
        stable = !(pj == q4 - 1 || pj == q4 || pj == 2 * q4 - 1 || pj == 2 * q4 || pj == 3 * q4 - 1 || pj == 3 * q4);
      }
      if (!stable) break;
      if (lane == prev_l) my_t = nmoved;
      nmoved++;
      picked |= 1u << prev_l;
      prev_l = -1;
    }
    unsigned allowed = avail;
    if (!LEAN && has_tk) {
      uint64_t ez = sc.ez;
      if (j > 0) {
        bool exact;
        ez = domain_mask(d, px, lane, &exact);
        if (!exact) break;
      }
      allowed &= __ballot_sync(FULL, wz >= 0 && ((ez >> wz) & 1ull));
    }
    if (!allowed) break;
    const int l = __ffs(allowed) - 1;
    const int cl = __shfl_sync(FULL, wc, l);
    int64_t q;
    int lo;
    bool adv;
    uint64_t its;
    out.nevals++;
    avail &= ~(1u << l);
    if (!fp_fit(d, I, px, cl, 1, lane, &q, &lo, &adv, &its)) {
      if (lane == 0) I.cmask[cl].y |= rbit;
      __syncwarp();
      continue;
    }
    claim_store_rq(d, I, cl, lane, q, lo, adv, its);
    const int pj = w0 + l - __popc(picked & ((1u << l) - 1));
    out.ev_sum += pj + 1;
    if (lane == 0 && I.pod_target) {
      I.pod_target[px.run_pod[j]] = KP_TARGET_CLAIM(cl);
      I.pod_error[px.run_pod[j]] = KP_PODERR_NONE;
    }
    if (!LEAN && !fast_ok) topo_record_fast(d, px, __shfl_sync(FULL, wz, l), d.tmpl_taintset[I.c_tmpl[cl]], E + cl, lane);
    __syncwarp();
    const unsigned rest = gmask & ~picked & ~(1u << l);
    prev_inv = !gend_known || (rest & ~((2u << l) - 1u)) != 0;
    prev_l = l;
    prev_pj = pj;
    j++;
    npick++;
  }
  if (npick == 0) {
    out.state = 1;
    return out;
  }
  const int m = nmoved;
  int gE = w0 + gsz - 1;
  if (gsz == 32 && m > 0) {
    for (int s0 = w0 + 32;; s0 += 32) {
      const int i = s0 + lane;
      const bool in = i < nC && cnt[i] == c0;
      const int vo = in ? ord[i] : 0;
      const unsigned gk = __ballot_sync(FULL, in);
      const int n = gk == FULL ? 32 : __ffs(~gk) - 1;
      __syncwarp();
      if (lane < n) {
        ord[i - m] = vo;
        cnt[i - m] = c0;
      }
      __syncwarp();
      gE = s0 + n - 1;
      if (n < 32) break;
    }
  }
  const bool mv = (picked >> lane) & 1u;
  const int rank = __popc(~picked & ((1u << lane) - 1));
  __syncwarp();
  if (lane < gsz) {
    if (mv) {
      ord[gE - my_t] = wc;
      cnt[gE - my_t] = c0 + 1;
    } else {
      ord[w0 + rank] = wc;
      cnt[w0 + rank] = lane == prev_l ? c0 + 1 : c0;
    }
  }
  __syncwarp();
  out.state = 2;
  out.npods = npick;
  out.moved = picked;
  out.w0 = w0;
  out.gE = gE;
  if (prev_l >= 0) {
    out.pert = PERT_INC;
    out.pert_pos = w0 + __popc(~picked & ((1u << prev_l) - 1));
  }
  return out;
}

__device__ __forceinline__ void load_alt_slots(const KpDev& d, PodCtx& px, int alt, int lane) {
  if (lane < d.K) {
    const ClsLane c = d.cls_lane[(size_t)alt * 32 + lane];
    Slot sl;
    sl.f = c.pod_f;
    sl.m = c.pod_m;
    sl.gte = 0;
    sl.lte = 0;
    if (d.has_bounds) {
      sl.gte = d.cp_g[(size_t)alt * d.K + lane];
      sl.lte = d.cp_l[(size_t)alt * d.K + lane];
    }
    px.pod_slot[lane] = sl;
  }
  __syncwarp();
}
__device__ __forceinline__ int next_alt(const KpDev& d, int alt) { return d.cls_lane[(size_t)alt * 32 + KP_HDR + 10].hdr; }

template <bool OVERLAY, bool STAGED, bool LEAN = false, bool COHORT = false, bool VOL = false>
__device__ void wsolve_run(const KpDev& d, WInst& I, PodCtx& ctx, Slot* scratch, const int lane, StageRing* ring = nullptr) {
  const int K = d.K, R = d.R, ITW = d.ITW, E = d.E, EW = d.EW;
  const int P = I.P;
  int head = 0, tail = P;
  const int cap = P + 1;
  int hq = 0, tq = P;
  const long long watchdog_limit = 4ll * P + 1024;
  int nC = 0;
  int pert = PERT_NONE, pert_pos = 0;
  long long ev_existing = 0, ev_inflight = 0, ev_tmpl = 0, commits = 0, slow_sorts = 0, scan_chunks = 0, evals = 0, fast_commits = 0;
  int n_unsched = 0, n_uninit = 0, status = KP_OK, n_born = 0;
  int32_t* ord = I.order;
  int32_t* cnt = I.cnt_at;
  int alive_tmpl = 0;
  for (int n = 0; n < d.N; n++) {
    uint64_t w = lane < ITW ? d.tmpl_its[(size_t)n * ITW + lane] : 0ull;
    alive_tmpl += __any_sync(FULL, w != 0) ? 1 : 0;
  }
  int n_active_nodes = 0;
  for (int w = lane; w < EW; w += 32) n_active_nodes += __popc(I.nactive[w]);
  for (int o = 16; o; o >>= 1) n_active_nodes += __shfl_xor_sync(FULL, n_active_nodes, o);
  if (OVERLAY) n_active_nodes -= I.n_removed;

  ClassRegs pf;
  int pf_idx = -1, ids_idx = -1, ids_cls = 0, ids_pod = 0;
  pf.hdr = 0;
  pf.req = 0;
  pf.pod = slot_absent();
  pf.strict = slot_absent();

  int lb0 = 0, lb1 = 0;
  int lr0 = 0, lr1 = 0;
  long long watchdog = 0;
  unsigned long long t_start = 0;
  if (d.deadline_ns > 0) asm volatile("mov.u64 %0, %%globaltimer;" : "=l"(t_start));
#ifdef KP_PHASE_PROF
  long long prof_t = clock64();
  const long long prof_t0 = prof_t;
  if (lane == 0)
    for (int p = 0; p < KP_NPHASE; p++) I.prof[p] = 0;
#endif
  for (;;) {
    KP_PROF_LAP(PH_OTHER);
    const int len = tail - head;
    if (len == 0) break;
    if (d.deadline_ns > 0 && (watchdog & 63) == 0) {
      unsigned long long now;
      asm volatile("mov.u64 %0, %%globaltimer;" : "=l"(now));
      now = __shfl_sync(FULL, now, 0);
      if ((long long)(now - t_start) > d.deadline_ns) {
        status = KP_DEADLINE;
        break;
      }
    }
    if (++watchdog > watchdog_limit) {
      status = KP_ERR_INVALID;
      break;
    }
    const int h = head;
    const int hq1 = hq + 1 >= cap ? hq + 1 - cap : hq + 1, hq2 = hq1 + 1 >= cap ? hq1 + 1 - cap : hq1 + 1;
    int li, X;
    if (STAGED) {
      if (lane == 0) ring->consumed = h;
      while (ring->produced <= h) {
      }
      __threadfence_block();
      __syncwarp();
      const PodCtx& sx = ring->slot[h & (KP_RING - 1)];
      li = sx.pod;
      X = sx.cls;
    } else if (ids_idx == h) {
      li = ids_pod;
      X = ids_cls;
    } else {
      li = I.queue[hq];
      X = I.qcls[hq];
    }
    if (h >= P && I.last_len[li] == len) break;
    head = h + 1;
    hq = hq1;
    if (!STAGED) {
      {
        ClassRegs cur = pf_idx == h ? pf : load_class_regs(d, X, li, lane);
        __syncwarp();
        store_class_regs(d, ctx, cur, lane);
        __syncwarp();
      }
      pf_idx = -1;
      if (h + 1 < tail) {
        int nli, nX;
        if (ids_idx == h + 1) {
          nli = ids_pod;
          nX = ids_cls;
        } else {
          nli = I.queue[hq1];
          nX = I.qcls[hq1];
        }
        pf = load_class_regs(d, nX, nli, lane);
        pf_idx = h + 1;
      }
      ids_idx = -1;
      if (h + 2 < tail) {
        ids_pod = I.queue[hq2];
        ids_cls = I.qcls[hq2];
        ids_idx = h + 2;
      }
    }
    PodCtx& pxw = STAGED ? ring->slot[h & (KP_RING - 1)] : ctx;
    int Xc = X;
  try_pod:
    const PodCtx& px = pxw;
    const int rv = px.rv, fsig = px.fsig;
    const unsigned long long fbit = (fsig >= 0 && fsig < 64) ? 1ull << fsig : 0ull;
    const unsigned long long rbit = (rv < 64 && !(VOL && px.vol_next >= 0)) ? 1ull << rv : 0ull;
    bool found = false;
    KP_PROF_LAP(PH_POP);

    if (E > 0 && px.nsig >= 0) {
      const uint32_t* fitrow = I.nfit + (size_t)rv * EW;
      const uint32_t* strow = I.nstat + (size_t)px.nsig * EW;
      int seen = 0;
      unsigned live = 0xffffffffu;
      if (d.ESW <= 32) {
        const uint32_t sw = lane < d.ESW ? (I.nfit_sum[(size_t)rv * d.ESW + lane] & I.nstat_sum[(size_t)px.nsig * d.ESW + lane]) : 0u;
        live = __ballot_sync(FULL, sw != 0);
      }
      for (int w0 = 0; w0 < EW && !found; w0 += 32) {
        if (d.ESW <= 32 && !((live >> (w0 >> 5)) & 1u)) continue;
        const int w = w0 + lane;
        uint32_t bits = w < EW ? (fitrow[w] & strow[w] & I.nactive[w]) : 0u;
        if (OVERLAY)
          for (int i = 0; i < I.n_removed; i++)
            if ((I.removed[i] >> 5) == w) bits &= ~(1u << (I.removed[i] & 31));
        unsigned has = __ballot_sync(FULL, bits != 0);
        while (has && !found) {
          const int src = __ffs(has) - 1;
          has &= has - 1;
          uint32_t bw = __shfl_sync(FULL, bits, src);
          while (bw && !found) {
            const int b = __ffs(bw) - 1;
            bw &= bw - 1;
            const int node = (w0 + src) * 32 + b;
            seen++;
            int oi = -1;
            if (OVERLAY) oi = ov_find(I, node, lane);
            Slot nb = slot_absent();
            int64_t rem = 0;
            uint32_t pr;
            if (OVERLAY && oi >= 0) {
              if (lane < K) nb = load_slot(I.ov_sflags, I.ov_smask, I.ov_sgte, I.ov_slte, (size_t)oi * K + lane, (!LEAN && d.has_bounds));
              if (lane < R) rem = I.ov_rem[(size_t)oi * R + lane];
              pr = I.ov_present[oi];
            } else {
              if (lane < K)
                nb = load_slot(I.node_sflags, I.node_smask, I.node_sgte, I.node_slte, (size_t)node * K + lane, (!LEAN && d.has_bounds));
              if (lane < R) rem = I.node_rem[(size_t)node * R + lane];
              pr = I.node_rem_present[node];
            }
            if (!LEAN && px.port_conf) {
              const unsigned long long used = (OVERLAY && oi >= 0) ? I.ov_ports[oi] : I.node_ports[node];
              if (used & px.port_conf) continue;
            }
            bool bad = false;
            if (lane < R) {
              const bool present = (pr >> lane) & 1;
              if (present && rem < 0) bad = true;
              if (px.req[lane] > (present ? rem : 0)) bad = true;
            }
            if (__any_sync(FULL, bad)) {
              if (!OVERLAY && lane == 0) I.nfit[(size_t)rv * EW + (node >> 5)] &= ~(1u << (node & 31));
              continue;
            }
            Eval ev = eval_candidate<LEAN>(d, px, false, nb, 0, 0, 0, node, scratch, lane);
            if (VOL && !ev.ok && px.vol_next >= 0) {
              for (int alt = px.vol_next; alt >= 0 && !ev.ok; alt = next_alt(d, alt)) {
                load_alt_slots(d, pxw, alt, lane);
                ev = eval_candidate<LEAN>(d, px, false, nb, 0, 0, 0, node, scratch, lane);
              }
              if (!ev.ok) load_alt_slots(d, pxw, Xc, lane);
            }
            if (!ev.ok) continue;
            if (OVERLAY) {
              const bool oi_new = oi < 0;
              if (oi < 0) {
                oi = I.n_ov;
                if (oi >= I.ov_cap) {
                  status = KP_ERR_CAPACITY;
                  break;
                }
                if (lane == 0) {
                  I.ov_node[oi] = node;
                  I.n_ov = oi + 1;
                }
              }
              if (lane < K) {
                const size_t i = (size_t)oi * K + lane;
                I.ov_sflags[i] = (uint8_t)ev.F.f;
                I.ov_smask[i] = ev.F.m;
                if ((!LEAN && d.has_bounds)) {
                  I.ov_sgte[i] = ev.F.gte;
                  I.ov_slte[i] = ev.F.lte;
                }
              }
              if (lane < R) I.ov_rem[(size_t)oi * R + lane] = rem - px.req[lane];
              if (lane == 0) I.ov_present[oi] = pr | ((1u << R) - 1);
              if (!LEAN && d.n_hostports && lane == 0) I.ov_ports[oi] = (oi_new ? I.node_ports[node] : I.ov_ports[oi]) | px.ports;
              __syncwarp();
            } else {
              if (ev.changed && lane < K) {
                const size_t i = (size_t)node * K + lane;
                I.node_sflags[i] = (uint8_t)ev.F.f;
                I.node_smask[i] = ev.F.m;
                if ((!LEAN && d.has_bounds)) {
                  I.node_sgte[i] = ev.F.gte;
                  I.node_slte[i] = ev.F.lte;
                }
              }
              if (lane < R) I.node_rem[(size_t)node * R + lane] = rem - px.req[lane];
              if (lane == 0) {
                I.node_rem_present[node] = pr | ((1u << R) - 1);
                I.node_npods[node]++;
                if (!LEAN && px.ports) I.node_ports[node] |= px.ports;
              }
            }
            if (lane == 0) {
              if (I.pod_target) {
                I.pod_target[li] = node;
                I.pod_error[li] = KP_PODERR_NONE;
              }
            }
            if (!(d.node_flags[node] & KP_NODE_INITIALIZED) && (!I.pod_kind || I.pod_kind[li] == 0)) n_uninit++;
            if (!LEAN) topo_record(d, px, ev.F, d.node_taintset[node], node, false, lane);
            ev_existing += node + 1;
            found = true;
          }
          if (status != KP_OK) break;
        }
        if (status != KP_OK) break;
      }
      if (status != KP_OK) break;
      if (found) {
        commits++;
        continue;
      }
      ev_existing += n_active_nodes;
    } else if (E > 0) {
      ev_existing += n_active_nodes;
    }

    KP_PROF_LAP(PH_OTHER);
    if (pert != PERT_NONE) {
      const int p = pert_pos;
      const bool inversion = pert == PERT_INC ? (p + 1 < nC && cnt[p + 1] < cnt[p]) : (nC >= 2 && cnt[nC - 1] < cnt[nC - 2]);
      if (inversion) {
        bool stable = d.stable_order || nC <= 12;
        if (!stable && nC >= 50) {
          const int q4 = nC / 4;
          stable = pert == PERT_APPEND || !(p == q4 - 1 || p == q4 || p == 2 * q4 - 1 || p == 2 * q4 || p == 3 * q4 - 1 || p == 3 * q4);
        }
        if (stable) {
          if (pert == PERT_INC) {
            const int ec = cnt[p], eo = ord[p];
            int i0 = p;
            for (;;) {
              const int i = i0 + lane;
              const bool in = i + 1 < nC;
              const int vc = in ? cnt[i + 1] : 0x7fffffff, vo = in ? ord[i + 1] : 0;
              const unsigned stop = __ballot_sync(FULL, vc >= ec);
              const int nmove = stop ? __ffs(stop) - 1 : 32;
              __syncwarp();
              if (lane < nmove) {
                cnt[i] = vc;
                ord[i] = vo;
              }
              __syncwarp();
              i0 += nmove;
              if (nmove < 32) break;
            }
            if (lane == 0) {
              cnt[i0] = ec;
              ord[i0] = eo;
            }
            if (p < lb0 && lb0 <= i0) lb0--;
            if (p < lb1 && lb1 <= i0) lb1--;
            if (p < lr0 && lr0 <= i0) lr0--;
            if (p < lr1 && lr1 <= i0) lr1--;
          } else {
            const int ec = cnt[nC - 1], eo = ord[nC - 1];
            int i0 = nC - 1;
            for (;;) {
              const int i = i0 - lane;
              const bool in = i - 1 >= 0;
              const int vc = in ? cnt[i - 1] : -0x7fffffff, vo = in ? ord[i - 1] : 0;
              const unsigned stop = __ballot_sync(FULL, vc <= ec);
              const int nmove = stop ? __ffs(stop) - 1 : 32;
              __syncwarp();
              if (lane < nmove) {
                cnt[i] = vc;
                ord[i] = vo;
              }
              __syncwarp();
              i0 -= nmove;
              if (nmove < 32) break;
            }
            if (lane == 0) {
              cnt[i0] = ec;
              ord[i0] = eo;
            }
            if (lb0 > i0) lb0 = i0;
            if (lb1 > i0) lb1 = i0;
            if (lr0 > i0) lr0 = i0;
            if (lr1 > i0) lr1 = i0;
          }
        } else {
          WarpSorter s{cnt, ord, lane};
          s.pdqsort(0, nC, WarpSorter::bits_len((unsigned long long)nC));
          slow_sorts++;
          lb0 = 0;
          lb1 = 0;
          lr0 = 0;
          lr1 = 0;
        }
        __syncwarp();
      } else if (pert == PERT_APPEND) {
        if (lb0 > nC - 1) lb0 = nC - 1;
        if (lb1 > nC - 1) lb1 = nC - 1;
        if (lr0 > nC - 1) lr0 = nC - 1;
        if (lr1 > nC - 1) lr1 = nC - 1;
      }
      pert = PERT_NONE;
    }
    KP_PROF_LAP(PH_SORT);

    {
      ScanCtx sc;
      sc.fbit = fbit;
      sc.rbit = rbit;
      sc.tok = px.tmpl_ok;
      sc.all_tmpl = (sc.tok & d.tmpl_all) == d.tmpl_all;
      sc.first_clear = -1;
      sc.first_rclear = -1;
      sc.use_ez = false;
      sc.ez = ~0ull;
      const int tki = px.tkinfo;
      const unsigned long long abit = (tki & TKI_ABIT) ? 1ull << (tki & 63) : 0ull;
      const bool fast_ok = tki & TKI_FAST;
      bool dom_fp = false, has_tk = false;
      if (!LEAN && (tki & TKI_TOPO)) {
        if (px.n_hc >= 0) {
          sc.hc = px.hc;
          sc.hoff = 0;
          sc.hend = px.n_hc;
        } else {
          sc.hc = d.cls_hchk;
          sc.hoff = px.hoff;
          sc.hend = px.hend;
        }
        dom_fp = (tki & TKI_FP) && I.c_dom != nullptr;
        has_tk = tki & TKI_TK;
        if (dom_fp && has_tk) {
          bool exact;
          sc.ez = domain_mask(d, px, lane, &exact);
          sc.use_ez = exact;
          dom_fp = exact;
        }
        dom_fp = dom_fp && abit != 0;
      } else {
        sc.hc = nullptr;
        sc.hoff = 0;
        sc.hend = 0;
      }
      KP_PROF_LAP(PH_DMASK);
      int lbf = 0, lbr = 0;
      if (fbit) lbf = __shfl_sync(FULL, fsig < 32 ? lb0 : lb1, fsig & 31);
      if (rbit) lbr = __shfl_sync(FULL, rv < 32 ? lr0 : lr1, rv & 31);
      const int lb = lbf > lbr ? lbf : lbr;
      const bool scanned = (sc.tok & d.tmpl_all) != 0;
      int from = lb;
      unsigned coh_moved = 0;
      int coh_w0 = 0, coh_gE = 0, coh_extra = 0;
      bool coh_ok = COHORT && STAGED && !OVERLAY && d.cohort && Xc == X && px.run_n >= 2 && abit != 0 && (fast_ok || dom_fp) &&
                    (LEAN || (px.ports == 0 && px.port_conf == 0)) && (fast_ok || !has_tk || n_active_nodes == 0);
      for (int i = sc.hoff; !LEAN && coh_ok && i < sc.hend; i++)
        if ((sc.hc[i].y & 0xff) == KP_TOPO_AFFINITY) coh_ok = false;
      while (scanned && !found) {
        int cc;
        int cpos;
        if (sc.hend > sc.hoff) {
          const int lim = from + 32;
          cpos = next_candidate<1, LEAN>(d, I, ord, nC, from, sc, lane, E, &cc, lim);
          if (cpos < 0 && lim < nC) cpos = next_candidate<4, LEAN>(d, I, ord, nC, lim, sc, lane, E, &cc);
        } else {
          cpos = next_candidate<1, LEAN>(d, I, ord, nC, from, sc, lane, E, &cc);
        }
        KP_PROF_LAP(PH_SCAN);
        if (cpos < 0) break;
        from = cpos + 1;
        {
          if (!LEAN && px.port_conf && (I.c_ports[cc] & px.port_conf)) continue;
          if (COHORT && coh_ok) {
            const CohortOut co = cohort_try<LEAN>(d, I, px, sc, ord, cnt, nC, lb, cpos, cc, E, lane, abit, rbit, fast_ok, has_tk);
            KP_PROF_LAP(PH_FAST);
            evals += co.nevals;
            if (co.state == 2) {
              fast_commits += co.npods;
              ev_inflight += co.ev_sum;
              coh_extra = co.npods - 1;
              coh_moved = co.moved;
              coh_w0 = co.w0;
              coh_gE = co.gE;
              pert = co.pert;
              pert_pos = co.pert_pos;
              found = true;
              continue;
            }
            if (co.state == 1) continue;
          }
          int zdom = -1;
          bool fp = false;
          if ((fast_ok || dom_fp) && (I.amask[cc] & abit)) {
            fp = true;
            if (!fast_ok && has_tk) {
              zdom = I.c_dom[cc];
              fp = zdom != 0xff;
            }
          }
          if (fp) {
            int64_t q;
            int lo;
            bool any_adv;
            uint64_t its;
            const bool ok = fp_fit(d, I, px, cc, 1, lane, &q, &lo, &any_adv, &its);
            evals++;
            if (!ok) {
              if (lane == 0) I.cmask[cc].y |= rbit;
              __syncwarp();
              KP_PROF_LAP(PH_FAST);
              continue;
            }
            claim_store_rq(d, I, cc, lane, q, lo, any_adv, its);
            if (lane == 0) {
              if (!LEAN && px.ports) I.c_ports[cc] |= px.ports;
              cnt[cpos]++;
              if (I.pod_target) {
                I.pod_target[li] = KP_TARGET_CLAIM(cc);
                I.pod_error[li] = KP_PODERR_NONE;
              }
            }
            KP_PROF_LAP(PH_FAST);
            if (!LEAN && !fast_ok) topo_record_fast(d, px, zdom, d.tmpl_taintset[I.c_tmpl[cc]], E + cc, lane);
            fast_commits++;
            __syncwarp();
            KP_PROF_LAP(PH_RECORD);
            pert = PERT_INC;
            pert_pos = cpos;
            ev_inflight += cpos + 1;
            found = true;
            continue;
          }
          Slot b;
          int64_t bq;
          uint64_t bi;
          int bj;
          claim_load<LEAN>(d, I, cc, lane, &b, &bq, &bi, &bj);
          evals++;
          Eval ev;
          unsigned long long held = 0, take = 0;
          bool alt_loaded = false;
          for (int alt = -1;;) {
            ev = eval_candidate<LEAN>(d, px, true, b, bq, bi, bj, E + cc, scratch, lane);
            if (!LEAN && d.mv_strict && ev.ok && !min_values_ok(d, I.c_tmpl[cc], ev.its, lane)) ev.ok = false;
            if (abit && ev.pod_noop && lane == 0) I.amask[cc] |= abit;
            held = 0;
            take = 0;
            if (!LEAN && d.n_rsv && ev.ok) {
              if (lane < K) scratch[lane] = ev.F;
              __syncwarp();
              held = I.c_rsv[cc];
              bool rerr;
              take = offerings_to_reserve(d, I.rsv_cap, scratch, ev.its, held, lane, &rerr);
              __syncwarp();
              if (rerr) ev.ok = false;
            }
            if (!VOL || ev.ok) break;
            alt = alt < 0 ? px.vol_next : next_alt(d, alt);
            if (alt < 0) break;
            load_alt_slots(d, pxw, alt, lane);
            alt_loaded = true;
          }
          if (VOL && alt_loaded && !ev.ok) load_alt_slots(d, pxw, Xc, lane);
          if (!ev.ok) {
            if (lane == 0) {
              ulonglong2 mk = I.cmask[cc];
              if (ev.res_dead) mk.y |= rbit;
              if (ev.compat_fail) mk.x |= fbit;
              I.cmask[cc] = mk;
            }
            __syncwarp();
            KP_PROF_LAP(PH_EVAL);
            continue;
          }
          claim_store<LEAN>(d, I, cc, lane, ev, ev.changed);
          if (!LEAN && d.n_rsv) {
            reservations_commit(d, I.rsv_cap, held, take, lane);
            if (lane == 0) I.c_rsv[cc] = take;
          }
          if (lane == 0) {
            if (!LEAN && px.ports) I.c_ports[cc] |= px.ports;
            cnt[cpos]++;
            if (I.pod_target) {
              I.pod_target[li] = KP_TARGET_CLAIM(cc);
              I.pod_error[li] = KP_PODERR_NONE;
            }
          }
          KP_PROF_LAP(PH_EVAL);
          if (!LEAN) topo_record(d, px, ev.F, d.tmpl_taintset[I.c_tmpl[cc]], E + cc, true, lane);
          __syncwarp();
          KP_PROF_LAP(PH_RECORD);
          pert = PERT_INC;
          pert_pos = cpos;
          ev_inflight += cpos + 1;
          found = true;
        }
      }
      if (fbit && scanned && lbf == lb) {
        const int nb = sc.first_clear >= 0 ? sc.first_clear : nC;
        if (lane == (fsig & 31)) {
          if (fsig < 32)
            lb0 = nb;
          else
            lb1 = nb;
        }
      }
      if (rbit && scanned && lbr == lb) {
        const int nb = sc.first_rclear >= 0 ? sc.first_rclear : nC;
        if (lane == (rv & 31)) {
          if (rv < 32)
            lr0 = nb;
          else
            lr1 = nb;
        }
      }
      if (found && coh_moved) {
        const int w0 = coh_w0, gE = coh_gE;
#define KP_COH_ADJ(b)                                                          \
  if ((b) > w0 && (b) <= gE) {                                                 \
    const int nb_ = (b) - w0;                                                  \
    (b) -= __popc(coh_moved & (nb_ >= 32 ? FULL : (1u << nb_) - 1u));          \
  }
        KP_COH_ADJ(lb0)
        KP_COH_ADJ(lb1)
        KP_COH_ADJ(lr0)
        KP_COH_ADJ(lr1)
#undef KP_COH_ADJ
      }
      if (found && coh_extra > 0) {
        commits += coh_extra;
        watchdog += coh_extra;
        scan_chunks += coh_extra + 1;
        if (E > 0) ev_existing += (long long)coh_extra * n_active_nodes;
        head += coh_extra;
        hq += coh_extra;
        if (hq >= cap) hq -= cap;
        if (STAGED) {
          if (lane == 0) ring->skip_to = head;
        }
      }
      if (found) {
        commits++;
        continue;
      }
      ev_inflight += nC;
    }

    int err = alive_tmpl ? KP_PODERR_INCOMPATIBLE : KP_PODERR_NO_TEMPLATES;
    for (int n = 0; n < d.N && !found; n++) {
      uint64_t tw = lane < ITW ? d.tmpl_its[(size_t)n * ITW + lane] : 0ull;
      const bool alive = __any_sync(FULL, tw != 0);
      if (!alive) continue;
      ev_tmpl++;
      const uint32_t lp = d.tmpl_limit_present[n];
      if (lp) {
        if (d.nodes_res >= 0 && (lp >> d.nodes_res & 1) && I.tmpl_remaining[(size_t)n * R + d.nodes_res] == 0) continue;
        if (lane < ITW) {
          uint64_t keep = 0;
          for (uint64_t bits = tw; bits;) {
            const int b = __ffsll((long long)bits) - 1;
            bits &= bits - 1;
            const int t = lane * 64 + b;
            bool viable = true;
            for (int r = 0; r < R; r++)
              if ((lp >> r & 1) && d.it_capacity[(size_t)t * R + r] > I.tmpl_remaining[(size_t)n * R + r]) viable = false;
            if (viable) keep |= 1ull << b;
          }
          tw = keep;
        }
        if (!__any_sync(FULL, tw != 0)) continue;
      }
      const int cnew = nC;
      if (cnew >= I.Cmax) {
        status = KP_ERR_CAPACITY;
        break;
      }
      if (!((px.tmpl_ok >> n) & 1ull)) continue;
      if (!LEAN && px.port_conf && (d.tmpl_ports[n] & px.port_conf)) continue;
      if (I.CS && cnew >= I.CS) {
        migrate_small(d, I, nC, lane);
        ord = I.order;
        cnt = I.cnt_at;
      }
      Slot b = lane < K ? rs_slot(d, d.tmpl_rs[n], lane) : slot_absent();
      const int64_t bq = lane < R ? d.tmpl_daemon[(size_t)n * R + lane] : 0;
      Eval ev;
      unsigned long long take = 0;
      bool rerr = false, alt_loaded = false;
      for (int alt = -1;;) {
        ev = eval_candidate<LEAN>(d, px, true, b, bq, tw, -1, E + cnew, scratch, lane);
        if (!LEAN && d.mv_strict && ev.ok && !min_values_ok(d, n, ev.its, lane)) ev.ok = false;
        take = 0;
        rerr = false;
        if (!LEAN && d.n_rsv && ev.ok) {
          if (lane < K) scratch[lane] = ev.F;
          __syncwarp();
          take = offerings_to_reserve(d, I.rsv_cap, scratch, ev.its, 0ull, lane, &rerr);
          __syncwarp();
          if (rerr) ev.ok = false;
        }
        if (!VOL || ev.ok) break;
        alt = alt < 0 ? px.vol_next : next_alt(d, alt);
        if (alt < 0) break;
        load_alt_slots(d, pxw, alt, lane);
        alt_loaded = true;
      }
      if (VOL && alt_loaded && !ev.ok) load_alt_slots(d, pxw, Xc, lane);
      if (rerr) {
        err = KP_PODERR_RESERVED;
        break;
      }
      if (!ev.ok) continue;
      claim_store<LEAN>(d, I, cnew, lane, ev, true);
      if (lane == 0) {
        I.c_tmpl[cnew] = n;
        ord[cnew] = cnew;
        cnt[cnew] = 1;
        if (I.pod_target) {
          I.pod_target[li] = KP_TARGET_CLAIM(cnew);
          I.pod_error[li] = KP_PODERR_NONE;
        }
      }
      if (lane == 0) {
        I.cmask[cnew] = make_ulonglong2(0ull, 0ull);
        I.amask[cnew] = ((px.tkinfo & TKI_ABIT) && ev.pod_noop) ? 1ull << (px.tkinfo & 63) : 0ull;
        if (!LEAN && d.n_rsv) I.c_rsv[cnew] = take;
        if (!LEAN && d.n_hostports) I.c_ports[cnew] = d.tmpl_ports[n] | px.ports;
      }
      if (!LEAN && d.n_rsv) reservations_commit(d, I.rsv_cap, 0ull, take, lane);
      if (lp) {
        for (int r = 0; r < R; r++) {
          if (!(lp >> r & 1)) continue;
          long long mx = 0;
          if (lane < ITW)
            for (uint64_t bits = ev.its; bits;) {
              const int bb = __ffsll((long long)bits) - 1;
              bits &= bits - 1;
              const long long capv = d.it_capacity[(size_t)(lane * 64 + bb) * R + r];
              if (capv > mx) mx = capv;
            }
          for (int o = 16; o; o >>= 1) {
            const long long other = __shfl_xor_sync(FULL, mx, o);
            if (other > mx) mx = other;
          }
          if (lane == 0) I.tmpl_remaining[(size_t)n * R + r] -= mx;
        }
      }
      if (!LEAN && d.GH > 0) {
        for (int g = lane; g < d.G; g += 32)
          if (d.groups[g].key == d.hostname_key) {
            d.g_ndomains[g]++;
            d.g_nempty[g]++;
          }
        __syncwarp();
      }
      if (!LEAN) topo_record(d, px, ev.F, d.tmpl_taintset[n], E + cnew, true, lane);
      __syncwarp();
      nC = cnew + 1;
      pert = PERT_APPEND;
      pert_pos = cnew;
      found = true;
      commits++;
    }
    KP_PROF_LAP(PH_NEW);
    if (status != KP_OK) break;
    if (!found) {
      const int nx = err == KP_PODERR_RESERVED ? -1 : px.relax;
      if (nx >= 0) {
        Xc = nx;
        for (int i = d.cls_lazy_off[nx]; !LEAN && i < d.cls_lazy_off[nx + 1]; i++) {
          const int g = d.cls_lazy[i];
          if (d.g_born[g]) continue;
          if (lane == 0) {
            d.g_born[g] = 1;
            d.g_birth[g] = n_born;
          }
          n_born++;
          __syncwarp();
        }
        ClassRegs cur = load_class_regs(d, Xc, li, lane);
        __syncwarp();
        store_class_regs(d, pxw, cur, lane);
        __syncwarp();
        goto try_pod;
      }
      if (lane == 0) {
        if (I.pod_target) {
          I.pod_error[li] = (uint8_t)err;
          I.pod_target[li] = KP_TARGET_UNSCHEDULED;
        }
        I.queue[tq] = li;
        I.qcls[tq] = X;
        I.last_len[li] = tail + 1 - head;
      }
      tail++;
      tq = tq + 1 >= cap ? tq + 1 - cap : tq + 1;
      if (STAGED) {
        __threadfence_block();
        if (lane == 0) ring->tail_pub = tail;
      }
      __syncwarp();
    }
  }
#ifdef KP_PHASE_PROF
  KP_PROF_LAP(PH_OTHER);
  if (lane == 0) I.prof_total = prof_t - prof_t0;
#endif
  if (STAGED) {
    __syncwarp();
    if (lane == 0) ring->done = 1;
  }
  for (int i = lane; i < nC; i += 32) I.c_npods[ord[i]] = cnt[i];
  n_unsched = tail - head;
  if (I.pod_kind && n_unsched > 0) {
    int keep = 0;
    for (int i = head + lane; i < tail; i += 32) keep += I.pod_kind[I.queue[i % cap]] != KP_EXTRA_PENDING;
    for (int o = 16; o; o >>= 1) keep += __shfl_xor_sync(FULL, keep, o);
    n_unsched = keep;
  }
  if (lane == 0) {
    I.n_claims = nC;
    I.n_unsched = n_unsched;
    I.n_uninit = n_uninit;
    I.status = status;
    I.ev_existing = ev_existing;
    I.ev_inflight = ev_inflight;
    I.ev_tmpl = ev_tmpl;
    I.commits = commits;
    I.slow_sorts = slow_sorts;
    I.scan_chunks = scan_chunks;
    I.evals = evals;
    I.fast_commits = fast_commits;
  }
  __syncwarp();
}
```

Baseline: 221,600.

## Store claim masks by sorted position and compact candidates before per-claim tests

Turns the per-claim cmask array into pmask, indexed by position in the sorted order, and moves its entries along with ord/cnt on every sort, rotation and shift. The candidate scan can then read mask words contiguously instead of gathering through ord. The scan also checks the first 32 positions on their own, then takes eight 32-wide chunks at a time, compacts the mask-passing positions with ballots, and runs the template/domain/topology tests only on the survivors. This adds extra 16-byte moves to every reorder of the claim list, and profiling counters for scan steps are added.

```diff
diff --git a/karpenter_b200/csrc/kp_api.cu b/karpenter_b200/csrc/kp_api.cu
--- a/karpenter_b200/csrc/kp_api.cu
+++ b/karpenter_b200/csrc/kp_api.cu
@@ -525,7 +525,7 @@
   CK(zeros(h, &d.c_j, C * t.R));
   CK(zeros(h, &d.order, C));
   CK(zeros(h, &d.cnt_at, C));
-  CK(zeros(h, &d.cmask, C));
+  CK(zeros(h, &d.pmask, C));
   CK(zeros(h, &d.amask, C));
   CK(zeros(h, &d.c_dom, C));
   d.n_hostports = p->n_hostports > 0 ? p->n_hostports : 0;
@@ -602,7 +602,7 @@
   CK(cudaMemsetAsync(d.node_npods, 0, (size_t)std::max(t.E, 1) * 4, h->stream));
   size_t C = (size_t)d.Cmax;
   CK(cudaMemsetAsync(d.c_npods, 0, C * 4, h->stream));
-  CK(cudaMemsetAsync(d.cmask, 0, C * sizeof(ulonglong2), h->stream));
+  CK(cudaMemsetAsync(d.pmask, 0, C * sizeof(ulonglong2), h->stream));
   CK(cudaMemsetAsync(d.amask, 0, C * 8, h->stream));
   CK(cudaMemsetAsync(d.c_rsv, 0, C * 8, h->stream));
   if (in.d_dropped) CK(cudaMemsetAsync(in.d_dropped, 0, C, h->stream));
@@ -641,16 +641,16 @@
     if (ntk > 0 && L.s_req - L.tk_slot <= 64 * 1024) in.tk_groups = ntk;
   }
   int CR = std::min(d.Cmax, 512);
-  while (CR > 0 && layout(0, CR, CR).cmask > budget / 2) CR -= 32;
+  while (CR > 0 && layout(0, CR, CR).pmask > budget / 2) CR -= 32;
   CR = std::max(CR, 0);
   const SolveSmem whole = layout(0, CR, CR);
-  const size_t rows = whole.cmask - whole.s_req;
+  const size_t rows = whole.pmask - whole.s_req;
   int CQ = CR;
   if (dom_fp) {
     CQ = std::min((d.Cmax + 31) / 32 * 32, (int)(rows / ((size_t)d.R * 12 + 1)) / 32 * 32);
-    while (CQ > 0 && layout(0, CQ, 0).cmask - whole.s_req > rows) CQ -= 32;
+    while (CQ > 0 && layout(0, CQ, 0).pmask - whole.s_req > rows) CQ -= 32;
     CR = 0;
-    while (CR + 32 <= CQ && layout(0, CQ, CR + 32).cmask - whole.s_req <= rows) CR += 32;
+    while (CR + 32 <= CQ && layout(0, CQ, CR + 32).pmask - whole.s_req <= rows) CR += 32;
   }
   int CS = 0;
   if (layout(64, CQ, CR).total <= budget) {
@@ -1216,10 +1216,10 @@
 #ifdef KP_PHASE_PROF
 int kp_phase_profile(kp_handle* h, int32_t instance, int64_t* out, int32_t n) {
   Instance* in = pick_instance(h, instance);
-  if (!in || n < KP_NPHASE + 1) return h->err = "kp_phase_profile: no such instance or buffer too small", -1;
+  if (!in || n < KP_NPROF) return h->err = "kp_phase_profile: no such instance or buffer too small", -1;
   cudaSetDevice(h->device);
-  CK(cudaMemcpy(out, in->dev.counters + KP_PROF_AT, (KP_NPHASE + 1) * 8, cudaMemcpyDeviceToHost));
-  return KP_NPHASE + 1;
+  CK(cudaMemcpy(out, in->dev.counters + KP_PROF_AT, KP_NPROF * 8, cudaMemcpyDeviceToHost));
+  return KP_NPROF;
 }
 #endif
 
diff --git a/karpenter_b200/csrc/kp_consolidate.cuh b/karpenter_b200/csrc/kp_consolidate.cuh
--- a/karpenter_b200/csrc/kp_consolidate.cuh
+++ b/karpenter_b200/csrc/kp_consolidate.cuh
@@ -121,7 +121,7 @@
 };
 
 struct SolveSmem {
-  size_t tab, tk_slot, tk_reg, tk_pop, tk_cnt, s_req, s_j, s_smask, s_its, s_sflags, cmask, amask, order, cnt_at, c_tmpl,
+  size_t tab, tk_slot, tk_reg, tk_pop, tk_cnt, s_req, s_j, s_smask, s_its, s_sflags, pmask, amask, order, cnt_at, c_tmpl,
       c_dom, total;
   __host__ __device__ SolveSmem(const KpDev& d, size_t tab_bytes, int CS, int CQ, int CR, int ntk) {
     size_t o = KP_ALIGN16(sizeof(WSolveShared));
@@ -140,7 +140,7 @@
     at(s_smask, KP_ALIGN16(c * d.K * 8));
     at(s_its, KP_ALIGN16(c * d.ITW * 8));
     at(s_sflags, KP_ALIGN16(c * d.K));
-    at(cmask, s * 16);
+    at(pmask, s * 16);
     at(amask, s * 8);
     at(order, s * 4);
     at(cnt_at, s * 4);
@@ -211,7 +211,7 @@
     I.c_j = d.c_j;
     I.order = d.order;
     I.cnt_at = d.cnt_at;
-    I.cmask = d.cmask;
+    I.pmask = d.pmask;
     I.amask = d.amask;
     I.tmpl_remaining = d.tmpl_remaining;
     I.node_rem = d.node_rem;
@@ -234,7 +234,7 @@
     I.g_order = d.order;
     I.g_cnt_at = d.cnt_at;
     I.g_c_tmpl = d.c_tmpl;
-    I.g_cmask = d.cmask;
+    I.g_pmask = d.pmask;
     I.g_amask = d.amask;
     I.c_dom = d.c_dom;
     I.g_c_dom = d.c_dom;
@@ -263,7 +263,7 @@
       I.CR = CR;
     }
     if (CS > 0) {
-      I.cmask = reinterpret_cast<ulonglong2*>(smem_raw + L.cmask);
+      I.pmask = reinterpret_cast<ulonglong2*>(smem_raw + L.pmask);
       I.amask = reinterpret_cast<unsigned long long*>(smem_raw + L.amask);
       I.order = reinterpret_cast<int32_t*>(smem_raw + L.order);
       I.cnt_at = reinterpret_cast<int32_t*>(smem_raw + L.cnt_at);
@@ -314,6 +314,9 @@
 #ifdef KP_PHASE_PROF
     for (int p = 0; p < KP_NPHASE; p++) d.counters[KP_PROF_AT + p] = I.prof[p];
     d.counters[KP_PROF_AT + KP_NPHASE] = I.prof_total;
+    d.counters[KP_PROF_AT + KP_NPHASE + 1] = I.scan_steps;
+    d.counters[KP_PROF_AT + KP_NPHASE + 2] = I.scan_pos;
+    d.counters[KP_PROF_AT + KP_NPHASE + 3] = I.scan_first_cyc;
 #endif
   }
 }
@@ -349,7 +352,7 @@
   X(c_its, uint64_t, (size_t)q.capq * d.ITW, true)                   \
   X(c_j, int32_t, (size_t)q.capq * d.R, true)                        \
   KP_SORT_SCRATCH(X, d, q)                                           \
-  X(cmask, ulonglong2, q.capq, true)                                 \
+  X(pmask, ulonglong2, q.capq, true)                                 \
   X(amask, unsigned long long, q.capq, true)                         \
   X(tmpl_remaining, int64_t, (size_t)(d.N > 0 ? d.N : 1) * d.R, true) \
   X(ov_node, int32_t, q.capq, true)                                  \
@@ -741,7 +744,7 @@
     I.c_j = w.c_j;
     I.order = w.order;
     I.cnt_at = w.cnt_at;
-    I.cmask = w.cmask;
+    I.pmask = w.pmask;
     I.amask = w.amask;
     I.tmpl_remaining = w.tmpl_remaining;
     I.node_rem = d.node_rem;
diff --git a/karpenter_b200/csrc/kp_gosort.cuh b/karpenter_b200/csrc/kp_gosort.cuh
--- a/karpenter_b200/csrc/kp_gosort.cuh
+++ b/karpenter_b200/csrc/kp_gosort.cuh
@@ -5,11 +5,12 @@
 #define FULL 0xffffffffu
 #endif
 
-template <class K>
+template <class K, bool PM = false>
 struct WarpSorterT {
   K* key;
   int* val;
   int lane;
+  ulonglong2* pm;
 
   __device__ bool less(int i, int j) const { return key[i] < key[j]; }
   __device__ void swap(int i, int j) {
@@ -20,6 +21,11 @@
       int t = val[i];
       val[i] = val[j];
       val[j] = t;
+      if (PM) {
+        const ulonglong2 tp = pm[i];
+        pm[i] = pm[j];
+        pm[j] = tp;
+      }
     }
     __syncwarp();
   }
@@ -58,48 +64,60 @@
   __device__ void rotate_right(int to, int from) {
     const K ek = key[from];
     const int ev = val[from];
+    ulonglong2 ep = {};
+    if (PM) ep = pm[from];
     for (int b0 = from; b0 > to; b0 -= 32) {
       const int i = b0 - lane;
       K vk = 0;
       int vv = 0;
+      ulonglong2 vp = {};
       if (i > to) {
         vk = key[i - 1];
         vv = val[i - 1];
+        if (PM) vp = pm[i - 1];
       }
       __syncwarp();
       if (i > to) {
         key[i] = vk;
         val[i] = vv;
+        if (PM) pm[i] = vp;
       }
       __syncwarp();
     }
     if (lane == 0) {
       key[to] = ek;
       val[to] = ev;
+      if (PM) pm[to] = ep;
     }
     __syncwarp();
   }
   __device__ void rotate_left(int from, int to) {
     const K ek = key[from];
     const int ev = val[from];
+    ulonglong2 ep = {};
+    if (PM) ep = pm[from];
     for (int b0 = from; b0 < to; b0 += 32) {
       const int i = b0 + lane;
       K vk = 0;
       int vv = 0;
+      ulonglong2 vp = {};
       if (i < to) {
         vk = key[i + 1];
         vv = val[i + 1];
+        if (PM) vp = pm[i + 1];
       }
       __syncwarp();
       if (i < to) {
         key[i] = vk;
         val[i] = vv;
+        if (PM) pm[i] = vp;
       }
       __syncwarp();
     }
     if (lane == 0) {
       key[to] = ek;
       val[to] = ev;
+      if (PM) pm[to] = ep;
     }
     __syncwarp();
   }
@@ -107,9 +125,11 @@
     const int n = b - a;
     K k = 0;
     int v = 0;
+    ulonglong2 p = {};
     if (lane < n) {
       k = key[a + lane];
       v = val[a + lane];
+      if (PM) p = pm[a + lane];
     }
     int rank = 0;
     for (int j = 0; j < n; j++) {
@@ -120,6 +140,7 @@
     if (lane < n) {
       key[a + rank] = k;
       val[a + rank] = v;
+      if (PM) pm[a + rank] = p;
     }
     __syncwarp();
   }
@@ -286,6 +307,11 @@
         val[i] = val[j];
         key[j] = tk;
         val[j] = tv;
+        if (PM) {
+          const ulonglong2 tp = pm[i];
+          pm[i] = pm[j];
+          pm[j] = tp;
+        }
       }
     }
     __syncwarp();
diff --git a/karpenter_b200/csrc/kp_tables.hpp b/karpenter_b200/csrc/kp_tables.hpp
--- a/karpenter_b200/csrc/kp_tables.hpp
+++ b/karpenter_b200/csrc/kp_tables.hpp
@@ -149,7 +149,7 @@
   int32_t* order;
   int32_t* cnt_at;
   int n_fsig;
-  ulonglong2* cmask;
+  ulonglong2* pmask;
   unsigned long long* amask;
   unsigned long long tmpl_all;
   int n_nsig, EW;
diff --git a/karpenter_b200/csrc/kp_wsolve.cuh b/karpenter_b200/csrc/kp_wsolve.cuh
--- a/karpenter_b200/csrc/kp_wsolve.cuh
+++ b/karpenter_b200/csrc/kp_wsolve.cuh
@@ -13,7 +13,8 @@
     prof_t = t_;                              \
   } while (0)
 #define KP_PROF_AT 16
-#define KP_NCOUNTERS (KP_PROF_AT + KP_NPHASE + 1)
+#define KP_NPROF (KP_NPHASE + 4)
+#define KP_NCOUNTERS (KP_PROF_AT + KP_NPROF)
 #else
 #define KP_PROF_LAP(p) \
   do {                 \
@@ -44,7 +45,7 @@
   int32_t* s_j;
   uint64_t* s_its;
   int32_t *order, *cnt_at;
-  ulonglong2* cmask;
+  ulonglong2* pmask;
   unsigned long long* amask;
   unsigned long long* g_amask;
   uint8_t *c_dom, *g_c_dom;
@@ -53,7 +54,7 @@
   unsigned long long *c_ports, *node_ports, *ov_ports;
   int CS;
   int32_t *g_order, *g_cnt_at, *g_c_tmpl;
-  ulonglong2* g_cmask;
+  ulonglong2* g_pmask;
   int64_t* tmpl_remaining;
   int64_t* node_rem;
   uint32_t* node_rem_present;
@@ -77,6 +78,7 @@
   long long ev_existing, ev_inflight, ev_tmpl, commits, slow_sorts, scan_chunks, evals, fast_commits;
 #ifdef KP_PHASE_PROF
   long long prof[KP_NPHASE], prof_total;
+  long long scan_steps, scan_pos, scan_first_cyc;
 #endif
 };
 
@@ -213,87 +215,150 @@
   bool use_ez;
   uint64_t ez;
   const int4* hc;
+#ifdef KP_PHASE_PROF
+  long long steps, first_cyc;
+#endif
 };
-template <int U, bool LEAN = false>
+
+template <bool LEAN>
+__device__ __forceinline__ bool claim_tests(const KpDev& d, const WInst& I, const ScanCtx& sc, int c, bool pass, int E) {
+  if (pass && !sc.all_tmpl) pass = (sc.tok >> I.c_tmpl[c]) & 1ull;
+  if (!LEAN && sc.use_ez && pass) {
+    const int z = I.c_dom[c];
+    if (z != 0xff) pass = (sc.ez >> z) & 1ull;
+  }
+  for (int i = sc.hoff; !LEAN && i < sc.hend; i += 2) {
+    const bool two = i + 1 < sc.hend;
+    const int4 ha = sc.hc[i], hb = two ? sc.hc[i + 1] : ha;
+    const bool cnt_a = (ha.y & 0xff) == KP_TOPO_SPREAD, cnt_b = (hb.y & 0xff) == KP_TOPO_SPREAD;
+    const int hi = E + c;
+    int ca = 0, cb = 0;
+    if (pass) {
+      ca = cnt_a ? __ldcg(d.host_cnt + (size_t)hi * d.GHS + ha.x)
+                 : (int)((d.host_pop[(size_t)ha.x * d.HW + (hi >> 5)] >> (hi & 31)) & 1u);
+      if (two)
+        cb = cnt_b ? __ldcg(d.host_cnt + (size_t)hi * d.GHS + hb.x)
+                   : (int)((d.host_pop[(size_t)hb.x * d.HW + (hi >> 5)] >> (hi & 31)) & 1u);
+    }
+#pragma unroll
+    for (int r = 0; r < 2; r++) {
+      if (r == 1 && !two) break;
+      const int4 hc = r == 0 ? ha : hb;
+      const int type = hc.y & 0xff, self = hc.y >> 8;
+      if (!pass) continue;
+      const int hcnt = r == 0 ? ca : cb;
+      if (type == KP_TOPO_SPREAD)
+        pass = hcnt + self <= hc.z;
+      else if (type == KP_TOPO_AFFINITY)
+        pass = hcnt > 0 || (self && (d.g_ndomains[hc.w] - d.g_nempty[hc.w]) == 0);
+      else
+        pass = hcnt == 0;
+    }
+  }
+  return pass;
+}
+
+__device__ __forceinline__ void scan_clear(ScanCtx& sc, int b, bool fclear, bool rclear) {
+  if (sc.fbit && sc.first_clear < 0) {
+    const unsigned fm = __ballot_sync(FULL, fclear);
+    if (fm) sc.first_clear = b + __ffs(fm) - 1;
+  }
+  if (sc.rbit && sc.first_rclear < 0) {
+    const unsigned rm = __ballot_sync(FULL, rclear);
+    if (rm) sc.first_rclear = b + __ffs(rm) - 1;
+  }
+}
+
+__device__ __forceinline__ int nth_bit(unsigned m, int n) {
+  int p = 0;
+#pragma unroll
+  for (int w = 16; w; w >>= 1) {
+    const int k = __popc(m & ((1u << w) - 1u));
+    if (n >= k) {
+      n -= k;
+      m >>= w;
+      p += w;
+    }
+  }
+  return p;
+}
+
+#define KP_SCAN_L1 8
+template <bool LEAN>
 __device__ __forceinline__ int next_candidate(const KpDev& d, const WInst& I, const int32_t* ord, int nC, int from,
-                                              ScanCtx& sc, int lane, int E, int* cc_out, int limit = 0x7fffffff) {
-  const ulonglong2* cm = I.cmask;
-  if (limit > nC) limit = nC;
-  for (int base = from; base < limit; base += 32 * U) {
-    bool pass[U], fclear[U], rclear[U];
-    int c[U];
+                                              ScanCtx& sc, int lane, int E, int* cc_out) {
+  const ulonglong2* pm = I.pmask;
+#ifdef KP_PHASE_PROF
+  const long long t0 = clock64();
+  sc.steps++;
+#endif
+  {
+    const int pos = from + lane;
+    int c = -1;
+    bool fclear = false, rclear = false;
+    if (pos < nC) {
+      c = ord[pos];
+      const ulonglong2 mk = pm[pos];
+      fclear = !(mk.x & sc.fbit);
+      rclear = !(mk.y & sc.rbit);
+    }
+    scan_clear(sc, from, fclear, rclear);
+    const unsigned m = __ballot_sync(FULL, claim_tests<LEAN>(d, I, sc, c, fclear && rclear, E));
+#ifdef KP_PHASE_PROF
+    sc.first_cyc += clock64() - t0;
+#endif
+    if (m) {
+      const int l = __ffs(m) - 1;
+      *cc_out = __shfl_sync(FULL, c, l);
+      return from + l;
+    }
+  }
+  for (int base = from + 32; base < nC; base += 32 * KP_SCAN_L1) {
+#ifdef KP_PHASE_PROF
+    sc.steps++;
+#endif
+    bool fclear[KP_SCAN_L1], rclear[KP_SCAN_L1];
 #pragma unroll
-    for (int u = 0; u < U; u++) {
+    for (int u = 0; u < KP_SCAN_L1; u++) {
       const int pos = base + u * 32 + lane;
-      c[u] = -1;
-      pass[u] = fclear[u] = rclear[u] = false;
-      if (pos < limit && pos >= from) {
-        c[u] = ord[pos];
-        const ulonglong2 mk = cm[c[u]];
+      fclear[u] = rclear[u] = false;
+      if (pos < nC) {
+        const ulonglong2 mk = pm[pos];
         fclear[u] = !(mk.x & sc.fbit);
         rclear[u] = !(mk.y & sc.rbit);
-        pass[u] = fclear[u] && rclear[u];
-        if (pass[u] && !sc.all_tmpl) pass[u] = (sc.tok >> I.c_tmpl[c[u]]) & 1ull;
-      }
-    }
-    if (!LEAN && sc.use_ez) {
+      }
+    }
+    unsigned sm[KP_SCAN_L1];
+    int pre[KP_SCAN_L1];
+    int S = 0;
 #pragma unroll
-      for (int u = 0; u < U; u++)
-        if (pass[u]) {
-          const int z = I.c_dom[c[u]];
-          if (z != 0xff) pass[u] = (sc.ez >> z) & 1ull;
-        }
-    }
-    for (int i = sc.hoff; !LEAN && i < sc.hend; i += 2) {
-      const bool two = i + 1 < sc.hend;
-      const int4 ha = sc.hc[i], hb = two ? sc.hc[i + 1] : ha;
-      const bool cnt_a = (ha.y & 0xff) == KP_TOPO_SPREAD, cnt_b = (hb.y & 0xff) == KP_TOPO_SPREAD;
-      int ca[U], cb[U];
+    for (int u = 0; u < KP_SCAN_L1; u++) {
+      scan_clear(sc, base + u * 32, fclear[u], rclear[u]);
+      sm[u] = __ballot_sync(FULL, fclear[u] && rclear[u]);
+      pre[u] = S;
+      S += __popc(sm[u]);
+    }
+    for (int b = 0; b < S; b += 32) {
+      const int r = b + lane;
+      int pos = -1, c = -1;
+      if (r < S) {
+        unsigned mu = sm[0];
+        int ru = r, uo = 0;
 #pragma unroll
-      for (int u = 0; u < U; u++) {
-        const int hi = E + c[u];
-        ca[u] = cb[u] = 0;
-        if (pass[u]) {
-          ca[u] = cnt_a ? __ldcg(d.host_cnt + (size_t)hi * d.GHS + ha.x)
-                        : (int)((d.host_pop[(size_t)ha.x * d.HW + (hi >> 5)] >> (hi & 31)) & 1u);
-          if (two)
-            cb[u] = cnt_b ? __ldcg(d.host_cnt + (size_t)hi * d.GHS + hb.x)
-                          : (int)((d.host_pop[(size_t)hb.x * d.HW + (hi >> 5)] >> (hi & 31)) & 1u);
-        }
-      }
-#pragma unroll
-      for (int r = 0; r < 2; r++) {
-        if (r == 1 && !two) break;
-        const int4 hc = r == 0 ? ha : hb;
-        const int type = hc.y & 0xff, self = hc.y >> 8;
-#pragma unroll
-        for (int u = 0; u < U; u++) {
-          if (!pass[u]) continue;
-          const int hcnt = r == 0 ? ca[u] : cb[u];
-          if (type == KP_TOPO_SPREAD)
-            pass[u] = hcnt + self <= hc.z;
-          else if (type == KP_TOPO_AFFINITY)
-            pass[u] = hcnt > 0 || (self && (d.g_ndomains[hc.w] - d.g_nempty[hc.w]) == 0);
-          else
-            pass[u] = hcnt == 0;
-        }
-      }
-    }
-#pragma unroll
-    for (int u = 0; u < U; u++) {
-      if (sc.fbit && sc.first_clear < 0) {
-        const unsigned fm = __ballot_sync(FULL, fclear[u]);
-        if (fm) sc.first_clear = base + u * 32 + __ffs(fm) - 1;
-      }
-      if (sc.rbit && sc.first_rclear < 0) {
-        const unsigned rm = __ballot_sync(FULL, rclear[u]);
-        if (rm) sc.first_rclear = base + u * 32 + __ffs(rm) - 1;
-      }
-      const unsigned m = __ballot_sync(FULL, pass[u]);
+        for (int u = 1; u < KP_SCAN_L1; u++)
+          if (r >= pre[u]) {
+            mu = sm[u];
+            ru = r - pre[u];
+            uo = u * 32;
+          }
+        pos = base + uo + nth_bit(mu, ru);
+        c = ord[pos];
+      }
+      const unsigned m = __ballot_sync(FULL, claim_tests<LEAN>(d, I, sc, c, r < S, E));
       if (m) {
         const int l = __ffs(m) - 1;
-        *cc_out = __shfl_sync(FULL, c[u], l);
-        return base + u * 32 + l;
+        *cc_out = __shfl_sync(FULL, c, l);
+        return __shfl_sync(FULL, pos, l);
       }
     }
   }
@@ -301,23 +366,10 @@
 }
 
 template <bool LEAN>
-__device__ __forceinline__ bool cheap_pass(const KpDev& d, const WInst& I, const ScanCtx& sc, int c, int E) {
-  const ulonglong2 mk = I.cmask[c];
-  bool pass = !(mk.x & sc.fbit) && !(mk.y & sc.rbit);
-  if (pass && !sc.all_tmpl) pass = (sc.tok >> I.c_tmpl[c]) & 1ull;
-  for (int i = sc.hoff; !LEAN && pass && i < sc.hend; i++) {
-    const int4 hc = sc.hc[i];
-    const int type = hc.y & 0xff, self = hc.y >> 8, hi = E + c;
-    const int hcnt = type == KP_TOPO_SPREAD ? __ldcg(d.host_cnt + (size_t)hi * d.GHS + hc.x)
-                                            : (int)((d.host_pop[(size_t)hc.x * d.HW + (hi >> 5)] >> (hi & 31)) & 1u);
-    if (type == KP_TOPO_SPREAD)
-      pass = hcnt + self <= hc.z;
-    else if (type == KP_TOPO_AFFINITY)
-      pass = hcnt > 0 || (self && (d.g_ndomains[hc.w] - d.g_nempty[hc.w]) == 0);
-    else
-      pass = hcnt == 0;
-  }
-  return pass;
+__device__ __forceinline__ bool cheap_pass(const KpDev& d, const WInst& I, const ScanCtx& sc, int c, ulonglong2 mk, int E) {
+  ScanCtx st = sc;
+  st.use_ez = false;
+  return claim_tests<LEAN>(d, I, st, c, !(mk.x & sc.fbit) && !(mk.y & sc.rbit), E);
 }
 
 __device__ __forceinline__ bool fp_fit(const KpDev& d, const WInst& I, const PodCtx& px, int cc, int k, int lane, int64_t* q_out,
@@ -360,7 +412,7 @@
     I.g_order[i] = I.order[i];
     I.g_cnt_at[i] = I.cnt_at[i];
     I.g_c_tmpl[i] = I.c_tmpl[i];
-    I.g_cmask[i] = I.cmask[i];
+    I.g_pmask[i] = I.pmask[i];
     I.g_amask[i] = I.amask[i];
     if (I.c_dom) I.g_c_dom[i] = I.c_dom[i];
   }
@@ -369,7 +421,7 @@
     I.order = I.g_order;
     I.cnt_at = I.g_cnt_at;
     I.c_tmpl = I.g_c_tmpl;
-    I.cmask = I.g_cmask;
+    I.pmask = I.g_pmask;
     I.amask = I.g_amask;
     if (I.c_dom) I.c_dom = I.g_c_dom;
     I.CS = 0;
@@ -492,15 +544,16 @@
     st.first_clear = 0;
     st.first_rclear = 0;
     int c2;
-    w0 = st.hend > st.hoff ? next_candidate<4, LEAN>(d, I, ord, nC, lb, st, lane, E, &c2)
-                           : next_candidate<1, LEAN>(d, I, ord, nC, lb, st, lane, E, &c2);
+    w0 = next_candidate<LEAN>(d, I, ord, nC, lb, st, lane, E, &c2);
     if (w0 < 0 || w0 > cpos) w0 = cpos;
   }
   const int pw = w0 + lane;
   int wc = -1, wn = -1;
+  ulonglong2 wp = make_ulonglong2(0ull, 0ull);
   if (pw < nC) {
     wc = ord[pw];
     wn = cnt[pw];
+    wp = I.pmask[pw];
   }
   const int c0 = __shfl_sync(FULL, wn, 0);
   const unsigned gmask = __ballot_sync(FULL, pw < nC && wn == c0);
@@ -533,7 +586,7 @@
       k = good;
     }
     if (k == 0) {
-      if (lane == 0) I.cmask[cc].y |= rbit;
+      if (lane == 0) I.pmask[cpos].y |= rbit;
       __syncwarp();
       out.state = 1;
       return out;
@@ -556,7 +609,7 @@
   bool wpass = false, wfp = false;
   int wz = -1;
   if (lane < gsz) {
-    wpass = cheap_pass<LEAN>(d, I, sc, wc, E);
+    wpass = cheap_pass<LEAN>(d, I, sc, wc, wp, E);
     if (wpass) {
       wfp = (I.amask[wc] & abit) != 0;
       if (wfp && !fast_ok && has_tk) {
@@ -607,7 +660,8 @@
     out.nevals++;
     avail &= ~(1u << l);
     if (!fp_fit(d, I, px, cl, 1, lane, &q, &lo, &adv, &its)) {
-      if (lane == 0) I.cmask[cl].y |= rbit;
+      if (lane == 0) I.pmask[w0 + l].y |= rbit;
+      if (lane == l) wp.y |= rbit;
       __syncwarp();
       continue;
     }
@@ -638,12 +692,14 @@
       const int i = s0 + lane;
       const bool in = i < nC && cnt[i] == c0;
       const int vo = in ? ord[i] : 0;
+      const ulonglong2 vp = in ? I.pmask[i] : make_ulonglong2(0ull, 0ull);
       const unsigned gk = __ballot_sync(FULL, in);
       const int n = gk == FULL ? 32 : __ffs(~gk) - 1;
       __syncwarp();
       if (lane < n) {
         ord[i - m] = vo;
         cnt[i - m] = c0;
+        I.pmask[i - m] = vp;
       }
       __syncwarp();
       gE = s0 + n - 1;
@@ -654,13 +710,10 @@
   const int rank = __popc(~picked & ((1u << lane) - 1));
   __syncwarp();
   if (lane < gsz) {
-    if (mv) {
-      ord[gE - my_t] = wc;
-      cnt[gE - my_t] = c0 + 1;
-    } else {
-      ord[w0 + rank] = wc;
-      cnt[w0 + rank] = lane == prev_l ? c0 + 1 : c0;
-    }
+    const int to = mv ? gE - my_t : w0 + rank;
+    ord[to] = wc;
+    cnt[to] = mv || lane == prev_l ? c0 + 1 : c0;
+    I.pmask[to] = wp;
   }
   __syncwarp();
   out.state = 2;
@@ -732,8 +785,10 @@
 #ifdef KP_PHASE_PROF
   long long prof_t = clock64();
   const long long prof_t0 = prof_t;
-  if (lane == 0)
+  if (lane == 0) {
     for (int p = 0; p < KP_NPHASE; p++) I.prof[p] = 0;
+    I.scan_steps = I.scan_pos = I.scan_first_cyc = 0;
+  }
 #endif
   for (;;) {
     KP_PROF_LAP(PH_OTHER);
@@ -953,20 +1008,24 @@
           const int q4 = nC / 4;
           stable = pert == PERT_APPEND || !(p == q4 - 1 || p == q4 || p == 2 * q4 - 1 || p == 2 * q4 || p == 3 * q4 - 1 || p == 3 * q4);
         }
+        ulonglong2* const pm = I.pmask;
         if (stable) {
           if (pert == PERT_INC) {
             const int ec = cnt[p], eo = ord[p];
+            const ulonglong2 ep = pm[p];
             int i0 = p;
             for (;;) {
               const int i = i0 + lane;
               const bool in = i + 1 < nC;
               const int vc = in ? cnt[i + 1] : 0x7fffffff, vo = in ? ord[i + 1] : 0;
+              const ulonglong2 vp = in ? pm[i + 1] : ep;
               const unsigned stop = __ballot_sync(FULL, vc >= ec);
               const int nmove = stop ? __ffs(stop) - 1 : 32;
               __syncwarp();
               if (lane < nmove) {
                 cnt[i] = vc;
                 ord[i] = vo;
+                pm[i] = vp;
               }
               __syncwarp();
               i0 += nmove;
@@ -975,6 +1034,7 @@
             if (lane == 0) {
               cnt[i0] = ec;
               ord[i0] = eo;
+              pm[i0] = ep;
             }
             if (p < lb0 && lb0 <= i0) lb0--;
             if (p < lb1 && lb1 <= i0) lb1--;
@@ -982,17 +1042,20 @@
             if (p < lr1 && lr1 <= i0) lr1--;
           } else {
             const int ec = cnt[nC - 1], eo = ord[nC - 1];
+            const ulonglong2 ep = pm[nC - 1];
             int i0 = nC - 1;
             for (;;) {
               const int i = i0 - lane;
               const bool in = i - 1 >= 0;
               const int vc = in ? cnt[i - 1] : -0x7fffffff, vo = in ? ord[i - 1] : 0;
+              const ulonglong2 vp = in ? pm[i - 1] : ep;
               const unsigned stop = __ballot_sync(FULL, vc <= ec);
               const int nmove = stop ? __ffs(stop) - 1 : 32;
               __syncwarp();
               if (lane < nmove) {
                 cnt[i] = vc;
                 ord[i] = vo;
+                pm[i] = vp;
               }
               __syncwarp();
               i0 -= nmove;
@@ -1001,6 +1064,7 @@
             if (lane == 0) {
               cnt[i0] = ec;
               ord[i0] = eo;
+              pm[i0] = ep;
             }
             if (lb0 > i0) lb0 = i0;
             if (lb1 > i0) lb1 = i0;
@@ -1008,7 +1072,7 @@
             if (lr1 > i0) lr1 = i0;
           }
         } else {
-          WarpSorter s{cnt, ord, lane};
+          WarpSorterT<int, true> s{cnt, ord, lane, pm};
           s.pdqsort(0, nC, WarpSorter::bits_len((unsigned long long)nC));
           slow_sorts++;
           lb0 = 0;
@@ -1037,6 +1101,10 @@
       sc.first_rclear = -1;
       sc.use_ez = false;
       sc.ez = ~0ull;
+#ifdef KP_PHASE_PROF
+      sc.steps = 0;
+      sc.first_cyc = 0;
+#endif
       const int tki = px.tkinfo;
       const unsigned long long abit = (tki & TKI_ABIT) ? 1ull << (tki & 63) : 0ull;
       const bool fast_ok = tki & TKI_FAST;
@@ -1080,14 +1148,10 @@
         if ((sc.hc[i].y & 0xff) == KP_TOPO_AFFINITY) coh_ok = false;
       while (scanned && !found) {
         int cc;
-        int cpos;
-        if (sc.hend > sc.hoff) {
-          const int lim = from + 32;
-          cpos = next_candidate<1, LEAN>(d, I, ord, nC, from, sc, lane, E, &cc, lim);
-          if (cpos < 0 && lim < nC) cpos = next_candidate<4, LEAN>(d, I, ord, nC, lim, sc, lane, E, &cc);
-        } else {
-          cpos = next_candidate<1, LEAN>(d, I, ord, nC, from, sc, lane, E, &cc);
-        }
+        const int cpos = next_candidate<LEAN>(d, I, ord, nC, from, sc, lane, E, &cc);
+#ifdef KP_PHASE_PROF
+        if (lane == 0) I.scan_pos += (cpos < 0 ? nC : cpos + 1) - from;
+#endif
         KP_PROF_LAP(PH_SCAN);
         if (cpos < 0) break;
         from = cpos + 1;
@@ -1128,7 +1192,7 @@
             const bool ok = fp_fit(d, I, px, cc, 1, lane, &q, &lo, &any_adv, &its);
             evals++;
             if (!ok) {
-              if (lane == 0) I.cmask[cc].y |= rbit;
+              if (lane == 0) I.pmask[cpos].y |= rbit;
               __syncwarp();
               KP_PROF_LAP(PH_FAST);
               continue;
@@ -1186,10 +1250,10 @@
           if (VOL && alt_loaded && !ev.ok) load_alt_slots(d, pxw, Xc, lane);
           if (!ev.ok) {
             if (lane == 0) {
-              ulonglong2 mk = I.cmask[cc];
+              ulonglong2 mk = I.pmask[cpos];
               if (ev.res_dead) mk.y |= rbit;
               if (ev.compat_fail) mk.x |= fbit;
-              I.cmask[cc] = mk;
+              I.pmask[cpos] = mk;
             }
             __syncwarp();
             KP_PROF_LAP(PH_EVAL);
@@ -1218,6 +1282,12 @@
           found = true;
         }
       }
+#ifdef KP_PHASE_PROF
+      if (lane == 0) {
+        I.scan_steps += sc.steps;
+        I.scan_first_cyc += sc.first_cyc;
+      }
+#endif
       if (fbit && scanned && lbf == lb) {
         const int nb = sc.first_clear >= 0 ? sc.first_clear : nC;
         if (lane == (fsig & 31)) {
@@ -1344,7 +1414,7 @@
         }
       }
       if (lane == 0) {
-        I.cmask[cnew] = make_ulonglong2(0ull, 0ull);
+        I.pmask[cnew] = make_ulonglong2(0ull, 0ull);
         I.amask[cnew] = ((px.tkinfo & TKI_ABIT) && ev.pod_noop) ? 1ull << (px.tkinfo & 63) : 0ull;
         if (!LEAN && d.n_rsv) I.c_rsv[cnew] = take;
         if (!LEAN && d.n_hostports) I.c_ports[cnew] = d.tmpl_ports[n] | px.ports;
```

Result: faster. 236,300, median of 6 (+6.6%).
